# Lichtso/contrast_renderer

Measured on AMD Instinct MI355X. Metric: paths/sec, 10k mixed-Bezier paths @ 4096^2 (tessellate + tile raster), higher is better.
Workload: dtype f32

## Files before the change

contrast_renderer_amd/_ffi.py:

```python
import ctypes as C
import os

import numpy as np

HERE = os.path.dirname(os.path.abspath(__file__))
LIB_PATH = os.path.join(HERE, "libcontrast_hip.so")

OK = 0
ERR_NUMBER_OF_STENCIL_BITS_IS_UNSUPPORTED = 1
ERR_CLIP_STACK_OVERFLOW = 2
ERR_TOO_MANY_NESTED_OPACITY_GROUPS = 3
ERR_TOO_MANY_DASH_INTERVALS = 4
ERR_DYNAMIC_STROKE_OPTIONS_INDEX_OUT_OF_BOUNDS = 5
ERR_NON_FINITE = 6
ERR_DEGENERATE_CUBIC = 7
ERR_UNSUPPORTED = 8
ERR_HIP = 9
ERR_INVALID_ARGUMENT = 10

STATUS_NAMES = {
    0: "Ok",
    1: "NumberOfStencilBitsIsUnsupported",
    2: "ClipStackOverflow",
    3: "TooManyNestedOpacityGroups",
# ... 111 lines not shown
                 shape_dynamic_begin=None, dynamic_stroke_options=()):
        self.shape_path_begin = np.ascontiguousarray(shape_path_begin, dtype=np.uint32)
        self.path_segment_begin = np.ascontiguousarray(path_segment_begin, dtype=np.uint32)
        self.path_start = np.ascontiguousarray(path_start, dtype=np.float32).reshape(-1, 2)
        self.path_stroke_options = np.ascontiguousarray(path_stroke_options, dtype=np.int32)
        self.segment_types = np.ascontiguousarray(segment_types, dtype=np.uint8)
        self.control_data = np.ascontiguousarray(control_data, dtype=np.float32).reshape(-1)
        self.n_shapes = len(self.shape_path_begin) - 1
        self.n_paths = len(self.path_segment_begin) - 1
        self.n_segments = len(self.segment_types)
        assert self.path_start.shape[0] == self.n_paths and len(self.path_stroke_options) == self.n_paths
        assert int(self.shape_path_begin[-1]) == self.n_paths and int(self.path_segment_begin[-1]) == self.n_segments
        sizes = np.asarray(SEGMENT_FLOATS, dtype=np.int64)[self.segment_types]
        assert int(sizes.sum()) == self.control_data.size, "control_data does not match segment_types"
        self.stroke_options = (StrokeOptionsC * max(1, len(stroke_options)))(*stroke_options)
        self.n_stroke_options = len(stroke_options)
        if shape_dynamic_begin is None:
            shape_dynamic_begin = np.zeros(self.n_shapes + 1, dtype=np.uint32)
        self.shape_dynamic_begin = np.ascontiguousarray(shape_dynamic_begin, dtype=np.uint32)
        self.dynamic_stroke_options = (DynamicStrokeOptionsC * max(1, len(dynamic_stroke_options)))(*dynamic_stroke_options)
        self.n_dynamic_stroke_options = len(dynamic_stroke_options)
        c = PathBatchC()
        c.n_shapes = self.n_shapes
        c.shape_path_begin = _ptr(self.shape_path_begin, C.c_uint32)
        c.n_paths = self.n_paths
        c.path_segment_begin = _ptr(self.path_segment_begin, C.c_uint32)
        c.path_start = _ptr(self.path_start, C.c_float)
        c.path_stroke_options = _ptr(self.path_stroke_options, C.c_int32)
        c.n_segments = self.n_segments
        c.segment_types = _ptr(self.segment_types, C.c_uint8)
        c.control_data = _ptr(self.control_data, C.c_float)
        c.n_control_floats = self.control_data.size
        c.n_stroke_options = self.n_stroke_options
        c.stroke_options = C.cast(self.stroke_options, C.POINTER(StrokeOptionsC))
        c.shape_dynamic_begin = _ptr(self.shape_dynamic_begin, C.c_uint32)
        c.n_dynamic_stroke_options = self.n_dynamic_stroke_options
        c.dynamic_stroke_options = C.cast(self.dynamic_stroke_options, C.POINTER(DynamicStrokeOptionsC))
        self.c = c

    def input_bytes(self):
        stroked = int((self.path_stroke_options >= 0).sum())
        return self.control_data.nbytes + self.n_segments + 8 * self.n_paths + 32 * stroked

    def slice_shapes(self, begin, end):
        p0, p1 = int(self.shape_path_begin[begin]), int(self.shape_path_begin[end])
        s0, s1 = int(self.path_segment_begin[p0]), int(self.path_segment_begin[p1])
        sizes = np.asarray(SEGMENT_FLOATS, dtype=np.int64)[self.segment_types]
        offsets = np.concatenate([[0], np.cumsum(sizes)])
        d0, d1 = int(self.shape_dynamic_begin[begin]), int(self.shape_dynamic_begin[end])
        return PathBatch(
            self.shape_path_begin[begin:end + 1] - p0,
            self.path_segment_begin[p0:p1 + 1] - s0,
            self.path_start[p0:p1],
            self.path_stroke_options[p0:p1],
            self.segment_types[s0:s1],
            self.control_data[int(offsets[s0]):int(offsets[s1])],
            [self.stroke_options[i] for i in range(self.n_stroke_options)],
            self.shape_dynamic_begin[begin:end + 1] - d0,
            [self.dynamic_stroke_options[i] for i in range(d0, d1)],
        )


class DrawC(C.Structure):
    _fields_ = [("shape", C.c_uint32), ("instance", C.c_uint32), ("op", C.c_uint32), ("clip_depth", C.c_uint32), ("alpha_layer", C.c_uint32)]


MAX_GRADIENT_STOPS = 8


class GradientStopC(C.Structure):
    _fields_ = [("offset", C.c_float), ("color", C.c_float * 4)]


class PaintC(C.Structure):
    _fields_ = [("kind", C.c_uint32), ("spread", C.c_uint32), ("p0", C.c_float * 2), ("p1", C.c_float * 2), ("n_stops", C.c_uint32),
                ("stops", GradientStopC * MAX_GRADIENT_STOPS)]


class ImagePaintC(C.Structure):
    _fields_ = [("image", C.c_void_p), ("filter", C.c_uint32), ("spread_x", C.c_uint32), ("spread_y", C.c_uint32), ("m", C.c_float * 6)]


class CompositeC(C.Structure):
    _fields_ = [("op", C.c_uint32), ("mode", C.c_uint32), ("opacity", C.c_float), ("x", C.c_int32), ("y", C.c_int32)]


class ConvolveC(C.Structure):
    _fields_ = [("order_x", C.c_uint32), ("order_y", C.c_uint32), ("target_x", C.c_uint32), ("target_y", C.c_uint32), ("kernel", C.POINTER(C.c_float)),
                ("divisor", C.c_float), ("bias", C.c_float), ("edge", C.c_uint32), ("preserve_alpha", C.c_uint32)]


class LightingC(C.Structure):
    _fields_ = [("op", C.c_uint32), ("light", C.c_uint32), ("edge", C.c_uint32), ("surface_scale", C.c_float), ("constant", C.c_float), ("specular_exponent", C.c_float),
                ("color", C.c_float * 3), ("azimuth", C.c_float), ("elevation", C.c_float), ("position", C.c_float * 3), ("points_at", C.c_float * 3),
                ("spot_exponent", C.c_float), ("cone_angle", C.c_float)]


class TurbulenceC(C.Structure):
    _fields_ = [("kind", C.c_uint32), ("octaves", C.c_uint32), ("seed", C.c_int32), ("stitch", C.c_uint32), ("opaque", C.c_uint32), ("base_frequency", C.c_float * 2),
                ("offset", C.c_float * 2)]


class DisplaceC(C.Structure):
    _fields_ = [("scale", C.c_float * 2), ("x_channel", C.c_uint32), ("y_channel", C.c_uint32), ("filter", C.c_uint32), ("edge", C.c_uint32)]


class FontMetricsC(C.Structure):
    _fields_ = [("units_per_em", C.c_uint32), ("number_of_glyphs", C.c_uint32), ("ascender", C.c_int32), ("descender", C.c_int32),
                ("line_gap", C.c_int32), ("height", C.c_int32), ("has_x_height", C.c_int32), ("x_height", C.c_int32),
                ("has_vertical_metrics", C.c_int32), ("vertical_height", C.c_int32), ("vertical_line_gap", C.c_int32), ("has_kerning", C.c_int32)]


class TextLayoutC(C.Structure):
    _fields_ = [("size", C.c_float), ("orientation", C.c_uint32), ("major_alignment", C.c_uint32), ("minor_alignment", C.c_uint32)]


_lib = None


def _share_hip_runtime_with_torch():
    import importlib.util
    import sys
    if "torch" not in sys.modules and importlib.util.find_spec("torch") is not None:
        import torch


def load_library():
    global _lib
    if _lib is not None:
        return _lib
    if not os.path.exists(LIB_PATH):
        raise RuntimeError(f"{LIB_PATH} is missing: build it with `python -c 'import __graft_entry__ as g; g.build()'` "
                           "(hipcc --offload-arch=gfx950). contrast_renderer_amd has no CPU fallback.")
    _share_hip_runtime_with_torch()
    lib = C.CDLL(LIB_PATH)
    V = C.c_void_p
    sig = {
        "crh_renderer_create": (C.c_int, [C.POINTER(ConfigC), C.c_int, C.POINTER(V)]),
        "crh_renderer_destroy": (None, [V]),
        "crh_renderer_get_config": (C.c_int, [V, C.POINTER(ConfigC)]),
        "crh_renderer_create_blended": (C.c_int, [C.POINTER(ConfigC), C.POINTER(ColorTargetStateC), C.c_int, C.POINTER(V)]),
        "crh_renderer_get_blending": (C.c_int, [V, C.POINTER(ColorTargetStateC)]),
        "crh_convert_dynamic_stroke_options": (C.c_int, [C.POINTER(DynamicStrokeOptionsC), C.POINTER(DynamicStrokeDescriptorC)]),
        "crh_scene_upload": (C.c_int, [V, C.POINTER(PathBatchC), V, C.POINTER(V)]),
        "crh_scene_tessellate": (C.c_int, [V]),
        "crh_scene_status": (C.c_int, [V]),
        "crh_scene_destroy": (None, [V]),
        "crh_shape_from_paths": (C.c_int, [V, C.POINTER(PathBatchC), V, C.POINTER(V)]),
        "crh_scene_shape_layout": (C.c_int, [V, C.c_uint32, C.POINTER(C.c_uint64), C.POINTER(C.c_uint64)]),
        "crh_scene_shape_download": (C.c_int, [V, C.c_uint32, V, V]),
        "crh_scene_layout_all": (C.c_int, [V, C.POINTER(C.c_uint64), C.POINTER(C.c_uint64), C.POINTER(C.c_uint64)]),
        "crh_scene_download_all": (C.c_int, [V, V, V]),
        "crh_scene_traffic": (C.c_int, [V, C.POINTER(C.c_uint64), C.POINTER(C.c_uint64)]),
        "crh_scene_set_dynamic_stroke_options": (C.c_int, [V, C.c_uint32, C.c_uint32, C.POINTER(DynamicStrokeOptionsC)]),
        "crh_frame_create": (C.c_int, [V, C.c_uint32, C.c_uint32, C.POINTER(V)]),
        "crh_frame_create_format": (C.c_int, [V, C.c_uint32, C.c_uint32, C.c_uint32, C.POINTER(V)]),
        "crh_frame_format": (C.c_int, [V, C.POINTER(C.c_uint32)]),
        "crh_frame_destroy": (None, [V]),
        "crh_frame_clear": (C.c_int, [V]),
        "crh_frame_keep_pass_state": (C.c_int, [V]),
        "crh_frame_synchronize": (C.c_int, [V]),
        "crh_frame_set_tile_rows": (C.c_int, [V, C.c_uint32, C.c_uint32]),
        "crh_frame_clear_depth": (C.c_int, [V, C.c_float]),
        "crh_frame_upload_depth": (C.c_int, [V, C.POINTER(C.c_float)]),
        "crh_frame_download_depth": (C.c_int, [V, C.POINTER(C.c_float)]),
        "crh_scene_render": (C.c_int, [V, V, C.POINTER(C.c_float), C.POINTER(C.c_float)]),
        "crh_scene_set_instances": (C.c_int, [V, C.POINTER(C.c_float), C.POINTER(C.c_float)]),
        "crh_scene_render_resident": (C.c_int, [V, V]),
        "crh_scene_render_draws": (C.c_int, [V, V, C.POINTER(C.c_float), C.POINTER(C.c_float), C.c_uint32, C.POINTER(DrawC), C.c_uint32]),
        "crh_paint_validate": (C.c_int, [C.POINTER(PaintC)]),
        "crh_scene_set_paints": (C.c_int, [V, C.POINTER(PaintC), C.c_uint32, C.POINTER(C.c_int32), C.c_uint32]),
        "crh_image_create": (C.c_int, [V, C.c_uint32, C.c_uint32, V, C.POINTER(V)]),
        "crh_image_create_from_frame": (C.c_int, [V, C.POINTER(V)]),
        "crh_image_size": (C.c_int, [V, C.POINTER(C.c_uint32), C.POINTER(C.c_uint32)]),
        "crh_image_destroy": (None, [V]),
        "crh_image_generate_mipmaps": (C.c_int, [V]),
        "crh_image_level_count": (C.c_int, [V, C.POINTER(C.c_uint32)]),
        "crh_image_download_level": (C.c_int, [V, C.c_uint32, V, C.POINTER(C.c_uint32), C.POINTER(C.c_uint32)]),
        "crh_blur_taps": (C.c_int, [C.c_float, C.POINTER(C.c_uint32), C.c_uint32, C.POINTER(C.c_uint32)]),
        "crh_image_blur": (C.c_int, [V, C.c_float, C.c_float, C.c_uint32, C.POINTER(V)]),
        "crh_composite_validate": (C.c_int, [C.POINTER(CompositeC)]),
        "crh_composite_texels": (C.c_int, [C.POINTER(CompositeC), V, V, C.c_uint64, V]),
        "crh_image_composite": (C.c_int, [V, V, C.POINTER(CompositeC), C.POINTER(V)]),
        "crh_color_filter_validate": (C.c_int, [C.POINTER(C.c_float), C.POINTER(C.c_uint8)]),
        "crh_color_filter_texels": (C.c_int, [C.POINTER(C.c_float), C.POINTER(C.c_uint8), V, C.c_uint64, V]),
        "crh_image_color_filter": (C.c_int, [V, C.POINTER(C.c_float), C.POINTER(C.c_uint8), C.POINTER(V)]),
        "crh_morphology_size": (C.c_int, [C.c_uint32, C.c_uint32, C.c_uint32, C.c_uint32, C.c_uint32, C.c_uint32, C.POINTER(C.c_uint32), C.POINTER(C.c_uint32)]),
        "crh_morphology_texels": (C.c_int, [C.c_uint32, C.c_uint32, V, C.c_uint32, C.c_uint32, C.c_uint32, C.c_uint32, V]),
        "crh_image_morphology": (C.c_int, [V, C.c_uint32, C.c_uint32, C.c_uint32, C.c_uint32, C.POINTER(V)]),
        "crh_convolve_validate": (C.c_int, [C.POINTER(ConvolveC)]),
        "crh_convolve_coefficients": (C.c_int, [C.POINTER(ConvolveC), C.POINTER(C.c_int32), C.c_uint32, C.POINTER(C.c_int32)]),
        "crh_convolve_texels": (C.c_int, [C.c_uint32, C.c_uint32, V, C.POINTER(ConvolveC), V]),
        "crh_image_convolve": (C.c_int, [V, C.POINTER(ConvolveC), C.POINTER(V)]),
        "crh_lighting_validate": (C.c_int, [C.POINTER(LightingC)]),
        "crh_lighting_texels": (C.c_int, [C.c_uint32, C.c_uint32, V, C.POINTER(LightingC), V]),
        "crh_image_lighting": (C.c_int, [V, C.POINTER(LightingC), C.POINTER(V)]),
        "crh_turbulence_validate": (C.c_int, [C.POINTER(TurbulenceC)]),
        "crh_turbulence_tables": (C.c_int, [C.c_int32, C.POINTER(C.c_uint8), C.POINTER(C.c_double)]),
        "crh_turbulence_texels": (C.c_int, [C.c_uint32, C.c_uint32, C.POINTER(TurbulenceC), V]),
        "crh_image_turbulence": (C.c_int, [V, C.c_uint32, C.c_uint32, C.POINTER(TurbulenceC), C.POINTER(V)]),
        "crh_displace_validate": (C.c_int, [C.POINTER(DisplaceC)]),
        "crh_displace_offset": (C.c_int, [C.POINTER(DisplaceC), C.c_uint32, C.c_uint32, C.POINTER(C.c_int32)]),
        "crh_displace_texels": (C.c_int, [C.c_uint32, C.c_uint32, V, V, C.POINTER(DisplaceC), V]),
        "crh_image_displace": (C.c_int, [V, V, C.POINTER(DisplaceC), C.POINTER(V)]),
        "crh_image_paint_validate": (C.c_int, [C.POINTER(ImagePaintC)]),
        "crh_scene_set_paints_with_images": (C.c_int, [V, C.POINTER(PaintC), C.c_uint32, C.POINTER(ImagePaintC), C.c_uint32, C.POINTER(C.c_int32), C.c_uint32]),
        "crh_frame_upload": (C.c_int, [V, V]),
        "crh_frame_load_image": (C.c_int, [V, V]),
        "crh_frame_download": (C.c_int, [V, V]),
        "crh_frame_download_f16": (C.c_int, [V, V]),
        "crh_frame_device_pointer": (C.c_int, [V, C.POINTER(V)]),
        "crh_composite_over": (C.c_int, [V, C.POINTER(V), C.c_uint32, C.c_uint64, V]),
        "crh_comm_shard": (C.c_int, [C.c_uint32, C.c_uint32, C.c_uint32, C.POINTER(C.c_uint32), C.POINTER(C.c_uint32)]),
        "crh_comm_slab_rows": (C.c_int, [C.c_uint32, C.c_uint32, C.c_uint32, C.POINTER(C.c_uint32), C.POINTER(C.c_uint32)]),
        "crh_comm_unique_id": (C.c_int, [V]),
        "crh_comm_create": (C.c_int, [V, C.c_uint32, C.c_uint32, V, C.POINTER(V)]),
        "crh_comm_create_local": (C.c_int, [V, C.c_uint32, C.c_uint32, V, C.POINTER(V)]),
        "crh_comm_destroy": (None, [V]),
        "crh_frame_exchange": (C.c_int, [V, V, V]),
        "crh_frame_gather_slabs": (C.c_int, [V, V, V]),
        "crh_comm_local_exchange": (C.c_int, [V, C.POINTER(V), V]),
        "crh_comm_local_gather_slabs": (C.c_int, [V, C.POINTER(V), V]),
        "crh_comm_last_traffic": (C.c_int, [V, C.POINTER(C.c_uint64), C.POINTER(C.c_uint64)]),
        "crh_comm_last_timing": (C.c_int, [V, C.POINTER(C.c_float)]),
        "crh_comm_last_peer_bytes": (C.c_int, [V, C.POINTER(C.c_uint64)]),
        "crh_comm_info": (C.c_int, [V, C.POINTER(C.c_uint32), C.POINTER(C.c_int32)]),
        "crh_renderer_synchronize": (C.c_int, [V]),
        "crh_renderer_stream": (V, [V]),
        "crh_renderer_enable_timing": (C.c_int, [V, C.c_int]),
        "crh_renderer_kernel_times": (C.c_int, [V, C.POINTER(KernelTimeC), C.c_uint32, C.POINTER(C.c_uint32)]),
        "crh_selftest_fmath": (C.c_int, [V, C.c_int, C.POINTER(C.c_float), C.POINTER(C.c_float), C.POINTER(C.c_float), C.c_uint64]),
        "crh_selftest_srgb": (C.c_int, [V, C.POINTER(C.c_float), C.POINTER(C.c_uint8), C.c_uint64, C.POINTER(C.c_float)]),
        "crh_font_create": (C.c_int, [V, C.c_size_t, C.POINTER(V)]),
        "crh_font_destroy": (None, [V]),
        "crh_font_get_metrics": (C.c_int, [V, C.POINTER(FontMetricsC)]),
        "crh_font_glyph_index": (C.c_int, [V, C.c_uint32, C.POINTER(C.c_uint16), C.POINTER(C.c_uint32)]),
        "crh_font_glyph_advance": (C.c_int, [V, C.c_uint16, C.c_uint32, C.POINTER(C.c_uint16), C.POINTER(C.c_uint32)]),
        "crh_font_glyph_bounding_box": (C.c_int, [V, C.c_uint16, C.POINTER(C.c_int16), C.POINTER(C.c_uint32)]),
        "crh_font_glyphs_kerning": (C.c_int, [V, C.c_uint16, C.c_uint16, C.POINTER(C.c_int16), C.POINTER(C.c_uint32)]),
        "crh_paths_of_glyph": (C.c_int, [V, C.c_uint16, C.POINTER(V)]),
        "crh_paths_of_text": (C.c_int, [V, C.POINTER(TextLayoutC), C.POINTER(C.c_uint32), C.c_size_t, C.POINTER(C.c_float), C.c_size_t, C.POINTER(V)]),
        "crh_text_aligned_positions": (C.c_int, [V, C.POINTER(TextLayoutC), C.POINTER(C.c_uint32), C.c_size_t, C.POINTER(C.c_int64), C.POINTER(C.c_int64),
                                                 C.POINTER(C.c_int64), C.POINTER(C.c_uint64), C.POINTER(C.c_uint64), C.POINTER(C.c_uint64)]),
        "crh_path_elliptical_arc": (C.c_int, [C.POINTER(C.c_float), C.POINTER(C.c_float), C.c_float, C.c_uint32, C.c_uint32, C.POINTER(C.c_float),
                                              C.POINTER(C.c_float), C.c_uint32, C.POINTER(C.c_uint32), C.POINTER(C.c_uint32)]),
        "crh_path_list_transform": (C.c_int, [V, C.c_float, C.POINTER(C.c_float)]),
        "crh_path_list_view": (C.c_int, [V, C.POINTER(PathBatchC)]),
        "crh_path_list_destroy": (None, [V]),
        "crh_last_error": (C.c_char_p, []),
        "crh_version": (C.c_char_p, []),
    }
    for name, (res, args) in sig.items():
        fn = getattr(lib, name)
        fn.restype = res
        fn.argtypes = args
    lib._crh_signatures = sig
    _lib = lib
    return lib


class ContrastError(RuntimeError):

    def __init__(self, status, detail=""):
        self.status = status
        super().__init__(f"{STATUS_NAMES.get(status, status)}{(': ' + detail) if detail else ''}")


def check(status):
    if status != OK:
        detail = ""
        if status == ERR_HIP and _lib is not None:
            detail = (_lib.crh_last_error() or b"").decode()
        raise ContrastError(status, detail)
```

contrast_renderer_amd/csrc/api.hip:

```cpp
#include <hip/hip_runtime.h>

#include <algorithm>
#include <atomic>
#include <chrono>
#include <cmath>
#include <cstdio>
#include <cstdlib>
#include <cstring>
#include <memory>
#include <string>
#include <vector>

#include "api_internal.hpp"
#include "launch.hpp"
#include "raster_params.hpp"
#include "scene.hpp"

using namespace crh;

namespace {
thread_local std::string g_error;

struct DevBuf {
    void* p = nullptr;
// ... 466 lines not shown

crh_status decode_status(crh_scene* scene, uint32_t word) {
    (void)scene;
    if (word == 0xFFFFFFFFu) return CRH_OK;
    const uint32_t code = word & 0xFFu;
    if (code >= 0x80u) return CRH_ERR_UNSUPPORTED;
    return static_cast<crh_status>(code);
}

void bind_tess_pointers(crh_scene* sc) {
    SceneDev& d = sc->d;
    d.elem_scan = sc->elem_scan.as<ElemScan>();
    d.wg_total = sc->wg_total.as<uint32_t>();
    d.wg_base = sc->wg_base.as<uint32_t>();
    d.group_base = sc->group_base.as<uint32_t>();
    d.totals = sc->totals.as<uint32_t>();
    d.shape_base = sc->shape_base.as<uint32_t>();
    d.path_scan = sc->path_scan.as<uint32_t>();
    d.hull_count = sc->hull_count.as<uint32_t>();
    d.hull_large_count = sc->hull_large.as<uint32_t>();
    d.hull_large_list = sc->hull_large.as<uint32_t>() + 4;
    d.status = sc->status.as<uint32_t>();
    d.line_v = sc->line_v.as<Vertex2f1i>();
    d.joint_v = sc->joint_v.as<Vertex3f1i>();
    d.solid_v = sc->solid_v.as<Vertex0>();
    d.iq_v = sc->iq_v.as<Vertex2f>();
    d.ic_v = sc->ic_v.as<Vertex3f>();
    d.rq_v = sc->rq_v.as<Vertex3f>();
    d.rc_v = sc->rc_v.as<Vertex4f>();
    d.hull_cand = sc->hull_cand.as<Vertex0>();
    d.hull_v = sc->hull_v.as<Vertex0>();
    d.hull_sort = sc->hull_sort.as<float2>();
    d.hull_chain = sc->hull_chain.as<float2>();
    d.line_i = sc->line_i.as<uint16_t>();
    d.joint_i = sc->joint_i.as<uint16_t>();
    d.solid_i = sc->solid_i.as<uint16_t>();
    d.solid_flag = sc->solid_flag.as<uint8_t>();
    d.line_pair_cut = sc->line_pair_cut.as<uint8_t>();
    d.line_pair_mode = sc->line_pair_mode.as<uint8_t>();
    d.line_inc = sc->line_inc.as<float>();
}

crh_status flip_tess_set(crh_scene* sc) {
    crh_scene::TessShadow& o = sc->shadow;
    DevBuf* cur[kTessBufs];
    sc->tess_bufs(cur);
    if (!o.allocated) {
        for (int i = 0; i < kTessBufs; ++i)
            if (cur[i]->cap) HIP_TRY(o.buf[i].ensure(cur[i]->cap));
        for (hipEvent_t* e : {&o.tess_done, &o.vertices_free, &o.ranges_free})
            if (!*e) HIP_TRY(hipEventCreateWithFlags(e, hipEventDisableTiming));
        o.capacity_known = sc->capacity_known;
        std::memcpy(o.totals_host, sc->totals_host, sizeof(o.totals_host));
        std::memcpy(o.cap_host, sc->cap_host, sizeof(o.cap_host));
        if (o.buf[5].p) HIP_TRY(hipMemsetAsync(o.buf[5].p, 0, o.buf[5].cap, sc->renderer->tessellation_stream()));
        if (o.buf[6].p) HIP_TRY(hipMemsetAsync(o.buf[6].p, 0, o.buf[6].cap, sc->renderer->tessellation_stream()));
        o.emitted_bytes = sc->emitted_bytes;
        o.rendered_once = false;
        o.allocated = true;
    }
    for (int i = 0; i < kTessBufs; ++i) std::swap(*cur[i], o.buf[i]);
    std::swap(sc->tess_done, o.tess_done);
    std::swap(sc->vertices_free, o.vertices_free);
    std::swap(sc->ranges_free, o.ranges_free);
    std::swap(sc->capacity_known, o.capacity_known);
    std::swap(sc->rendered_once, o.rendered_once);
    std::swap(sc->last_render_one_event, o.last_render_one_event);
    std::swap(sc->emitted_bytes, o.emitted_bytes);
    for (int c = 0; c < NCH; ++c) std::swap(sc->totals_host[c], o.totals_host[c]), std::swap(sc->cap_host[c], o.cap_host[c]);
    for (int c = 0; c < NCH; ++c) sc->d.capacity[c] = sc->capacity_known ? sc->cap_host[c] : 0u;
    bind_tess_pointers(sc);
    return CRH_OK;
}

crh_status ensure_outputs(crh_scene* sc) {
    uint32_t want[NCH];
    for (int c = 0; c < NCH; ++c) want[c] = (uint32_t)std::min<uint64_t>(0xFFFFFFF0ull, (uint64_t)sc->totals_host[c] + sc->totals_host[c] / 16u + 64u);
    want[CH_LINE_V] &= ~1u;
    const uint32_t* t = want;
    SceneDev& d = sc->d;
    const size_t pairs = t[CH_LINE_V] / 2 + 1;
    HIP_TRY(sc->line_v.ensure((size_t)t[CH_LINE_V] * 20));
    HIP_TRY(sc->line_i.ensure(((size_t)t[CH_LINE_V] + t[CH_LINE_CUT]) * 2));
    HIP_TRY(sc->line_inc.ensure(pairs * 4));
    HIP_TRY(sc->line_pair_cut.ensure(pairs));
    HIP_TRY(sc->line_pair_mode.ensure(pairs));
    HIP_TRY(sc->joint_v.ensure((size_t)t[CH_JOINT] * 5 * 24));
    HIP_TRY(sc->joint_i.ensure((size_t)t[CH_JOINT] * 6 * 2));
    HIP_TRY(sc->solid_v.ensure((size_t)t[CH_SOLID_V] * 8));
    HIP_TRY(sc->solid_i.ensure(((size_t)t[CH_SOLID_V] + t[CH_SOLID_END]) * 2));
    HIP_TRY(sc->solid_flag.ensure((size_t)t[CH_SOLID_V] + 2));
    HIP_TRY(sc->iq_v.ensure((size_t)t[CH_IQ] * 3 * 16));
    HIP_TRY(sc->ic_v.ensure((size_t)t[CH_IC_V] * 20));
    HIP_TRY(sc->rq_v.ensure((size_t)t[CH_RQ] * 3 * 20));
    HIP_TRY(sc->rc_v.ensure((size_t)t[CH_RC_V] * 24));
    HIP_TRY(sc->hull_cand.ensure((size_t)t[CH_HULL] * 8));
    HIP_TRY(sc->hull_v.ensure((size_t)t[CH_HULL] * 8));
    if (sc->big_shapes || sc->has_stroke) {
        HIP_TRY(sc->hull_sort.ensure((size_t)t[CH_HULL] * 16 + 16));
        HIP_TRY(sc->hull_chain.ensure((size_t)t[CH_HULL] * 16 + 16));
    }
    for (int c = 0; c < NCH; ++c) d.capacity[c] = sc->cap_host[c] = t[c];
    bind_tess_pointers(sc);
    t = sc->totals_host;
    sc->emitted_bytes = (uint64_t)t[CH_LINE_V] * 20 + ((uint64_t)t[CH_LINE_V] + t[CH_LINE_CUT]) * 2 + (uint64_t)t[CH_JOINT] * (5 * 24 + 6 * 2) +
                        (uint64_t)t[CH_SOLID_V] * 8 + ((uint64_t)t[CH_SOLID_V] + t[CH_SOLID_END]) * 2 + (uint64_t)t[CH_IQ] * 48 + (uint64_t)t[CH_IC_V] * 20 +
                        (uint64_t)t[CH_RQ] * 60 + (uint64_t)t[CH_RC_V] * 24;
    return CRH_OK;
}

crh_status run_tessellation(crh_scene* sc, bool again) {
    crh_renderer* r = sc->renderer;
    HIP_TRY(hipSetDevice(r->device));
    if (sc->tessellated_once && !again) {
        const crh_status st = flip_tess_set(sc);
        if (st != CRH_OK) return st;
    }
    sc->tessellated_once = true;
    sc->tess_runs += 1u;
    if (again) sc->bounds_generation = 0;
    if (again) sc->hull_queued_state = 0;
    SceneDev& d = sc->d;
    const hipStream_t ts = r->tessellation_stream();
    if (sc->rendered_once) HIP_TRY(hipStreamWaitEvent(ts, sc->vertices_free, 0));
    if (sc->geometry_pending) {
        HIP_TRY(hipStreamWaitEvent(ts, sc->geometry_ready, 0));
        launch_build_elements(sc->pending_build, ts);
        sc->geometry_pending = false;
    }
    if (r->raster_exclusive && r->raster_events[1]) HIP_TRY(hipStreamWaitEvent(ts, r->raster_events[1], 0));
    r->begin_marks(1);
    HIP_TRY(hipMemsetAsync(d.status, 0xFF, 4, ts));
    if (d.n_elems == 0) {
        HIP_TRY(hipMemsetAsync(d.totals, 0, NCH * 4, ts));
        if (d.n_shapes) HIP_TRY(hipMemsetAsync(d.shape_base, 0, (size_t)d.n_shapes * kShapeRow * 4, ts));
        if (d.n_shapes) HIP_TRY(hipMemsetAsync(d.hull_count, 0, (size_t)d.n_shapes * 4, ts));
    }
    const uint64_t bytes[4] = {sc->input_bytes, 0, sc->input_bytes + sc->emitted_bytes, 0};
    if (!sc->capacity_known)
        for (int c = 0; c < NCH; ++c) d.capacity[c] = 0u;
    launch_tessellate(d, ts, r->mark_fn_tess(), r, bytes, sc->has_stroke, !sc->capacity_known || !sc->counts_valid || getenv("CRH_TESS_COUNT_EVERY_RUN") != nullptr);
    sc->counts_valid = true;
    if (!sc->capacity_known) {
        HIP_TRY(hipMemcpyAsync(sc->totals_host, d.totals, sizeof(uint32_t) * NCH, hipMemcpyDeviceToHost, ts));
        HIP_TRY(hipStreamSynchronize(ts));
        crh_status st = ensure_outputs(sc);
        if (st != CRH_OK) return st;
        sc->capacity_known = true;
        sc->optimistic = false;
    }
    if (sc->has_stroke) HIP_TRY(hipMemsetAsync(d.line_pair_cut, 0, sc->line_pair_cut.cap, ts));
    const uint64_t bytes2[4] = {sc->input_bytes, 0, sc->input_bytes + sc->emitted_bytes, (uint64_t)sc->totals_host[CH_HULL] * 8};
    if (sc->hull_queued_state == 1 && hipEventQuery(sc->hull_queued_ready) == hipSuccess) sc->hull_queued_state = 2;
    launch_emit(d, ts, r->mark_fn_tess(), r, bytes2, sc->has_stroke, sc->big_shapes, sc->hull_queued_state == 2 ? sc->hull_queued_host : nullptr);
    if (sc->hull_queued_state == 0 && (sc->has_stroke || sc->big_shapes)) {
        if (!sc->hull_queued_host) HIP_TRY(hipHostMalloc(reinterpret_cast<void**>(&sc->hull_queued_host), 16, hipHostMallocDefault));
        if (!sc->hull_queued_ready) HIP_TRY(hipEventCreateWithFlags(&sc->hull_queued_ready, hipEventDisableTiming));
        HIP_TRY(hipMemcpyAsync(sc->hull_queued_host, d.hull_large_count, 16, hipMemcpyDeviceToHost, ts));
        HIP_TRY(hipEventRecord(sc->hull_queued_ready, ts));
        sc->hull_queued_state = 1;
    }
    if (sc->rendered_once && !sc->last_render_one_event) HIP_TRY(hipStreamWaitEvent(ts, sc->ranges_free, 0));
    launch_plain_ranges(d, sc->shape_ncand.as<uint32_t>(), sc->shape_prim_begin.as<uint32_t>(), sc->shape_nslots.as<uint32_t>(), sc->shape_slot_begin.as<uint32_t>(),
                        sc->prim_scan_scratch.as<uint32_t>(), sc->prim_scan_scratch.as<uint32_t>() + ((size_t)(d.n_shapes + 511) / 512 + 2), ts);
    if (r->timing & 2u) crh_renderer::mark_cb_tess(r, "tess_prim_ranges", 0);
    HIP_TRY(hipEventRecord(sc->tess_done, ts));
    HIP_TRY(hipGetLastError());
    sc->layout_valid = false;
    return CRH_OK;
}

crh_status settle_tessellation(crh_scene* sc, uint32_t* status_word) {
    crh_renderer* r = sc->renderer;
    for (int attempt = 0; attempt < 2; ++attempt) {
        uint32_t word = 0;
        HIP_TRY(hipMemcpyAsync(&word, sc->d.status, 4, hipMemcpyDeviceToHost, r->tessellation_stream()));
        HIP_TRY(r->sync());
        if (word != 0xFFFFFFFFu && (word & 0xFFu) >= 0x80u && attempt == 0) {
            sc->capacity_known = false, sc->optimistic = false;
            crh_status st = run_tessellation(sc, true);
            if (st != CRH_OK) return st;
            continue;
        }
        if (sc->optimistic && sc->capacity_known) {
            HIP_TRY(hipMemcpy(sc->totals_host, sc->d.totals, sizeof(uint32_t) * NCH, hipMemcpyDeviceToHost));
            sc->optimistic = false;
        }
        *status_word = word;
        return CRH_OK;
    }
    return CRH_ERR_UNSUPPORTED;
}

crh_status fetch_layout(crh_scene* sc) {
    if (sc->layout_valid) return CRH_OK;
    crh_renderer* r = sc->renderer;
    uint32_t word;
    crh_status st = settle_tessellation(sc, &word);
    if (st != CRH_OK) return st;
    sc->shape_base_host.resize((size_t)sc->d.n_shapes * kShapeRow);
    sc->hull_count_host.resize(sc->d.n_shapes);
    if (sc->d.n_shapes) HIP_TRY(hipMemcpyAsync(sc->shape_base_host.data(), sc->d.shape_base, sc->shape_base_host.size() * 4, hipMemcpyDeviceToHost, r->stream));
    if (sc->d.n_shapes == 0) sc->shape_base_host.clear();
    if (sc->d.n_shapes) HIP_TRY(hipMemcpyAsync(sc->hull_count_host.data(), sc->d.hull_count, sc->hull_count_host.size() * 4, hipMemcpyDeviceToHost, r->stream));
    HIP_TRY(hipMemcpyAsync(sc->totals_host, sc->d.totals, sizeof(uint32_t) * NCH, hipMemcpyDeviceToHost, r->stream));
    HIP_TRY(r->sync());
    sc->layout_valid = true;
    return CRH_OK;
}

void shape_layout(const crh_scene* sc, uint32_t s, uint64_t vo[8], uint64_t io[3]) {
    const uint32_t* a = &sc->shape_base_host[(size_t)s * kShapeRow];
    const uint32_t* b = a + NCH;
    auto n = [&](int c) { return (uint64_t)(b[c] - a[c]); };
    uint64_t v = 0;
    v += n(CH_LINE_V) * 20;
    vo[0] = v;
    v += n(CH_JOINT) * 5 * 24;
    vo[1] = v;
    v += n(CH_SOLID_V) * 8;
    vo[2] = v;
    v += n(CH_IQ) * 3 * 16;
    vo[3] = v;
    v += n(CH_IC_V) * 20;
    vo[4] = v;
    v += n(CH_RQ) * 3 * 20;
    vo[5] = v;
    v += n(CH_RC_V) * 24;
    vo[6] = v;
    v += (uint64_t)sc->hull_count_host[s] * 8;
    vo[7] = v;
    uint64_t i = 0;
    i += (n(CH_LINE_V) + n(CH_LINE_CUT)) * 2;
    io[0] = i;
    i += n(CH_JOINT) * 6 * 2;
    io[1] = i;
    i += (n(CH_SOLID_V) + n(CH_SOLID_END)) * 2;
    io[2] = i;
}

struct HostCopy {
    std::vector<uint8_t> line_v, joint_v, solid_v, iq_v, ic_v, rq_v, rc_v, hull_v, line_i, joint_i, solid_i;
};
crh_status fetch_outputs(crh_scene* sc, HostCopy& h) {
    const uint32_t* t = sc->totals_host;
    hipStream_t st = sc->renderer->stream;
    auto get = [&](std::vector<uint8_t>& dst, const void* src, size_t bytes) -> crh_status {
        dst.resize(bytes);
        if (bytes) HIP_TRY(hipMemcpyAsync(dst.data(), src, bytes, hipMemcpyDeviceToHost, st));
        return CRH_OK;
    };
    crh_status rc;
    if ((rc = get(h.line_v, sc->d.line_v, (size_t)t[CH_LINE_V] * 20)) != CRH_OK) return rc;
    if ((rc = get(h.joint_v, sc->d.joint_v, (size_t)t[CH_JOINT] * 120)) != CRH_OK) return rc;
    if ((rc = get(h.solid_v, sc->d.solid_v, (size_t)t[CH_SOLID_V] * 8)) != CRH_OK) return rc;
    if ((rc = get(h.iq_v, sc->d.iq_v, (size_t)t[CH_IQ] * 48)) != CRH_OK) return rc;
    if ((rc = get(h.ic_v, sc->d.ic_v, (size_t)t[CH_IC_V] * 20)) != CRH_OK) return rc;
    if ((rc = get(h.rq_v, sc->d.rq_v, (size_t)t[CH_RQ] * 60)) != CRH_OK) return rc;
    if ((rc = get(h.rc_v, sc->d.rc_v, (size_t)t[CH_RC_V] * 24)) != CRH_OK) return rc;
    if ((rc = get(h.hull_v, sc->d.hull_v, (size_t)t[CH_HULL] * 8)) != CRH_OK) return rc;
    if ((rc = get(h.line_i, sc->d.line_i, ((size_t)t[CH_LINE_V] + t[CH_LINE_CUT]) * 2)) != CRH_OK) return rc;
    if ((rc = get(h.joint_i, sc->d.joint_i, (size_t)t[CH_JOINT] * 12)) != CRH_OK) return rc;
    if ((rc = get(h.solid_i, sc->d.solid_i, ((size_t)t[CH_SOLID_V] + t[CH_SOLID_END]) * 2)) != CRH_OK) return rc;
    HIP_TRY(hipStreamSynchronize(st));
    return CRH_OK;
}

void assemble_shape(const crh_scene* sc, const HostCopy& h, uint32_t s, uint8_t* vb, uint8_t* ib) {
    const uint32_t* a = &sc->shape_base_host[(size_t)s * kShapeRow];
    const uint32_t* b = a + NCH;
    auto put = [](uint8_t*& dst, const std::vector<uint8_t>& src, size_t begin, size_t bytes) {
        if (dst && bytes) {
            std::memcpy(dst, src.data() + begin, bytes);
            dst += bytes;
        }
    };
    put(vb, h.line_v, (size_t)a[CH_LINE_V] * 20, (size_t)(b[CH_LINE_V] - a[CH_LINE_V]) * 20);
    put(vb, h.joint_v, (size_t)a[CH_JOINT] * 120, (size_t)(b[CH_JOINT] - a[CH_JOINT]) * 120);
    put(vb, h.solid_v, (size_t)a[CH_SOLID_V] * 8, (size_t)(b[CH_SOLID_V] - a[CH_SOLID_V]) * 8);
    put(vb, h.iq_v, (size_t)a[CH_IQ] * 48, (size_t)(b[CH_IQ] - a[CH_IQ]) * 48);
    put(vb, h.ic_v, (size_t)a[CH_IC_V] * 20, (size_t)(b[CH_IC_V] - a[CH_IC_V]) * 20);
    put(vb, h.rq_v, (size_t)a[CH_RQ] * 60, (size_t)(b[CH_RQ] - a[CH_RQ]) * 60);
    put(vb, h.rc_v, (size_t)a[CH_RC_V] * 24, (size_t)(b[CH_RC_V] - a[CH_RC_V]) * 24);
    put(vb, h.hull_v, (size_t)a[CH_HULL] * 8, (size_t)sc->hull_count_host[s] * 8);
    put(ib, h.line_i, ((size_t)a[CH_LINE_V] + a[CH_LINE_CUT]) * 2, ((size_t)(b[CH_LINE_V] - a[CH_LINE_V]) + (b[CH_LINE_CUT] - a[CH_LINE_CUT])) * 2);
    put(ib, h.joint_i, (size_t)a[CH_JOINT] * 12, (size_t)(b[CH_JOINT] - a[CH_JOINT]) * 12);
    put(ib, h.solid_i, ((size_t)a[CH_SOLID_V] + a[CH_SOLID_END]) * 2, ((size_t)(b[CH_SOLID_V] - a[CH_SOLID_V]) + (b[CH_SOLID_END] - a[CH_SOLID_END])) * 2);
}

size_t grown_pair_bytes(const crh_frame* f, const uint32_t ov[8]) {
    size_t pairs = (size_t)ov[1] + (ov[1] >> 1) + 65536;
    if (ov[5] != 0) pairs = std::max(pairs, f->pair_capacity_bytes / 4 + f->pair_capacity_bytes / 8);
    return pairs * 4;
}
constexpr uint32_t kMovingListRadius = 3u;
int choose_pass(crh_scene* sc, const crh_frame* f, int* timed, bool* measured) {
    *timed = -1, *measured = false;
    if (!edge_pass_samples(sc->renderer->config.msaa_sample_count)) return 2;
    const bool rows_eligible = sc->renderer->config.msaa_sample_count == 1 && !sc->has_stroke && getenv("CRH_NO_ROWS") == nullptr;
    if (f->triangle_pass_for == sc && f->triangle_pass_generation == sc->generation) return 2;
    if (getenv("CRH_TRIANGLE_PASS")) return 2;
    if (getenv("CRH_ROWS")) return rows_eligible ? 3 : 1;
    if (getenv("CRH_EDGE_PASS")) return 1;
    if (sc->d.n_shapes < 256u) return 1;
    uint32_t cls = 0;
    for (uint64_t area = (uint64_t)f->width * f->height; area > 3u && cls < 15u; area >>= 2) ++cls;
    if (cls != sc->pass_class) {
        sc->pass_class = cls;
        sc->pass_choice = sc->pass_known[cls], sc->pass_frames = 0;
        for (crh_scene::PassTrial& t : sc->pass_trial) t.started = t.recorded = false;
    }
    if (sc->pass_choice == 3 && !rows_eligible) return 1;
    *measured = sc->pass_choice != 0;
    if (sc->pass_choice) return sc->pass_choice;
    const uint32_t candidates = rows_eligible ? 3u : 2u;
    static const int code_of[3] = {1, 2, 3};
    const uint32_t n = sc->pass_frames++;
// ... 957 lines not shown
            for (size_t i = 0; i < n; ++i) {
                uint32_t u;
                std::memcpy(&u, &src[i], 4);
                bad |= (uint32_t)((u & 0x7F800000u) == 0x7F800000u);
                dst[i] = src[i] + 0.0f;
            }
            return bad;
        };
        uint32_t bad = canonical(reinterpret_cast<float*>(arena + part[R_CONTROL].at), b->control_data, b->n_control_floats);
        bad |= canonical(reinterpret_cast<float*>(arena + part[R_START].at), b->path_start, 2u * (size_t)b->n_paths);
        if (bad != 0u) {
            if (!existing) {
                sc->geometry_stage.release();
                delete sc;
            }
            return CRH_ERR_NON_FINITE;
        }
        if (b->n_segments) std::memcpy(arena + part[R_TYPES].at, b->segment_types, b->n_segments);
        std::memcpy(arena + part[R_PATH_SEG].at, b->path_segment_begin, ((size_t)b->n_paths + 1) * 4);
        std::memcpy(arena + part[R_SHAPE_PATH].at, b->shape_path_begin, ((size_t)b->n_shapes + 1) * 4);
        std::memcpy(arena + part[R_SEG_PREFIX].at, seg_prefix.data(), ((size_t)b->n_segments + 1) * 4);
        if (b->n_segments) std::memcpy(arena + part[R_SEG_PATH].at, seg_path.data(), (size_t)b->n_segments * 4);
        if (b->n_paths) std::memcpy(arena + part[P_PATH_STROKE].at, b->path_stroke_options, (size_t)b->n_paths * 4);
        uint32_t* const dyn_begin = reinterpret_cast<uint32_t*>(arena + part[P_DYN_BEGIN].at);
        if (b->shape_dynamic_begin) std::memcpy(dyn_begin, b->shape_dynamic_begin, ((size_t)b->n_shapes + 1) * 4);
        else std::memset(dyn_begin, 0, ((size_t)b->n_shapes + 1) * 4);
        sc->shape_dyn_begin_host.assign(dyn_begin, dyn_begin + b->n_shapes + 1);
        if (b->n_stroke_options) std::memcpy(arena + part[P_OPTIONS].at, b->stroke_options, part[P_OPTIONS].bytes);
        if (!descriptors.empty()) std::memcpy(arena + part[P_DESCRIPTORS].at, descriptors.data(), part[P_DESCRIPTORS].bytes);
        if (!runs.empty()) std::memcpy(arena + part[P_RUNS].at, runs.data(), part[P_RUNS].bytes);
    }
    phase("element stream built");
    sc->renderer = r;
    sc->device = r->device;
    static std::atomic<uint64_t> next_generation{1};
    sc->generation = next_generation.fetch_add(1);
    if (!sc->tess_done) {
        if (!hip_ok(hipEventCreateWithFlags(&sc->tess_done, hipEventDisableTiming), "hipEventCreate") ||
            !hip_ok(hipEventCreateWithFlags(&sc->vertices_free, hipEventDisableTiming), "hipEventCreate") ||
            !hip_ok(hipEventCreateWithFlags(&sc->ranges_free, hipEventDisableTiming), "hipEventCreate")) {
            if (!existing) delete sc;
            return CRH_ERR_HIP;
        }
        for (hipEvent_t& e : sc->rec_raster_done)
            if (!hip_ok(hipEventCreateWithFlags(&e, hipEventDisableTiming), "hipEventCreate")) {
                if (!existing) delete sc;
                return CRH_ERR_HIP;
            }
    }
    const uint32_t new_runs = (runs.empty() || n_elems == 0u) ? 0u : (uint32_t)runs.size() - 1u;
    const bool same_structure = existing && sc->capacity_known && sc->d.n_elems == n_elems && sc->d.n_paths == b->n_paths && sc->d.n_shapes == b->n_shapes && sc->has_stroke == has_stroke &&
                                sc->d.n_runs == new_runs && sc->d.run_block == run_block && n_elems != 0u && sc->structure_hash == structure_hash && std::getenv("CRH_NO_OPTIMISTIC_UPLOAD") == nullptr;
    sc->structure_hash = structure_hash;
    sc->rendered_once = false;
    sc->last_render_one_event = false;
    if (sc->shadow.allocated && !same_structure) {
        if (!hip_ok(r->sync(), "sync")) return CRH_ERR_HIP;
        for (DevBuf& buf : sc->shadow.buf) buf.release();
        sc->shadow.allocated = false;
    }
    sc->tessellated_once_before_upload = sc->tessellated_once;
    sc->tessellated_once = false;
    {
        auto log2_of = [](uint32_t v) { uint32_t n = 0; while (v > 1u) v >>= 1, ++n; return n; };
        const uint32_t geometry = (log2_of(b->n_shapes) << 8) | log2_of(b->n_segments);
        if (geometry != sc->pass_geometry || !existing) {
            sc->pass_choice = 0, sc->pass_frames = 0, sc->pass_class = 0;
            std::memset(sc->pass_known, 0, sizeof(sc->pass_known));
            for (crh_scene::PassTrial& t : sc->pass_trial) t.started = t.recorded = false;
        } else if (sc->pass_choice == 0) {
            sc->pass_frames = 0;
            for (crh_scene::PassTrial& t : sc->pass_trial) t.started = t.recorded = false;
        }
        sc->pass_geometry = geometry;
    }
    for (bool& used : sc->rec_used) used = false;
    sc->n_segments = b->n_segments;
    sc->has_stroke = has_stroke;
    sc->capacity_known = same_structure, sc->optimistic = same_structure, sc->counts_valid = false;
    if (same_structure) {
        std::memcpy(sc->totals_host, sc->cap_host, sizeof(sc->totals_host));
        if (sc->shadow.allocated) std::memcpy(sc->shadow.totals_host, sc->shadow.cap_host, sizeof(sc->shadow.totals_host));
    } else {
        sc->lineage = sc->generation;
    }
    if (std::getenv("CRH_NO_LINEAGE")) sc->lineage = sc->generation;
    if (sc->hull_queued_state == 1) (void)hipEventSynchronize(sc->hull_queued_ready);
    sc->hull_queued_state = 0;
    sc->instances_set = false;
    sc->layout_valid = false;
    uint64_t stroked = 0;
    for (uint32_t p = 0; p < b->n_paths; ++p) stroked += b->path_stroke_options[p] >= 0;
    sc->input_bytes = (uint64_t)b->n_control_floats * 4 + b->n_segments + 8ull * b->n_paths + 32ull * stroked;
    sc->big_shapes = false;
    for (uint32_t s = 0; s < b->n_shapes; ++s) {
        const uint32_t p0 = b->shape_path_begin[s], p1 = b->shape_path_begin[s + 1];
        const uint64_t segs = b->path_segment_begin[p1] - b->path_segment_begin[p0];
        if (3 * segs + (p1 - p0) > 64) sc->big_shapes = true;
    }
    SceneDev& d = sc->d;
    std::memset(&d, 0, sizeof(d));
    d.n_elems = n_elems;
    d.n_paths = b->n_paths;
    d.n_shapes = b->n_shapes;
    d.n_wg = (n_elems + kTessBlock - 1) / kTessBlock;
    d.n_runs = new_runs;
    d.run_block = run_block;
    for (int c = 0; c < NCH; ++c) d.capacity[c] = same_structure ? sc->cap_host[c] : 0u;
    const hipStream_t st = r->upload_stream;
    crh_status rc;
    {
        if (!sc->geometry_ready && !hip_ok(hipEventCreateWithFlags(&sc->geometry_ready, hipEventDisableTiming), "hipEventCreate")) {
            rc = CRH_ERR_HIP;
            goto fail;
        }
        bool ok = true;
        if (existing && sc->tess_done && sc->tessellated_once_before_upload) ok = hip_ok(hipStreamWaitEvent(st, sc->tess_done, 0), "hipStreamWaitEvent");
        if (existing && sc->shadow.tess_done && sc->tessellated_once_before_upload) ok = ok && hip_ok(hipStreamWaitEvent(st, sc->shadow.tess_done, 0), "hipStreamWaitEvent");
        for (int k = 0; k < kPipelineDepth && ok; ++k)
            if (existing && sc->rec_used_ever[k]) ok = hip_ok(hipStreamWaitEvent(st, sc->rec_raster_done[k], 0), "hipStreamWaitEvent");
        const size_t second_off = has_stroke ? ((part[P_OFF].bytes + 255u) & ~(size_t)255u) : 0u;
        ok = ok && hip_ok(sc->geometry.ensure(arena_bytes + second_off + 256u), "hipMalloc");
        if (ok && staged_bytes) ok = hip_ok(hipMemcpyAsync(static_cast<uint8_t*>(sc->geometry.p) + staged_begin, staged, staged_bytes, hipMemcpyHostToDevice, st), "hipMemcpyAsync");
        if (ok) {
            uint8_t* const g = static_cast<uint8_t*>(sc->geometry.p);
            UploadBuild u = {};
            u.control = reinterpret_cast<const float*>(g + part[R_CONTROL].at), u.start = reinterpret_cast<const float*>(g + part[R_START].at), u.types = g + part[R_TYPES].at;
            u.path_seg = reinterpret_cast<const uint32_t*>(g + part[R_PATH_SEG].at), u.shape_path = reinterpret_cast<const uint32_t*>(g + part[R_SHAPE_PATH].at);
            u.n_segments = b->n_segments, u.n_paths = b->n_paths, u.n_shapes = b->n_shapes, u.n_elems = n_elems;
            u.seg_prefix = reinterpret_cast<const uint32_t*>(g + part[R_SEG_PREFIX].at), u.seg_path = reinterpret_cast<const uint32_t*>(g + part[R_SEG_PATH].at);
            u.elem_type = g + part[P_TYPE].at, u.elem_off = reinterpret_cast<uint32_t*>(g + part[P_OFF].at), u.elem_off_again = second_off ? reinterpret_cast<uint32_t*>(g + arena_bytes) : nullptr;
            u.elem_prev_off = reinterpret_cast<uint32_t*>(g + part[P_PREV].at), u.elem_path = reinterpret_cast<uint32_t*>(g + part[P_PATH].at), u.pool = reinterpret_cast<float*>(g + part[P_POOL].at);
            u.path_elem_begin = reinterpret_cast<uint32_t*>(g + part[P_PATH_BEGIN].at), u.path_shape = reinterpret_cast<uint32_t*>(g + part[P_PATH_SHAPE].at);
            u.shape_elem_begin = reinterpret_cast<uint32_t*>(g + part[P_SHAPE_BEGIN].at);
            sc->pending_build = u;
        }
        if (ok) ok = hip_ok(sc->status.ensure(4), "hipMalloc") && hip_ok(hipMemsetAsync(sc->status.p, 0xFF, 4, st), "hipMemset");
        if (ok) ok = hip_ok(sc->geometry_stage.done(st), "hipEventRecord") && hip_ok(hipEventRecord(sc->geometry_ready, st), "hipEventRecord");
        if (!ok) {
            rc = CRH_ERR_HIP;
            goto fail;
        }
        sc->geometry_pending = true;
    }
    if ((d.n_runs == 0u && (!hip_ok(sc->elem_scan.ensure((size_t)n_elems * sizeof(ElemScan)), "hipMalloc elem_scan") ||
        !hip_ok(sc->wg_total.ensure((size_t)d.n_wg * NCH * 4), "hipMalloc") || !hip_ok(sc->wg_base.ensure((size_t)d.n_wg * NCH * 4), "hipMalloc") || !hip_ok(sc->group_base.ensure(((size_t)d.n_wg / 64 + 2) * NCH * 4), "hipMalloc"))) ||
        (d.n_runs != 0u && (!hip_ok(sc->elem_cnt.ensure((size_t)n_elems * 4), "hipMalloc") || !hip_ok(sc->run_base.ensure(((size_t)d.n_runs + 1) * NCH * 4), "hipMalloc"))) ||
        (d.n_runs != 0u && has_stroke && !hip_ok(sc->path_scan.ensure((size_t)b->n_paths * 12), "hipMalloc")) ||
        !hip_ok(sc->totals.ensure(NCH * 4), "hipMalloc") || !hip_ok(sc->shape_base.ensure((size_t)b->n_shapes * kShapeRow * 4), "hipMalloc") ||
        !hip_ok(sc->hull_count.ensure((size_t)b->n_shapes * 4), "hipMalloc") || !hip_ok(sc->hull_large.ensure((3 * (size_t)b->n_shapes + 4) * 4), "hipMalloc") || !hip_ok(sc->status.ensure(4), "hipMalloc") ||
        !hip_ok(sc->transforms.ensure((size_t)b->n_shapes * 64), "hipMalloc") || !hip_ok(sc->colors.ensure((size_t)b->n_shapes * 16), "hipMalloc") ||
        !hip_ok(sc->shape_ncand.ensure((size_t)b->n_shapes * 4 + 4), "hipMalloc") || !hip_ok(sc->shape_prim_begin.ensure(((size_t)b->n_shapes + 1) * 4), "hipMalloc") ||
        !hip_ok(sc->shape_nslots.ensure((size_t)b->n_shapes * 4 + 4), "hipMalloc") || !hip_ok(sc->shape_slot_begin.ensure(((size_t)b->n_shapes + 1) * 4), "hipMalloc") ||
        !hip_ok(sc->prim_scan_scratch.ensure(((size_t)(b->n_shapes + 511) / 512 + 2) * 8), "hipMalloc")) {
        rc = CRH_ERR_HIP;
        goto fail;
    }
    {
        uint8_t* const g = static_cast<uint8_t*>(sc->geometry.p);
        auto at = [&](int k) { return g + part[k].at; };
        d.elem_type = at(P_TYPE);
        d.elem_off0 = reinterpret_cast<const uint32_t*>(at(P_OFF));
        d.elem_off = has_stroke ? reinterpret_cast<uint32_t*>(g + arena_bytes) : reinterpret_cast<uint32_t*>(at(P_OFF));
        d.elem_prev_off = reinterpret_cast<uint32_t*>(at(P_PREV));
        d.elem_path = reinterpret_cast<const uint32_t*>(at(P_PATH));
        d.pool = reinterpret_cast<const float*>(at(P_POOL));
        d.path_elem_begin = reinterpret_cast<const uint32_t*>(at(P_PATH_BEGIN));
        d.path_shape = reinterpret_cast<const uint32_t*>(at(P_PATH_SHAPE));
        d.path_stroke = reinterpret_cast<const int32_t*>(at(P_PATH_STROKE));
        d.shape_elem_begin = reinterpret_cast<const uint32_t*>(at(P_SHAPE_BEGIN));
        d.shape_dyn_begin = reinterpret_cast<const uint32_t*>(at(P_DYN_BEGIN));
        d.stroke_options = reinterpret_cast<const crh_stroke_options*>(at(P_OPTIONS));
        d.descriptors = reinterpret_cast<crh_dynamic_stroke_descriptor*>(at(P_DESCRIPTORS));
        d.tess_run = reinterpret_cast<const uint32_t*>(at(P_RUNS));
    }
    d.elem_cnt = sc->elem_cnt.as<uint32_t>(), d.run_base = sc->run_base.as<uint32_t>();
    bind_tess_pointers(sc);
    if (!existing) r->scenes.push_back(sc);
    phase("enqueued");
    *out = sc;
    return CRH_OK;
fail:
    if (!existing) {
        sc->release_all();
        delete sc;
    }
    return rc;
}

crh_status crh_scene_tessellate(crh_scene* sc) {
    if (!sc) return CRH_ERR_INVALID_ARGUMENT;
    return run_tessellation(sc, false);
}
crh_status crh_scene_status(crh_scene* sc) {
    if (!sc) return CRH_ERR_INVALID_ARGUMENT;
    HIP_TRY(hipSetDevice(sc->renderer->device));
    uint32_t word = 0xFFFFFFFFu;
    crh_status st = settle_tessellation(sc, &word);
    if (st != CRH_OK) return st;
    return decode_status(sc, word);
}
void crh_scene_destroy(crh_scene* sc) {
    if (!sc) return;
    (void)hipSetDevice(sc->device);
    if (sc->renderer) {
        (void)settle_frames_of(sc, true);
        (void)sc->renderer->sync();
        if (sc->renderer->last_pass_scene == sc) sc->renderer->last_pass_scene = nullptr, sc->renderer->last_pass_steady = false;
        for (hipEvent_t& seen : sc->renderer->raster_events)
            for (hipEvent_t mine : sc->rec_raster_done)
                if (seen == mine) seen = nullptr;
        std::vector<crh_scene*>& live = sc->renderer->scenes;
        for (size_t i = 0; i < live.size(); ++i)
            if (live[i] == sc) {
                live.erase(live.begin() + (long)i);
                break;
            }
    }
    sc->release_all();
    if (sc->geometry_ready) (void)hipEventSynchronize(sc->geometry_ready);
    for (hipEvent_t e : {sc->tess_done, sc->vertices_free, sc->ranges_free, sc->shadow.tess_done, sc->shadow.vertices_free, sc->shadow.ranges_free, sc->geometry_ready})
        if (e) (void)hipEventDestroy(e);
    for (hipEvent_t e : sc->rec_raster_done)
        if (e) (void)hipEventDestroy(e);
    for (crh_scene::PassTrial& t : sc->pass_trial)
        for (hipEvent_t e : t.e)
            if (e) (void)hipEventDestroy(e);
    delete sc;
}
crh_status crh_shape_from_paths(crh_renderer* r, const crh_path_batch* one_shape, crh_scene* existing, crh_scene** out) {
    if (!one_shape || one_shape->n_shapes != 1) return CRH_ERR_INVALID_ARGUMENT;
    crh_status st = crh_scene_upload(r, one_shape, existing, out);
    if (st != CRH_OK) return st;
    st = crh_scene_tessellate(*out);
    if (st != CRH_OK) return st;
    return crh_scene_status(*out);
}

crh_status crh_scene_shape_layout(crh_scene* sc, uint32_t shape, uint64_t vo[8], uint64_t io[3]) {
    if (!sc || shape >= sc->d.n_shapes) return CRH_ERR_INVALID_ARGUMENT;
    HIP_TRY(hipSetDevice(sc->renderer->device));
    crh_status st = fetch_layout(sc);
    if (st != CRH_OK) return st;
    shape_layout(sc, shape, vo, io);
    return CRH_OK;
}
crh_status crh_scene_shape_download(crh_scene* sc, uint32_t shape, void* vb, void* ib) {
    if (!sc || shape >= sc->d.n_shapes) return CRH_ERR_INVALID_ARGUMENT;
    HIP_TRY(hipSetDevice(sc->renderer->device));
    crh_status st = fetch_layout(sc);
    if (st != CRH_OK) return st;
    HostCopy h;
    if ((st = fetch_outputs(sc, h)) != CRH_OK) return st;
    assemble_shape(sc, h, shape, static_cast<uint8_t*>(vb), static_cast<uint8_t*>(ib));
    return CRH_OK;
}
crh_status crh_scene_layout_all(crh_scene* sc, uint64_t* layout, uint64_t* total_v, uint64_t* total_i) {
    if (!sc) return CRH_ERR_INVALID_ARGUMENT;
    HIP_TRY(hipSetDevice(sc->renderer->device));
    crh_status st = fetch_layout(sc);
    if (st != CRH_OK) return st;
    uint64_t tv = 0, ti = 0;
    for (uint32_t s = 0; s < sc->d.n_shapes; ++s) {
        uint64_t vo[8], io[3];
        shape_layout(sc, s, vo, io);
        if (layout) {
            for (int k = 0; k < 8; ++k) layout[(size_t)s * 11 + k] = vo[k];
            for (int k = 0; k < 3; ++k) layout[(size_t)s * 11 + 8 + k] = io[k];
        }
        tv += vo[7];
        ti += io[2];
    }
    if (total_v) *total_v = tv;
    if (total_i) *total_i = ti;
    return CRH_OK;
}
crh_status crh_scene_download_all(crh_scene* sc, void* vb, void* ib) {
    if (!sc) return CRH_ERR_INVALID_ARGUMENT;
    HIP_TRY(hipSetDevice(sc->renderer->device));
    crh_status st = fetch_layout(sc);
    if (st != CRH_OK) return st;
    HostCopy h;
    if ((st = fetch_outputs(sc, h)) != CRH_OK) return st;
    uint8_t* v = static_cast<uint8_t*>(vb);
    uint8_t* i = static_cast<uint8_t*>(ib);
    for (uint32_t s = 0; s < sc->d.n_shapes; ++s) {
        uint64_t vo[8], io[3];
        shape_layout(sc, s, vo, io);
        assemble_shape(sc, h, s, v, i);
        if (v) v += vo[7];
        if (i) i += io[2];
    }
    return CRH_OK;
}
crh_status crh_scene_traffic(crh_scene* sc, uint64_t* bytes_read, uint64_t* bytes_written) {
    if (!sc) return CRH_ERR_INVALID_ARGUMENT;
    if (bytes_read) *bytes_read = sc->input_bytes;
    if (bytes_written) *bytes_written = sc->emitted_bytes;
    return CRH_OK;
}
crh_status crh_scene_set_dynamic_stroke_options(crh_scene* sc, uint32_t shape, uint32_t group, const crh_dynamic_stroke_options* o) {
    if (!sc || !o || shape >= sc->d.n_shapes) return CRH_ERR_INVALID_ARGUMENT;
    const uint32_t begin = sc->shape_dyn_begin_host[shape], end = sc->shape_dyn_begin_host[shape + 1];
    if (group >= end - begin) return CRH_ERR_DYNAMIC_STROKE_OPTIONS_INDEX_OUT_OF_BOUNDS;
    crh_dynamic_stroke_descriptor d;
    const crh_status st = convert_options(*o, d);
    if (st != CRH_OK) return st;
    HIP_TRY(hipSetDevice(sc->renderer->device));
    {
        const crh_status pending = settle_frames_of(sc, false);
        if (pending != CRH_OK) return pending;
    }
    if (sc->geometry_ready) HIP_TRY(hipEventSynchronize(sc->geometry_ready));
    HIP_TRY(hipMemcpyAsync(sc->d.descriptors + begin + group, &d, sizeof(d), hipMemcpyHostToDevice, sc->renderer->stream));
    HIP_TRY(sc->renderer->sync());
    return CRH_OK;
}

crh_status crh_frame_create(crh_renderer* r, uint32_t width, uint32_t height, crh_frame** out) { return crh_frame_create_format(r, width, height, CRH_FORMAT_RGBA8, out); }
crh_status crh_frame_format(const crh_frame* f, uint32_t* format) {
    if (!f || !format) return CRH_ERR_INVALID_ARGUMENT;
    *format = f->format;
    return CRH_OK;
}
crh_status crh_frame_create_format(crh_renderer* r, uint32_t width, uint32_t height, uint32_t format, crh_frame** out) {
    if (!r || !out || width == 0 || height == 0 || width > 65535u || height > 65535u || format > CRH_FORMAT_BGRA8_SRGB_ATTACHMENT) return CRH_ERR_INVALID_ARGUMENT;
    HIP_TRY(hipSetDevice(r->device));
    crh_frame* f = new crh_frame;
    f->renderer = r;
    f->format = format;
    f->device = r->device;
    f->width = width;
    f->height = height;
    f->tiles_x = (width + 15) / 16;
    f->tiles_y = (height + 15) / 16;
    f->n_tiles = f->tiles_x * f->tiles_y;
    bool ok = hip_ok(f->rgba8.ensure(f->image_bytes()), "hipMalloc frame") && hip_ok(hipEventCreateWithFlags(&f->ext_read, hipEventDisableTiming), "hipEventCreate") &&
              hip_ok(hipEventCreateWithFlags(&f->ext_write, hipEventDisableTiming), "hipEventCreate");
    for (crh_frame::BinSet& set : f->sets)
        ok = ok && hip_ok(set.tile_count_cursor.ensure((size_t)f->n_tiles * 8 + 512), "hipMalloc") && hip_ok(set.tile_offset.ensure((size_t)(f->n_tiles + 1) * 4), "hipMalloc") &&
             hip_ok(set.tile_list.ensure(f->pair_capacity_bytes), "hipMalloc") &&
             hip_ok(hipEventCreateWithFlags(&set.bin_done, hipEventDisableTiming), "hipEventCreate") &&
             hip_ok(hipEventCreateWithFlags(&set.raster_done, hipEventDisableTiming), "hipEventCreate") &&
             hip_ok(hipEventCreateWithFlags(&set.flags_ready, hipEventDisableTiming), "hipEventCreate") &&
             hip_ok(hipHostMalloc(reinterpret_cast<void**>(&set.flags_host), sizeof(uint32_t) * 128, hipHostMallocDefault), "hipHostMalloc");
    if (!ok) {
        crh_frame_destroy(f);
        return CRH_ERR_HIP;
    }
    HIP_TRY(hipMemsetAsync(f->rgba8.p, 0, f->image_bytes(), r->stream));
    if (r->config.depth_compare != CRH_COMPARE_ALWAYS || r->config.depth_write_enabled) {
        const size_t n = (size_t)width * height * r->config.msaa_sample_count;
        HIP_TRY(f->depth.ensure(n * 4));
        HIP_TRY(hipMemsetD32Async(reinterpret_cast<hipDeviceptr_t>(f->depth.p), 0x3f800000, n, r->stream));
    }
    for (crh_frame::BinSet& set : f->sets) {
        set.overflow_p = static_cast<uint8_t*>(set.tile_count_cursor.p) + (size_t)f->n_tiles * 8;
        HIP_TRY(hipMemsetAsync(set.overflow_p, 0, 512, r->stream));
    }
    HIP_TRY(r->sync());
    r->frames.push_back(f);
    *out = f;
    return CRH_OK;
}
void crh_frame_destroy(crh_frame* f) {
    if (!f) return;
    (void)hipSetDevice(f->device);
    if (f->ext_read_set) (void)hipEventSynchronize(f->ext_read);
    if (f->ext_write_set) (void)hipEventSynchronize(f->ext_write);
    if (f->renderer) {
        (void)f->renderer->sync();
        for (size_t i = 0; i < f->renderer->frames.size(); ++i)
            if (f->renderer->frames[i] == f) {
                f->renderer->frames.erase(f->renderer->frames.begin() + (long)i);
                break;
            }
    }
    DevBuf* all[] = {&f->tile_order, &f->item_cost, &f->bin_batches, &f->tile_base, &f->tile_base_b, &f->tile_caps, &f->rgba8, &f->depth, &f->items, &f->item_transforms, &f->item_colors, &f->item_transforms_b, &f->item_colors_b, &f->item_ncand, &f->item_prim_begin, &f->item_scan_scratch,
                     &f->item_nslots, &f->item_slot_begin, &f->state_stencil, &f->state_alpha, &f->state_color};
    for (DevBuf* b : all) b->release();
    f->item_upload_t.release();
    f->item_upload_c.release();
    for (InstanceSlot& k : f->item_slot) k.release();
    for (crh_frame::BinSet& set : f->sets) {
        DevBuf* bins[] = {&set.tile_count_cursor, &set.tile_offset, &set.tile_list, &set.scan_scratch, &set.pair_tile, &set.pair_pos, &set.pair_key, &set.bin_queue, &set.item_elsewhere};
        for (DevBuf* b : bins) b->release();
        if (set.bin_done) (void)hipEventDestroy(set.bin_done);
        if (set.raster_done) (void)hipEventDestroy(set.raster_done);
        if (set.flags_ready) (void)hipEventDestroy(set.flags_ready);
        if (set.flags_host) (void)hipHostFree(set.flags_host), set.flags_host = nullptr;
    }
    if (f->ext_read) {
        if (f->ext_read_set) (void)hipEventSynchronize(f->ext_read);
        (void)hipEventDestroy(f->ext_read);
    }
    if (f->ext_write) {
        if (f->ext_write_set) (void)hipEventSynchronize(f->ext_write);
        (void)hipEventDestroy(f->ext_write);
    }
    delete f;
}
crh_status crh_frame_clear(crh_frame* f) {
    if (!f) return CRH_ERR_INVALID_ARGUMENT;
    f->cleared = true;
    f->carry = f->carry_valid = f->carry_recolor = false;
    return f->depth.p ? crh_frame_clear_depth(f, 1.0f) : CRH_OK;
}
crh_status crh_frame_keep_pass_state(crh_frame* f) {
    if (!f) return CRH_ERR_INVALID_ARGUMENT;
    f->carry = true;
    return CRH_OK;
}
namespace {
crh_status load_pixels(crh_frame* f, const void* rgba8, hipMemcpyKind kind) {
    crh_renderer* r = f->renderer;
    HIP_TRY(hipSetDevice(r->device));
    const crh_status st = settle_frame(f);
    if (st != CRH_OK) return st;
    HIP_TRY(order_after_external(f, r->stream));
    HIP_TRY(hipMemcpyAsync(f->rgba8.p, rgba8, f->image_bytes(), kind, r->stream));
    HIP_TRY(hipStreamSynchronize(r->stream));
    f->cleared = false;
    f->carry = f->carry_valid = f->carry_recolor = false;
    f->counts_describe_pixels = false, f->check_pending = false, f->last_scene = nullptr;
    return CRH_OK;
}
bool loadable(const crh_frame* f) { return f && f->renderer && f->format != CRH_FORMAT_RGBA16F && f->slab_ty0 == 0u && f->slab_ty1 == 0xFFFFFFFFu; }
}
crh_status crh_frame_upload(crh_frame* f, const void* rgba8) {
    if (!loadable(f) || !rgba8) return CRH_ERR_INVALID_ARGUMENT;
    return load_pixels(f, rgba8, hipMemcpyHostToDevice);
}
crh_status crh_frame_load_image(crh_frame* f, const crh_image* image) {
    if (!loadable(f) || !image) return CRH_ERR_INVALID_ARGUMENT;
    if (image->renderer != f->renderer) {
        g_error = "crh_frame_load_image: the image belongs to another renderer";
        return CRH_ERR_INVALID_ARGUMENT;
    }
    if (image->width != f->width || image->height != f->height) {
        g_error = "crh_frame_load_image: the image's size is not the frame's";
        return CRH_ERR_INVALID_ARGUMENT;
    }
    return load_pixels(f, image->pixels->p, hipMemcpyDeviceToDevice);
}
crh_status crh_frame_clear_depth(crh_frame* f, float value) {
    if (!f || !f->depth.p || !std::isfinite(value)) return CRH_ERR_INVALID_ARGUMENT;
    crh_renderer* r = f->renderer;
    HIP_TRY(hipSetDevice(r->device));
    uint32_t bits;
    memcpy(&bits, &value, 4);
    HIP_TRY(hipMemsetD32Async(reinterpret_cast<hipDeviceptr_t>(f->depth.p), (int)bits, (size_t)f->width * f->height * r->config.msaa_sample_count, r->stream));
// ... 659 lines not shown
```

contrast_renderer_amd/csrc/bin_edges.hip:

```cpp
#include <algorithm>
#include <type_traits>
#include <vector>

#include "edge_slots.hpp"
#include "launch.hpp"

namespace crh {

struct ItemCtx {
    uint32_t shape, instance, dyn0;
    uint32_t lv0, jn0, iq0, ic0, rq0, rc0, hull0, sv0;
    uint32_t cb[8];
    float m0, m4, m12, m1, m5, m13;
    float col[4];
};
CRH_D ItemCtx item_ctx(const SceneDev& s, const RasterParams& r, const DrawItem& it, const uint32_t cb[8]) {
    ItemCtx c;
    const uint32_t* b0 = s.shape_base + it.shape * kShapeRow;
    c.shape = it.shape, c.instance = it.instance, c.dyn0 = s.shape_dyn_begin[it.shape];
    c.lv0 = b0[CH_LINE_V], c.jn0 = b0[CH_JOINT], c.iq0 = b0[CH_IQ], c.ic0 = b0[CH_IC_V], c.rq0 = b0[CH_RQ], c.rc0 = b0[CH_RC_V], c.hull0 = b0[CH_HULL], c.sv0 = b0[CH_SOLID_V];
#pragma unroll
    for (int i = 0; i < 8; ++i) c.cb[i] = cb[i];
    const float* m = r.transforms + 16u * it.instance;
    c.m0 = m[0], c.m4 = m[4], c.m12 = m[12], c.m1 = m[1], c.m5 = m[5], c.m13 = m[13];
// ... 1716 lines not shown
                else
                    begin = sub * region + got;
            }
            for (uint32_t w = 0; w < kFlatWaveCount; ++w) {
                const uint32_t mine = wave_entries[kFlatWaveCount + w] + wave_entries[w];
                wave_entries[w] = begin;
                if (begin != 0xFFFFFFFFu) begin += mine;
            }
        }
        lds_barrier();
        st.at = wave_entries[wave];
#pragma unroll 1
        for (uint32_t ch = 0; !direct_cells && ch * kFlatThreads < n_pool; ++ch) {
            const uint32_t p = ch * kFlatThreads + tid;
            const bool active = p < n_pool;
            const uint32_t j = active ? find_item(pool_begin, p) : 0u;
            const FlatItem& fi = items[j];
            const uint32_t q = active ? p - pool_begin[j] : 0u, row_len = max(fi.nx, 1u), qy = q / row_len, qx = q - qy * row_len;
            const uint32_t tile = (fi.ty_a + qy) * r.tiles_x + fi.tx_a + qx;
            const uint32_t verdict = active ? (uint32_t)pool_back[p] : 0u;
            const SynthKeys keys = synth_keys(fi, verdict);
            const uint32_t cover_key = keys.cover, bd_key = keys.bd, hbd_key = keys.hbd;
            uint32_t left = verdict & 4095u, n_bd = (verdict >> 12) & 4095u, pos = active ? pool_cursor[p] - left : 0u;
            bool cover = (verdict >> 24) & 1u;
            if (replay && active) pool_back[p] = (int)tile;
            for (;;) {
                const unsigned long long ballot = __ballot(left != 0u);
                if (!ballot) break;
                uint32_t key = 0;
                if (left) {
                    if (cover)
                        cover = false, key = cover_key;
                    else if (n_bd)
                        --n_bd, key = bd_key;
                    else
                        key = hbd_key;
                }
                stage_append<true>(st, r, lane, ballot, tile, pos, key);
                if (left) ++pos, --left;
            }
        }
        lds_barrier();
        CRH_FLAT_PHASE(6)
        if (replay) {
            stage_flush_reserved(st, r, lane);
            for (uint32_t i = lane; i < n_hits; i += 64u) {
                const uint32_t rec = *hit_slot(i), cell = (rec >> kHitIndexBits) & ((1u << kHitCellBits) - 1u);
                const uint32_t tile = (uint32_t)pool_back[cell], pos = pool_cursor[cell] + (rec & ((1u << kHitIndexBits) - 1u)), key = key0 + (rec >> (kHitIndexBits + kHitCellBits));
#ifdef CRH_ABLATE
                if (r.debug & 512u) continue;
#endif
                if (direct_cells) {
                    if (pos < tile) r.tile_list[pos] = key;
                    else r.overflow[0] = 1u;
                } else if (r.direct) {
                    const uint32_t place = r.tile_base[tile];
                    if (pos < r.tile_base[tile + 1u] - place && place + pos < r.pair_capacity) r.tile_list[place + pos] = key;
                    else r.overflow[0] = 1u;
                } else if (st.at != 0xFFFFFFFFu) {
                    r.pair_tile[st.at + i] = tile, r.pair_pos[st.at + i] = pos, r.pair_key[st.at + i] = key;
                }
            }
            if (st.at != 0xFFFFFFFFu) st.at += n_hits;
        } else {
        for_edge_rows([&](bool active, const BinEdge& e, uint32_t j, const FlatItem& fi, int ty, int x0, int x1, uint32_t key) {
            const uint32_t base = pool_begin[j] + ((uint32_t)ty - fi.ty_a) * fi.nx, tx_a = fi.tx_a;
            const uint32_t cols = wave_max_u32(active && x0 <= x1 ? (uint32_t)(x1 - x0 + 1) : 0u);
            for (uint32_t c = 0; c < cols; ++c) {
                const int tx = x0 + (int)c;
                const bool hit = active && tx <= x1 && matters(e, tx, ty);
                const unsigned long long ballot = __ballot(hit);
                if (ballot) {
                    uint32_t pos = 0;
                    if (hit) pos = atomicAdd(&pool_cursor[base + ((uint32_t)tx - tx_a)], 1u);
                    stage_append<true>(st, r, lane, ballot, (uint32_t)ty * r.tiles_x + (uint32_t)tx, pos, key);
                }
            }
        });
        if (n_tris) {
            const FlatItem& fi = items[tri.item];
            const bool live = tri.nt != 0u && fi.n_rect != 0u;
            const uint32_t base = pool_begin[tri.item], nx = fi.nx, tx_a = fi.tx_a, ty_a = fi.ty_a;
            walk_tri(tri, live, [&](bool hit, uint32_t tx, uint32_t ty) {
                const unsigned long long ballot = __ballot(hit);
                if (ballot) {
                    uint32_t pos = 0;
                    if (hit) pos = atomicAdd(&pool_cursor[base + (ty - ty_a) * nx + (tx - tx_a)], 1u);
                    stage_append<true>(st, r, lane, ballot, ty * r.tiles_x + tx, pos, tri.key);
                }
            });
        }
        stage_flush_reserved(st, r, lane);
        }
        CRH_FLAT_PHASE(7)
        bool any_folded = false;
        for (uint32_t j = 0; j < n_turn; ++j) any_folded = any_folded || (items[j].flags & (kFiHullTris | kFiSkip)) == kFiHullTris;
        if (any_folded) {
            st.sub = ((kFlatWaveCount * blockIdx.x + wave + 977u * turn) * 2654435761u) >> 26;
            for (uint32_t j = 0; j < n_turn; ++j) {
                const FlatItem& fi = items[j];
                if ((fi.flags & (kFiHullTris | kFiSkip)) != kFiHullTris) continue;
                const ItemCtx& ctx = fi.ctx;
                for (uint32_t t0 = 64u * wave; t0 + 2u < fi.n_hull; t0 += kFlatThreads) {
                    const uint32_t t = t0 + lane;
                    PrimRec rec = {};
                    bool drawn = false;
                    if (t + 2u < fi.n_hull) {
                        drawn = setup_plain_triangle(s, r, ctx, ctx.cb[6] + t, rec);
                        if (drawn) *reinterpret_cast<PrimRec*>(r.slots + (size_t)(fi.hull_slot0 + 4u * t) * 32u) = rec;
                    }
                    bin_triangles(st, r, lane, drawn, rec.cov, fi.hull_slot0 + 4u * t, ry_first, r_last);
                }
            }
            stage_flush(st, r, lane);
        }
#ifdef CRH_ABLATE
        dump_items += n_turn, dump_tris += n_tris, dump_edges += n_edges, dump_pool += n_pool, dump_work += n_work, dump_walk += wave_max_u32(tri.nt);
#endif
        next += n_turn;
        ++turn;
        CRH_FLAT_PHASE(8)
    }
    if (r.bin_batches && turn > 1u && tid0 == 0u) atomicAdd(&r.overflow[kExtraTurnsWord], turn - 1u);
#ifdef CRH_ABLATE
    if ((r.debug & 65536u) && tid0 == 0u) {
        const unsigned long long life = __builtin_amdgcn_s_memtime() - born_t;
        atomicMax(reinterpret_cast<unsigned long long*>(r.overflow + 120), life);
        atomicAdd(reinterpret_cast<unsigned long long*>(r.overflow + 122), life);
        atomicAdd(r.overflow + 124, 1u);
    }
    if ((r.debug & 65536u) && r.item_cost && tid0 == 0u) {
        uint32_t* rec = r.item_cost + 2u * (size_t)(r.n_items + 1u) + 8u * (size_t)blockIdx.x;
        rec[0] = (uint32_t)(__builtin_amdgcn_s_memtime() - born_t), rec[1] = min(turn, 255u) | (min(dump_wave_hits, 4095u) << 8) | (min(dump_batch_hits, 4095u) << 20), rec[2] = dump_items, rec[3] = dump_tris, rec[4] = dump_edges, rec[5] = dump_pool, rec[6] = dump_work, rec[7] = dump_walk;
    }
#endif
}

__global__ __launch_bounds__(256) void k_scatter(RasterParams r) {
    if (r.overflow[0] | r.overflow[5]) return;
    const uint32_t i = blockIdx.x * 256u + threadIdx.x, region = r.pair_capacity / kSubStreams;
    const uint32_t sub = i / region, at = i - sub * region;
    if (sub >= kSubStreams || at >= r.pair_cursor[sub]) return;
    r.tile_list[r.tile_offset[r.pair_tile[i]] + r.pair_pos[i]] = r.pair_key[i];
}

void launch_slot_ranges(const SceneDev& s, const RasterParams& r, uint32_t n_items, uint32_t* item_nslots, uint32_t* slot_begin, uint32_t* scratch, hipStream_t stream) {
    if (n_items == 0) {
        (void)hipMemsetAsync(slot_begin, 0, 4, stream);
        return;
    }
    hipLaunchKernelGGL(k_item_nslots, dim3((n_items + 255u) / 256u), dim3(256), 0, stream, s, r, n_items, item_nslots);
    launch_scan_u32(item_nslots, slot_begin, scratch, n_items, stream);
}
__global__ __launch_bounds__(64) void k_shape_counts(SceneDev s, uint32_t* shape_ncand, uint32_t* shape_nslots) {
    const uint32_t shape = blockIdx.x * 64u + threadIdx.x;
    if (shape >= s.n_shapes) return;
    uint32_t c[8];
    shape_ncand[shape] = shape_candidates(s, shape, c);
    RasterParams plain = {};
    shape_nslots[shape] = item_slots(s, item_of(plain, shape)).total;
}
struct WaveScan {
    const uint32_t* in;
    uint32_t* out;
    uint32_t* block_sum;
};
constexpr uint32_t kWaveScanItems = 8, kWaveScanBlock = 64 * kWaveScanItems;
__global__ __launch_bounds__(64) void k_wave_scan_local2(WaveScan a, WaveScan b, uint32_t n) {
    const WaveScan j = blockIdx.y ? b : a;
    const uint32_t lane = threadIdx.x, i0 = blockIdx.x * kWaveScanBlock + lane * kWaveScanItems;
    uint32_t v[kWaveScanItems], mine = 0;
#pragma unroll
    for (uint32_t k = 0; k < kWaveScanItems; ++k) v[k] = i0 + k < n ? j.in[i0 + k] : 0u, mine += v[k];
    uint32_t incl = mine;
#pragma unroll
    for (int d = 1; d < 64; d <<= 1) {
        const uint32_t up = __shfl_up(incl, d, 64);
        if (lane >= (uint32_t)d) incl += up;
    }
    uint32_t run = incl - mine;
#pragma unroll
    for (uint32_t k = 0; k < kWaveScanItems; ++k) {
        if (i0 + k < n) j.out[i0 + k] = run;
        run += v[k];
    }
    if (lane == 63u) j.block_sum[blockIdx.x] = incl;
}
__global__ __launch_bounds__(64) void k_wave_scan_add2(WaveScan a, WaveScan b, uint32_t n, uint32_t blocks) {
    const WaveScan j = blockIdx.y ? b : a;
    const uint32_t lane = threadIdx.x;
    uint32_t sum = 0;
    for (uint32_t k = lane; k < blockIdx.x; k += 64u) sum += j.block_sum[k];
#pragma unroll
    for (int d = 32; d > 0; d >>= 1) sum += (uint32_t)__shfl_xor((int)sum, d, 64);
    const uint32_t i0 = blockIdx.x * kWaveScanBlock + lane * kWaveScanItems;
#pragma unroll
    for (uint32_t k = 0; k < kWaveScanItems; ++k)
        if (i0 + k < n) j.out[i0 + k] += sum;
    if (blockIdx.x + 1u == blocks && lane == 0u) j.out[n] = sum + j.block_sum[blockIdx.x];
}
void launch_plain_ranges(const SceneDev& s, uint32_t* shape_ncand, uint32_t* shape_prim_begin, uint32_t* shape_nslots, uint32_t* shape_slot_begin, uint32_t* scratch0, uint32_t* scratch1, hipStream_t stream) {
    if (s.n_shapes == 0) {
        (void)hipMemsetAsync(shape_prim_begin, 0, 4, stream);
        (void)hipMemsetAsync(shape_slot_begin, 0, 4, stream);
        return;
    }
    hipLaunchKernelGGL(k_shape_counts, dim3((s.n_shapes + 63u) / 64u), dim3(64), 0, stream, s, shape_ncand, shape_nslots);
    const uint32_t blocks = (s.n_shapes + kWaveScanBlock - 1u) / kWaveScanBlock;
    const WaveScan a = {shape_ncand, shape_prim_begin, scratch0}, b = {shape_nslots, shape_slot_begin, scratch1};
    hipLaunchKernelGGL(k_wave_scan_local2, dim3(blocks, 2), dim3(64), 0, stream, a, b, s.n_shapes);
    hipLaunchKernelGGL(k_wave_scan_add2, dim3(blocks, 2), dim3(64), 0, stream, a, b, s.n_shapes, blocks);
}
uint32_t flat_threads_for(uint32_t n_items) {
    if (const char* e = getenv("CRH_BIN_FLAT_THREADS")) return atoi(e) == 64 ? 64u : kFlatThreads;
    return (n_items >= 65536u && kFlatThreads != 64u) ? 64u : kFlatThreads;
}
bool bin_itemwise(const RasterParams& r) {
    const FlatShape shape = flat_shape(flat_threads_for(r.n_items));
    return getenv("CRH_BIN_ITEMWISE") != nullptr ||
           (getenv("CRH_BIN_FLAT") == nullptr && r.n_items != 0u && (r.hint_tris / r.n_items > shape.tris / 2u || r.hint_edges / r.n_items > shape.edges / 2u));
}
void flat_batches(const uint32_t* cost, uint32_t n_items, std::vector<uint32_t>& runs) {
    const FlatShape shape = flat_shape(flat_threads_for(n_items));
    const uint32_t kFlatBatch = shape.batch, kFlatTris = shape.tris, kFlatEdges = shape.edges, kFlatPool = shape.pool;
    struct Run {
        uint32_t first, last;
        float ticks;
    };
    std::vector<Run> all;
    const float cap = getenv("CRH_BIN_BATCH_TICKS") ? (float)atof(getenv("CRH_BIN_BATCH_TICKS")) : 0.0f;
    const uint32_t most = getenv("CRH_BIN_BATCH_ITEMS") ? (uint32_t)std::max(1, atoi(getenv("CRH_BIN_BATCH_ITEMS"))) : kFlatBatch;
    uint32_t n = 0, tris = 0, edges = 0, cells = 0, widest = 0, folded = 0, first = 0;
    bool closed = false;
    auto ticks = [&]() { return 76000.0f + 2000.0f * (float)n + 40.0f * (float)tris + 250.0f * (float)edges + 60.0f * (float)cells + 45.0f * (float)widest + 8000.0f * (float)folded; };
    for (uint32_t i = 0; i < n_items; ++i) {
        const uint32_t c = cost[2u * i], w = cost[2u * i + 1u];
        const bool alone = c == 0xFFFFFFFFu;
        const uint32_t t = (w >> 31) ? 0u : (w & 0x1FFu), e = (w >> 31) ? 0u : ((w >> 9) & 0x3FFu);
        if (n != 0u && (alone || closed || n >= std::min(most, kFlatBatch) || tris + t > kFlatTris || edges + e > kFlatEdges || cells + c > kFlatPool || (cap > 0.0f && ticks() > cap))) {
            all.push_back(Run{first, i, ticks()});
            n = tris = edges = cells = widest = folded = 0u, first = i, closed = false;
        }
        n += 1u, tris += t, edges += e, cells += alone ? 0u : c, widest = std::max(widest, alone ? 0u : c), folded += (w >> 29) & 1u;
        if (alone) closed = true;
    }
    if (n_items) all.push_back(Run{first, n_items, ticks()});
    const bool in_order = getenv("CRH_BIN_BATCH_ORDER") != nullptr;
    if (!in_order) std::stable_sort(all.begin(), all.end(), [](const Run& a, const Run& b) { return a.ticks > b.ticks; });
    runs.clear();
    for (const Run& run : all) runs.push_back(run.first), runs.push_back(run.last);
}
void flat_batch_limits(uint32_t n_items, uint32_t limits[4]) {
    const FlatShape shape = flat_shape(flat_threads_for(n_items));
    limits[0] = shape.batch, limits[1] = shape.tris, limits[2] = shape.edges, limits[3] = shape.pool;
}
constexpr uint32_t kClearWordsPerLane = 8u;
__global__ __launch_bounds__(64) void k_clear_words(uint32_t* words, uint32_t n) {
    const uint32_t first = blockIdx.x * (64u * kClearWordsPerLane) + threadIdx.x;
#pragma unroll
    for (uint32_t k = 0; k < kClearWordsPerLane; ++k) {
        const uint32_t i = first + k * 64u;
        if (i < n) words[i] = 0u;
    }
}
void launch_clear_words(uint32_t* words, size_t n_words, hipStream_t stream) {
    if (n_words == 0) return;
    if (getenv("CRH_NO_CLEAR_KERNEL") != nullptr || n_words > 0x7FFFFFFFu) {
        (void)hipMemsetAsync(words, 0, n_words * sizeof(uint32_t), stream);
        return;
    }
    const uint32_t per_group = 64u * kClearWordsPerLane;
    hipLaunchKernelGGL(k_clear_words, dim3((uint32_t)((n_words + per_group - 1u) / per_group)), dim3(64), 0, stream, words, (uint32_t)n_words);
}
uint32_t launch_bin_edges(const SceneDev& s, const RasterParams& r, uint32_t samples, hipStream_t stream, MarkFn mark, void* ctx, hipEvent_t after_bin) {
    if (!edge_pass_samples(samples)) return 0u;
    launch_clear_words(r.tile_count, (size_t)r.n_tiles + 8u + kSubStreams + 8u, stream);
    const uint32_t pinned = getenv("CRH_BIN_ITEMS") ? max(1, atoi(getenv("CRH_BIN_ITEMS"))) : 0u;
    const bool itemwise = bin_itemwise(r);
    auto by_samples = [&](auto launch) { samples == 4 ? launch(std::integral_constant<int, 4>{}) : launch(std::integral_constant<int, 1>{}); };
    uint32_t route = r.n_items == 0u ? 0u : (itemwise ? kBinItemwise : (r.bin_batches ? kBinFlatBatches : kBinFlatItems));
    if (r.n_items && itemwise) {
        const uint32_t items_per_group = pinned ? pinned : min(8u, max(1u, (r.n_items + 12287u) / 12288u));
        route |= min(items_per_group, 255u) << 16;
        const uint32_t bin_grid = (r.n_items + items_per_group - 1u) / items_per_group;
        by_samples([&](auto S) { hipLaunchKernelGGL((k_bin_edges<S(), false>), dim3(bin_grid), dim3(128), 0, stream, s, r); });
    } else if (r.n_items) {
        const FlatShape shape = flat_shape(flat_threads_for(r.n_items));
        const uint32_t resident = (getenv("CRH_BIN_CUS") ? (uint32_t)max(1, atoi(getenv("CRH_BIN_CUS"))) : 256u) * (4u * CRH_FLAT_WAVES) / (shape.threads / 64u);
        const uint32_t by_tris = r.hint_tris ? (uint32_t)((uint64_t)shape.tris * 9u / 10u * r.n_items / r.hint_tris) : shape.batch;
        const uint32_t by_edges = r.hint_edges ? (uint32_t)((uint64_t)shape.edges * 9u / 10u * r.n_items / r.hint_edges) : shape.batch;
        const uint32_t fitting = max(1u, min(shape.batch, min(by_tris, by_edges)));
        const uint32_t items_per_group = pinned ? min(pinned, shape.batch) : min(fitting, max(1u, (r.n_items + resident - 1u) / resident));
        const uint32_t flat_grid = r.bin_batches ? r.n_bin_batches : (r.n_items + items_per_group - 1u) / items_per_group, queue_grid = min(r.n_items, 4096u);
        if (!r.bin_batches) route |= min(items_per_group, 255u) << 16;
        const char* const replay_env = getenv("CRH_BIN_REPLAY");
        const bool replay = flat_replays(shape.threads) && !(replay_env && atoi(replay_env) == 0);
        const uint32_t replay_cap = getenv("CRH_BIN_REPLAY_CAP") ? (uint32_t)max(0, atoi(getenv("CRH_BIN_REPLAY_CAP"))) : 0xFFFFFFFFu;
        if (replay) route |= kBinReplayed;
        by_samples([&](auto S) {
            if (shape.threads == 64u) hipLaunchKernelGGL((k_bin_flat<S(), 64u, false>), dim3(flat_grid), dim3(64), 0, stream, s, r, items_per_group, replay_cap);
            else if (replay) hipLaunchKernelGGL((k_bin_flat<S(), kFlatThreads, kFlatThreads == 128u>), dim3(flat_grid), dim3(kFlatThreads), 0, stream, s, r, items_per_group, replay_cap);
            else hipLaunchKernelGGL((k_bin_flat<S(), kFlatThreads, false>), dim3(flat_grid), dim3(kFlatThreads), 0, stream, s, r, items_per_group, replay_cap);
            if (!r.skip_queue) hipLaunchKernelGGL((k_bin_edges<S(), true>), dim3(queue_grid), dim3(128), 0, stream, s, r);
        });
    }
    if (after_bin) (void)hipEventRecord(after_bin, stream);
    if (mark) mark(ctx, "raster_bin", 0);
    if (!r.direct) launch_scan_tiles(r, stream);
    if (mark) mark(ctx, "raster_tile_scan", 0);
    return route;
}
void launch_scatter(const RasterParams& r, hipStream_t stream, MarkFn mark, void* ctx) {
    if (r.pair_capacity && !r.direct) hipLaunchKernelGGL(k_scatter, dim3((r.pair_capacity + 255u) / 256u), dim3(256), 0, stream, r);
    if (mark) mark(ctx, "raster_scatter", 0);
}
constexpr uint32_t kListSlack = 64u;
__global__ __launch_bounds__(64) void k_tile_caps(const uint32_t* count, uint32_t* caps, uint32_t n, uint32_t tiles_x, uint32_t radius) {
    const uint32_t t = blockIdx.x * 64u + threadIdx.x;
    if (t >= n) return;
    uint32_t longest = count[t];
    if (radius) {
        const uint32_t tiles_y = n / tiles_x, ty = t / tiles_x, tx = t - ty * tiles_x;
        const uint32_t x0 = tx > radius ? tx - radius : 0u, x1 = min(tiles_x - 1u, tx + radius), y0 = ty > radius ? ty - radius : 0u, y1 = min(tiles_y - 1u, ty + radius);
        for (uint32_t y = y0; y <= y1; ++y)
            for (uint32_t x = x0; x <= x1; ++x) longest = max(longest, count[y * tiles_x + x]);
    }
    caps[t] = longest + (longest >> 1) + kListSlack;
}
void launch_tile_bases(const uint32_t* tile_count, uint32_t* caps, uint32_t* tile_base, uint32_t* scratch, uint32_t n_tiles, uint32_t tiles_x, uint32_t radius, hipStream_t stream) {
    const uint32_t blocks = (n_tiles + kWaveScanBlock - 1u) / kWaveScanBlock;
    const WaveScan job = {caps, tile_base, scratch};
    hipLaunchKernelGGL(k_tile_caps, dim3((n_tiles + 63u) / 64u), dim3(64), 0, stream, tile_count, caps, n_tiles, tiles_x, radius);
    hipLaunchKernelGGL(k_wave_scan_local2, dim3(blocks, 1), dim3(64), 0, stream, job, job, n_tiles);
    hipLaunchKernelGGL(k_wave_scan_add2, dim3(blocks, 1), dim3(64), 0, stream, job, job, n_tiles, blocks);
}

}
```

contrast_renderer_amd/csrc/edge_slots.hpp:

```cpp
#pragma once
#include "raster_common.hpp"

namespace crh {

constexpr uint32_t EK_EDGE = 0, EK_SYNTH = 7, EK_COVER_TRI = 8;
constexpr uint32_t kCoverHull = 9u, kCoverOpaque = 18u;
constexpr uint32_t kEdgeTl = 1u, kEdgeSigmaPos = 2u, kEdgeHull = 4u;
struct EdgeRec {
    uint32_t flags, pad0;
    float lo_x, lo_y, hi_x, hi_y, bx, nay;
};
struct SynthRec {
    uint32_t flags, first_slot;
    float r, g, b, a;
    uint32_t synth_a, pad;
};
static_assert(sizeof(EdgeRec) == 32 && sizeof(SynthRec) == 32, "slots");

struct ItemSlots {
    uint32_t n_tri, n_fe, n_hull;
    uint32_t fe0, synth_a, hull0, synth_b, total;
    uint32_t cb[8];
};
CRH_D ItemSlots item_slots(const SceneDev& s, const DrawItem& it) {
    ItemSlots k;
    shape_candidates(s, it.shape, k.cb);
    const uint32_t* b0 = s.shape_base + it.shape * kShapeRow;
    const bool stencil = (it.ops & 1u) != 0u, cover = (it.ops >> 4) != 0u;
    const uint32_t hn = s.hull_count[it.shape];
    k.n_tri = stencil ? k.cb[1] + (k.cb[6] - k.cb[2]) : 0u;
    k.n_fe = stencil ? b0[NCH + CH_SOLID_V] - b0[CH_SOLID_V] : 0u;
    k.n_hull = (cover && hn >= 3u) ? hn : 0u;
    k.fe0 = 4u * k.n_tri;
    k.synth_a = k.fe0 + ((k.n_fe + 3u) & ~3u);
    k.hull0 = k.synth_a + 4u;
    k.synth_b = k.hull0 + (k.n_hull ? 4u * (k.n_hull - 2u) : 0u);
    k.total = k.synth_b + 28u;
    return k;
}

}
```

contrast_renderer_amd/csrc/launch.hpp:

```cpp
#pragma once
#include <hip/hip_runtime.h>

#include <vector>

#include "raster_params.hpp"
#include "scene.hpp"

namespace crh {

typedef void (*MarkFn)(void*, const char*, uint64_t);

void launch_tessellate(const SceneDev& s, hipStream_t stream, MarkFn mark, void* ctx, const uint64_t bytes[4], bool has_stroke, bool need_totals);
void launch_emit(const SceneDev& s, hipStream_t stream, MarkFn mark, void* ctx, const uint64_t bytes[4], bool has_stroke, bool big_shapes, const uint32_t* hull_queued);
void launch_build_elements(const UploadBuild& u, hipStream_t stream);
void launch_fmath(int fn, const float* a, const float* b, float* out, uint64_t n, hipStream_t stream);

void launch_prim_ranges(const SceneDev& s, uint32_t* shape_ncand, uint32_t* shape_prim_begin, uint32_t* scratch, hipStream_t stream);
void launch_item_ranges(const SceneDev& s, const RasterParams& r, uint32_t* item_ncand, uint32_t* item_prim_begin, uint32_t* scratch, hipStream_t stream);
void launch_bin(const SceneDev& s, const RasterParams& r, uint32_t samples, hipStream_t stream, MarkFn mark, void* ctx, hipEvent_t after_setup);
void launch_fill(const SceneDev& s, const RasterParams& r, uint32_t samples, hipStream_t stream, MarkFn mark, void* ctx, hipEvent_t after_fill);
uint32_t launch_raster(const SceneDev& s, const RasterParams& r, uint32_t samples, hipStream_t stream, MarkFn mark, void* ctx, uint64_t raster_bytes, bool has_stroke,
                       const BlendForm* blend, const PaintArgs* paint = nullptr, const ImageArgs* images = nullptr, bool mips = false);
void launch_paint_items(const RasterParams& r, const PaintTable& t, hipStream_t stream);
void launch_paint_items_images(const RasterParams& r, const PaintTable& t, uint32_t n_gradients, hipStream_t stream);
void launch_image_downsample(const uint32_t* src, uint32_t src_w, uint32_t src_h, uint32_t* dst, uint32_t dst_w, uint32_t dst_h, hipStream_t stream);
void launch_scan_u32(const uint32_t* in, uint32_t* out, uint32_t* block_sum, uint32_t n, hipStream_t stream);
void launch_scan_u32_pair(const uint32_t* in0, uint32_t* out0, uint32_t* block_sum0, const uint32_t* in1, uint32_t* out1, uint32_t* block_sum1, uint32_t n, hipStream_t stream);
void launch_scan_tiles(const RasterParams& r, hipStream_t stream);
void launch_state_colors_from_image(const RasterParams& r, uint32_t samples, hipStream_t stream);
void launch_selftest_srgb(const float* x, uint8_t* codes, uint64_t n, float* decoded, hipStream_t stream);
void launch_composite(const uint8_t* const* layers_dev, uint32_t n_layers, uint64_t n_pixels, uint8_t* dst, hipStream_t stream);

constexpr uint32_t kBlurMaxRadius = 192;
constexpr uint32_t kBlurTapPad = 8;
void launch_image_blur_h(const uint32_t* src, uint32_t src_w, uint32_t src_h, void* tmp, uint32_t out_w, const uint32_t* taps, uint32_t radius, uint32_t origin, uint32_t edge, hipStream_t stream);
void launch_image_blur_v(const void* tmp, uint32_t tmp_h, uint32_t* out, uint32_t out_w, uint32_t out_h, const uint32_t* pairs, uint32_t radius, uint32_t origin, uint32_t edge, hipStream_t stream);
void launch_image_composite(const uint32_t* backdrop, uint32_t w, uint32_t h, const uint32_t* source, uint32_t source_w, uint32_t source_h, int32_t x, int32_t y, uint32_t o, uint32_t mode,
                            uint32_t op, uint32_t* out, hipStream_t stream);
struct ColorFilterCoefficients;
void launch_image_color_filter(const uint32_t* src, uint32_t w, uint32_t h, const ColorFilterCoefficients& f, const uint32_t* tables, uint32_t* out, hipStream_t stream);
void launch_image_morph_h(const uint32_t* src, uint32_t src_w, uint32_t src_h, uint32_t* out, uint32_t out_w, uint32_t op, uint32_t radius, uint32_t origin, uint32_t edge, hipStream_t stream);
void launch_image_morph_v(const uint32_t* in, uint32_t in_h, uint32_t* out, uint32_t out_w, uint32_t out_h, uint32_t op, uint32_t radius, uint32_t origin, uint32_t edge, hipStream_t stream);
struct ConvolveCoefficients;
void launch_image_convolve(const uint32_t* src, uint32_t w, uint32_t h, const ConvolveCoefficients& f, uint32_t order_x, uint32_t order_y, uint32_t target_x, uint32_t target_y, uint32_t edge,
                           bool preserve_alpha, uint32_t* out, hipStream_t stream);
struct LightingConstants;
void launch_image_lighting(const uint32_t* src, uint32_t w, uint32_t h, const LightingConstants& f, uint32_t op, uint32_t light, uint32_t edge, uint32_t* out, hipStream_t stream);
struct TurbulenceTables;
struct TurbulenceConstants;
void launch_image_turbulence(const TurbulenceTables* tables, uint32_t w, uint32_t h, const TurbulenceConstants& f, uint32_t kind, bool opaque, uint32_t* out, hipStream_t stream);
struct DisplaceConstants;
void launch_image_displace(const uint32_t* src, const uint32_t* map, uint32_t w, uint32_t h, const DisplaceConstants& f, uint32_t* out, hipStream_t stream);

void launch_clear_words(uint32_t* words, size_t n_words, hipStream_t stream);
void launch_slot_ranges(const SceneDev& s, const RasterParams& r, uint32_t n_items, uint32_t* item_nslots, uint32_t* slot_begin, uint32_t* scratch, hipStream_t stream);
uint32_t launch_bin_edges(const SceneDev& s, const RasterParams& r, uint32_t samples, hipStream_t stream, MarkFn mark, void* ctx, hipEvent_t after_bin);
void launch_scatter(const RasterParams& r, hipStream_t stream, MarkFn mark, void* ctx);
void launch_shape_bounds(const SceneDev& s, float* bounds, hipStream_t stream);
void launch_slab_items(const RasterParams& r, uint8_t* elsewhere, hipStream_t stream);
void launch_plain_ranges(const SceneDev& s, uint32_t* shape_ncand, uint32_t* shape_prim_begin, uint32_t* shape_nslots, uint32_t* shape_slot_begin, uint32_t* scratch0, uint32_t* scratch1, hipStream_t stream);
bool bin_itemwise(const RasterParams& r);
void flat_batches(const uint32_t* cost, uint32_t n_items, std::vector<uint32_t>& runs);
void flat_batch_limits(uint32_t n_items, uint32_t limits[4]);
void launch_tile_bases(const uint32_t* tile_count, uint32_t* caps, uint32_t* tile_base, uint32_t* scratch, uint32_t n_tiles, uint32_t tiles_x, uint32_t radius, hipStream_t stream);

uint32_t launch_raster_edges(const SceneDev& s, const RasterParams& r, uint32_t samples, hipStream_t stream, MarkFn mark, void* ctx, uint64_t raster_bytes, bool has_stroke);

}
```

contrast_renderer_amd/csrc/raster_common.hpp:

```cpp
#pragma once
#include "ga.hpp"
#include "raster_params.hpp"
#include "scene.hpp"
#include "srgb_tables.h"

#ifndef CRH_TILE_WAVES
#define CRH_TILE_WAVES 6
#endif
#ifndef CRH_WALK_WAVES
#define CRH_WALK_WAVES 2
#endif


namespace crh {

constexpr int kTile = 16;
constexpr uint32_t kSortBytesMax = 32u * 1024u;

CRH_D constexpr uint32_t sample_pattern_x(int samples) { return samples == 2 ? 0x4Cu : (samples == 4 ? 0xA2E6u : (samples == 8 ? 0xFB135D79u : 0x8u)); }
CRH_D constexpr uint32_t sample_pattern_y(int samples) { return samples == 2 ? 0x4Cu : (samples == 4 ? 0xEA62u : (samples == 8 ? 0x1F7D39B5u : 0x8u)); }
CRH_D constexpr float sample_dx(int samples, int k) { return (float)((sample_pattern_x(samples) >> (4 * k)) & 15u) * 0.0625f; }
CRH_D constexpr float sample_dy(int samples, int k) { return (float)((sample_pattern_y(samples) >> (4 * k)) & 15u) * 0.0625f; }
CRH_D constexpr float sample_lo(int samples) { return samples == 2 ? 0.25f : (samples == 4 ? 0.125f : (samples == 8 ? 0.0625f : 0.5f)); }
CRH_D constexpr float sample_hi(int samples) { return samples == 2 ? 0.75f : (samples == 4 ? 0.875f : (samples == 8 ? 0.9375f : 0.5f)); }
// ... 8 lines not shown
    const float v[4] = {c0, c1, c2, c3};
    uint32_t out = 0;
#pragma unroll
    for (int ch = 0; ch < 4; ++ch) {
#if defined(__HIP_DEVICE_COMPILE__)
        const float x = __builtin_amdgcn_fmed3f(v[ch], 0.0f, 1.0f);
#else
        const float x = v[ch];
#endif
        out |= (uint32_t)(int)(x * 255.0f + 0.5f) << (8 * ch);
    }
    return out;
}
CRH_D float attachment_unorm8(float v) {
#if defined(__HIP_DEVICE_COMPILE__)
    const float x = __builtin_amdgcn_fmed3f(v, 0.0f, 1.0f);
#else
    const float x = v;
#endif
    return (float)(uint32_t)(int)(x * 255.0f + 0.5f) * (1.0f / 255.0f);
}
CRH_D float clamp_unit(float v) {
    const float x = v > 0.0f ? v : 0.0f;
    return x < 1.0f ? x : 1.0f;
}
CRH_D void store_pixel(const RasterParams& r, uint32_t gx, uint32_t gy, float c0, float c1, float c2, float c3) {
    const size_t at = (size_t)gy * r.width + gx;
    if (r.format == CRH_FORMAT_RGBA16F) {
        float v[4] = {c0, c1, c2, c3};
#pragma unroll
        for (int ch = 0; ch < 4; ++ch) {
            float x = v[ch];
            x = x < 0.0f ? 0.0f : (x > 1.0f ? 1.0f : x);
            if (!(x == x)) x = 0.0f;
            v[ch] = x;
        }
        typedef _Float16 h4 __attribute__((ext_vector_type(4)));
        reinterpret_cast<h4*>(r.rgba8)[at] = h4{(_Float16)v[0], (_Float16)v[1], (_Float16)v[2], (_Float16)v[3]};
    } else {
        reinterpret_cast<uint32_t*>(r.rgba8)[at] = pack_unorm8(c0, c1, c2, c3);
    }
}
CRH_D float4 load_pixel(const RasterParams& r, uint32_t gx, uint32_t gy) {
    const size_t at = (size_t)gy * r.width + gx;
    if (r.format == CRH_FORMAT_RGBA16F) {
        typedef _Float16 h4 __attribute__((ext_vector_type(4)));
        const h4 d = reinterpret_cast<const h4*>(r.rgba8)[at];
        return make_float4((float)d[0], (float)d[1], (float)d[2], (float)d[3]);
    }
    const uchar4 d = reinterpret_cast<const uchar4*>(r.rgba8)[at];
    return make_float4((float)d.x * (1.0f / 255.0f), (float)d.y * (1.0f / 255.0f), (float)d.z * (1.0f / 255.0f), (float)d.w * (1.0f / 255.0f));
}

static __constant__ float kSrgbDecode[256] = CRH_SRGB_DECODE_INIT;
static __constant__ float kSrgbThreshold[257] = CRH_SRGB_THRESHOLD_INIT;
__device__ __forceinline__ bool format_srgb(uint32_t format) { return format - 5u <= 3u; }
__device__ __forceinline__ bool format_bgra(uint32_t format) { return format - 5u > 1u; }
__device__ __forceinline__ bool format_rounds(uint32_t format) { return ((format - 3u) & 1u) != 0u; }
__device__ __forceinline__ float srgb_decode(uint32_t code) { return kSrgbDecode[code]; }
__device__ __forceinline__ uint32_t srgb_encode(float v) {
    const float x = __builtin_amdgcn_fmed3f(v, 0.0f, 1.0f);
    const float s = x <= 0.0031308f ? x * 12.92f : 1.055f * __builtin_amdgcn_exp2f(__builtin_amdgcn_logf(x) * (1.0f / 2.4f)) - 0.055f;
    const int c = (int)__builtin_amdgcn_fmed3f(s * 255.0f + 0.5f, 0.0f, 255.0f);
    return (uint32_t)(c + (int)(x >= kSrgbThreshold[c + 1]) - (int)(x < kSrgbThreshold[c]));
}
__device__ __forceinline__ uint32_t unorm8(float v) { return (uint32_t)(int)(__builtin_amdgcn_fmed3f(v, 0.0f, 1.0f) * 255.0f + 0.5f); }
__device__ __forceinline__ uint32_t pack_pixel_x(uint32_t format, float c0, float c1, float c2, float c3) {
    const bool srgb = format_srgb(format);
    const uint32_t r = srgb ? srgb_encode(c0) : unorm8(c0), g = srgb ? srgb_encode(c1) : unorm8(c1), b = srgb ? srgb_encode(c2) : unorm8(c2);
    const uint32_t a = unorm8(c3) << 24;
    return format_bgra(format) ? (b | g << 8 | r << 16 | a) : (r | g << 8 | b << 16 | a);
}
__device__ __forceinline__ float4 unpack_pixel_x(uint32_t format, uint32_t bits) {
    const uint32_t lo = bits & 255u, mid = (bits >> 8) & 255u, hi = (bits >> 16) & 255u;
    const uint32_t r = format_bgra(format) ? hi : lo, g = mid, b = format_bgra(format) ? lo : hi;
    const float a = (float)(bits >> 24) * (1.0f / 255.0f);
    if (format_srgb(format)) return make_float4(srgb_decode(r), srgb_decode(g), srgb_decode(b), a);
    return make_float4((float)r * (1.0f / 255.0f), (float)g * (1.0f / 255.0f), (float)b * (1.0f / 255.0f), a);
}
__device__ __forceinline__ float attachment_x(uint32_t format, int ch, float v) {
    return (ch < 3 && format_srgb(format)) ? srgb_decode(srgb_encode(v)) : attachment_unorm8(v);
}
template <bool XFMT>
__device__ __forceinline__ void store_px(const RasterParams& r, uint32_t gx, uint32_t gy, float c0, float c1, float c2, float c3) {
    if constexpr (XFMT) reinterpret_cast<uint32_t*>(r.rgba8)[(size_t)gy * r.width + gx] = pack_pixel_x(r.format, c0, c1, c2, c3);
    else store_pixel(r, gx, gy, c0, c1, c2, c3);
}
template <bool XFMT>
__device__ __forceinline__ float4 load_px(const RasterParams& r, uint32_t gx, uint32_t gy) {
    if constexpr (XFMT) return unpack_pixel_x(r.format, reinterpret_cast<const uint32_t*>(r.rgba8)[(size_t)gy * r.width + gx]);
    else return load_pixel(r, gx, gy);
}
template <bool XFMT>
__device__ __forceinline__ uint32_t pack_px(const RasterParams& r, float c0, float c1, float c2, float c3) {
    if constexpr (XFMT) return pack_pixel_x(r.format, c0, c1, c2, c3);
    else return pack_unorm8(c0, c1, c2, c3);
}
template <bool XFMT>
__device__ __forceinline__ bool rounds_writes(const RasterParams& r) {
    if constexpr (XFMT) return format_rounds(r.format);
    else return r.format == CRH_FORMAT_RGBA8_ATTACHMENT;
}
template <bool XFMT>
__device__ __forceinline__ float attachment(const RasterParams& r, int ch, float v) {
    if constexpr (XFMT) return attachment_x(r.format, ch, v);
    else return attachment_unorm8(v);
}

enum : uint32_t { KIND_SOLID = 0, KIND_IQ = 1, KIND_IC = 2, KIND_RQ = 3, KIND_RC = 4, KIND_LINE = 5, KIND_JOINT = 6, KIND_COVER = 7 };

struct PrimCoverage {
    uint32_t flags;
    uint32_t desc;
    ushort4 box;
    float lo_x[3], lo_y[3], bx[3], nay[3];
};
struct PrimFragment {
    float a0[4], gx[4], gy[4];
    float v0x, v0y;
    uint32_t flat_u;
    float end_y;
};
struct PrimRec {
    PrimCoverage cov;
    PrimFragment frag;
};
static_assert(sizeof(PrimCoverage) == 64 && sizeof(PrimFragment) == 64 && sizeof(PrimRec) == 128, "PrimRec");
struct PrimProj {
    float q0, qgx, qgy, z0, zgx, zgy, ax, ay;
};
static_assert(sizeof(PrimProj) == 32, "PrimProj");
constexpr uint32_t kFlagProjective = 1u << 28;

#if defined(__HIP_DEVICE_COMPILE__)
#define CRH_CONST __attribute__((address_space(4)))
#else
#define CRH_CONST
#endif
typedef uint32_t u32x4 __attribute__((ext_vector_type(4)));
typedef float f32x2 __attribute__((ext_vector_type(2)));
CRH_D f32x2 fma2(f32x2 a, f32x2 b, f32x2 c) { return __builtin_elementwise_fma(a, b, c); }
CRH_D f32x2 splat2(float v) { return f32x2{v, v}; }
template <class T>
CRH_D T load_uniform(const T* p) {
    static_assert(sizeof(T) % 16 == 0, "16-byte multiples");
    T out;
    const u32x4 CRH_CONST* src = (const u32x4 CRH_CONST*)p;
    u32x4* dst = reinterpret_cast<u32x4*>(&out);
#pragma unroll
    for (unsigned i = 0; i < sizeof(T) / 16; ++i) dst[i] = src[i];
    return out;
}

CRH_D uint32_t shape_candidates(const SceneDev& s, uint32_t shape, uint32_t c[8]) {
    const uint32_t* b0 = s.shape_base + shape * kShapeRow;
    const uint32_t* b1 = b0 + NCH;
    const uint32_t lvn = b1[CH_LINE_V] - b0[CH_LINE_V], svn = b1[CH_SOLID_V] - b0[CH_SOLID_V], hn = s.hull_count[shape];
    c[0] = lvn >= 3u ? lvn - 2u : 0u;
    c[1] = c[0] + 3u * (b1[CH_JOINT] - b0[CH_JOINT]);
    c[2] = c[1] + (svn >= 3u ? svn - 2u : 0u);
    c[3] = c[2] + (b1[CH_IQ] - b0[CH_IQ]);
    c[4] = c[3] + (b1[CH_IC_V] - b0[CH_IC_V]) / 3u;
    c[5] = c[4] + (b1[CH_RQ] - b0[CH_RQ]);
    c[6] = c[5] + (b1[CH_RC_V] - b0[CH_RC_V]) / 3u;
    c[7] = c[6] + (hn >= 3u ? hn - 2u : 0u);
    return c[7];
}

CRH_D DrawItem item_of(const RasterParams& r, uint32_t i) {
    if (r.items) return r.items[i];
    return DrawItem{i, i, 1u | ((uint32_t)(CRH_OP_COLOR + 1) << 4), 0u};
}
CRH_D void item_candidates(const SceneDev& s, const DrawItem& it, uint32_t cb[8], uint32_t& first, uint32_t& last) {
    shape_candidates(s, it.shape, cb);
    first = (it.ops & 1u) ? 0u : cb[6];
    last = (it.ops >> 4) ? cb[7] : cb[6];
}

CRH_D bool cap_test(float x, float y, uint32_t cap_type) {
    switch (cap_type & 15u) {
        case 0: return y > 0.5f;
        case 1: return x * x + y * y < 0.25f;
        case 2: return 0.5f - y > fabsf(x);
        case 3: return y < fabsf(x);
        case 4: return 0.5f - y > x;
        case 5: return y - 0.5f < x;
        default: return y < 0.0f;
    }
}
CRH_D float wave_uniform(float v) {
#if defined(__HIP_DEVICE_COMPILE__)
    return __uint_as_float(__builtin_amdgcn_readfirstlane(__float_as_uint(v)));
#else
    return v;
#endif
}
CRH_D bool stroke_dashed(const crh_dynamic_stroke_descriptor& d, float tx, float ty) {
    const float ge0 = wave_uniform(d.gap_end[0]), ge1 = wave_uniform(d.gap_end[1]), ge2 = wave_uniform(d.gap_end[2]), ge3 = wave_uniform(d.gap_end[3]);
    const float gs0 = wave_uniform(d.gap_start[0]), gs1 = wave_uniform(d.gap_start[1]), gs2 = wave_uniform(d.gap_start[2]), gs3 = wave_uniform(d.gap_start[3]);
    const uint32_t last = d.count_dashed_join >> 3;
    const float ge_last = last == 0u ? ge0 : (last == 1u ? ge1 : (last == 2u ? ge2 : ge3));
    const float pattern_length = ge_last;
    float position = crh_wgsl_mod(ty - d.phase, pattern_length);
    if (position < 0.0f) position = position + pattern_length;
    const bool a0 = !(ge0 - position >= 0.0f) && 0u < last;
    const bool a1 = a0 && !(ge1 - position >= 0.0f) && 1u < last;
    const bool a2 = a1 && !(ge2 - position >= 0.0f) && 2u < last;
    const uint32_t interval = (uint32_t)a0 + (uint32_t)a1 + (uint32_t)a2;
    const float ge = a2 ? ge3 : (a1 ? ge2 : (a0 ? ge1 : ge0));
    const float gs = a2 ? gs3 : (a1 ? gs2 : (a0 ? gs1 : gs0));
    const float gap_end = ge - position;
    const float gap_start = position - gs;
    if (gap_start > 0.0f) {
        const uint32_t caps = d.caps >> (interval * 8u);
        const bool start_cap = cap_test(tx, gap_start, caps >> 4);
        const bool end_cap = cap_test(tx, gap_end, caps);
        return start_cap || end_cap;
    }
    return true;
}
CRH_D bool stroke_dashed_joint(const crh_dynamic_stroke_descriptor& d, float radius, float a0, float a1, float a2) {
    const float tau = crh_acosf(-1.0f) * 2.0f;
    return stroke_dashed(d, radius, a2 + crh_atan2f(a1, a0) / tau);
}

}
```

contrast_renderer_amd/csrc/tessellate.hip:

```cpp
#include "fill.hpp"
#include "launch.hpp"
#include "paint_angle.hpp"
#include "scene.hpp"
#include "stroke.hpp"

namespace crh {

struct CountSink {
    uint32_t curve_n = 0, solid_n = 0, hull_n = 0;
    CRH_D void curve(float2, const float*) { curve_n += 1; }
    CRH_D void solid(float2) { solid_n += 1; }
    CRH_D void hull(float2) { hull_n += 1; }
};

struct SolidCursor {
    const SceneDev* s;
    uint32_t vertex_base;
    uint32_t index_base;
    uint32_t first_value;
    uint32_t n;
    uint32_t j;
    CRH_D void push(float2 v) {
        const uint32_t pos = (j < ((n + 1) >> 1)) ? 2u * j : 2u * (n - 1u - j) + 1u;
        s->solid_v[vertex_base + pos] = {v.x, v.y};
        s->solid_i[index_base + pos] = (uint16_t)(first_value + pos);
        s->solid_flag[vertex_base + pos] = (uint8_t)((pos & 1u) | (pos + 1u == n ? 2u : 0u));
        j += 1;
    }
};

struct HullCursor {
    const SceneDev* s;
    uint32_t at;
    uint32_t path;
    CRH_D void push(float2 v) {
        if (!is_finite(v.x) || !is_finite(v.y)) raise_error(*s, path, CRH_ERR_NON_FINITE);
        s->hull_cand[at] = {v.x == 0.0f ? 0.0f : v.x, v.y == 0.0f ? 0.0f : v.y};
        at += 1;
    }
};

template <bool RATIONAL>
struct CubicEmitSink {
    SolidCursor solid_cursor;
    HullCursor hull_cursor;
    uint32_t curve_at;
    CRH_D void curve(float2 v, const float* w) {
        if constexpr (RATIONAL)
            solid_cursor.s->rc_v[curve_at] = {v.x, v.y, w[0], w[1], w[2], w[3]};
        else
            solid_cursor.s->ic_v[curve_at] = {v.x, v.y, w[0], w[1], w[2]};
        curve_at += 1;
    }
    CRH_D void solid(float2 v) { solid_cursor.push(v); }
    CRH_D void hull(float2 v) { hull_cursor.push(v); }
};

CRH_D float2 fill_start_point(const SceneDev& s, uint32_t e) {
    const float* q = s.pool + s.elem_off[e - 1u];
    if (s.elem_type[e - 1u] == ELEM_RC) {
        const float w = q[3];
        return make_float2((q[8] * w) / w, (q[9] * w) / w);
    }
    const float* p = s.pool + s.elem_off[e];
    return make_float2(p[-2], p[-1]);
}

CRH_D void load_cubic(const SceneDev& s, uint32_t e, bool rational, Pt cp[4]) {
    const float* p = s.pool + s.elem_off[e];
    const float2 start = fill_start_point(s, e);
    if (rational) {
        cp[0] = weighted_vec_to_point(p[0], start.x, start.y);
        cp[1] = weighted_vec_to_point(p[1], p[4], p[5]);
        cp[2] = weighted_vec_to_point(p[2], p[6], p[7]);
        cp[3] = weighted_vec_to_point(p[3], p[8], p[9]);
    } else {
        cp[0] = vec_to_point(start.x, start.y);
        cp[1] = vec_to_point(p[0], p[1]);
        cp[2] = vec_to_point(p[2], p[3]);
        cp[3] = vec_to_point(p[4], p[5]);
    }
}

CRH_D void count_fill_element(const SceneDev& s, uint32_t e, uint32_t type, uint32_t path, uint32_t cnt[NCH]) {
    switch (type) {
        case ELEM_MOVE:
        case ELEM_LINE:
            cnt[CH_SOLID_V] = 1;
            cnt[CH_HULL] = 1;
            break;
        case ELEM_IQ:
            cnt[CH_SOLID_V] = 1;
            cnt[CH_HULL] = 2;
            cnt[CH_IQ] = 1;
            break;
        case ELEM_RQ:
            cnt[CH_SOLID_V] = 1;
            cnt[CH_HULL] = 2;
            cnt[CH_RQ] = 1;
            break;
        case ELEM_IC:
        case ELEM_RC: {
            Pt cp[4];
            load_cubic(s, e, type == ELEM_RC, cp);
            CountSink sink;
            uint32_t err = 0;
            cubic_fill(cp, type == ELEM_IC, sink, err);
            if (err) raise_error(s, path, err);
            cnt[CH_SOLID_V] = sink.solid_n;
            cnt[CH_HULL] = sink.hull_n;
            cnt[type == ELEM_IC ? CH_IC_V : CH_RC_V] = sink.curve_n;
            break;
        }
        default:
            cnt[CH_SOLID_END] = 1;
            break;
    }
}

template <bool STROKES = true>
CRH_D void count_element(const SceneDev& s, uint32_t e, uint32_t cnt[NCH]) {
    const uint32_t type = s.elem_type[e];
    const uint32_t path = s.elem_path[e];
    const int32_t stroke = STROKES ? s.path_stroke[path] : -1;
    if (!STROKES || stroke < 0)
        count_fill_element(s, e, type, path, cnt);
    else
        count_stroke_element(s, e, type, path, s.stroke_options[stroke], cnt);
}

#ifdef CRH_TESS_WAVES
#define CRH_TESS_OCCUPANCY __attribute__((amdgpu_waves_per_eu(CRH_TESS_WAVES)))
#else
#define CRH_TESS_OCCUPANCY
#endif
__global__ __launch_bounds__(kTessBlock) CRH_TESS_OCCUPANCY void k_count(SceneDev s) {
    __shared__ uint32_t wave_total[kTessBlock / 64][NCH];
    const uint32_t e = blockIdx.x * kTessBlock + threadIdx.x;
    const uint32_t lane = threadIdx.x & 63u, wave = threadIdx.x >> 6;
    uint32_t cnt[NCH];
#pragma unroll
    for (int c = 0; c < NCH; ++c) cnt[c] = 0;
    if (e < s.n_elems) count_element(s, e, cnt);
    uint32_t excl[NCH];
#pragma unroll
    for (int c = 0; c < NCH; ++c) {
        uint32_t v = cnt[c];
#pragma unroll
        for (int d = 1; d < 64; d <<= 1) {
            const uint32_t up = __shfl_up(v, d, 64);
            if (lane >= (uint32_t)d) v += up;
        }
// ... 214 lines not shown
template <bool STROKES, int BLOCK>
__global__ __launch_bounds__(BLOCK) CRH_TESS_OCCUPANCY void k_tess_count_runs(SceneDev s) {
    __shared__ uint32_t wave_total[BLOCK / 64][NCH];
    const uint32_t tid = threadIdx.x, lane = tid & 63u, wave = tid >> 6;
    const uint32_t shape0 = s.tess_run[blockIdx.x], shape1 = s.tess_run[blockIdx.x + 1u];
    const uint32_t first = s.shape_elem_begin[shape0], n = s.shape_elem_begin[shape1] - first;
    const uint32_t e = first + tid;
    uint32_t cnt[NCH];
#pragma unroll
    for (int c = 0; c < NCH; ++c) cnt[c] = 0;
    if (tid < n) {
        count_element<STROKES>(s, e, cnt);
        const uint32_t path = s.elem_path[e];
        bool fits_word;
        s.elem_cnt[e] = pack_counts(cnt, STROKES && s.path_stroke[path] >= 0, fits_word);
        if (!fits_word) raise_error(s, path, CRH_ERR_UNSUPPORTED);
    }
#pragma unroll
    for (int c = 0; c < NCH; ++c) {
        uint32_t v = cnt[c];
#pragma unroll
        for (int d = 32; d > 0; d >>= 1) v += (uint32_t)__shfl_xor((int)v, d, 64);
        if (lane == 0u) wave_total[wave][c] = v;
    }
    __syncthreads();
    if (tid < NCH) {
        uint32_t total = 0;
        for (uint32_t w = 0; w < (uint32_t)BLOCK / 64u; ++w) total += wave_total[w][tid];
        s.run_base[blockIdx.x * NCH + tid] = total;
    }
}

constexpr uint32_t kScanRunsThreads = 64;
__global__ __launch_bounds__(kScanRunsThreads) void k_scan_runs(SceneDev s) {
    const uint32_t lane = threadIdx.x;
    const uint32_t per = (s.n_runs + kScanRunsThreads - 1u) / kScanRunsThreads, first = min(s.n_runs, lane * per), last = min(s.n_runs, first + per);
    uint32_t sum[NCH];
#pragma unroll
    for (int c = 0; c < NCH; ++c) sum[c] = 0u;
    for (uint32_t run = first; run < last; ++run)
#pragma unroll
        for (int c = 0; c < NCH; ++c) sum[c] += s.run_base[run * NCH + c];
    uint32_t begin[NCH], total[NCH];
#pragma unroll
    for (int c = 0; c < NCH; ++c) {
        uint32_t v = sum[c];
#pragma unroll
        for (int d = 1; d < 64; d <<= 1) {
            const uint32_t up = __shfl_up(v, d, 64);
            if (lane >= (uint32_t)d) v += up;
        }
        begin[c] = v - sum[c];
        total[c] = (uint32_t)__shfl((int)v, 63, 64);
    }
    for (uint32_t run = first; run < last; ++run)
#pragma unroll
        for (int c = 0; c < NCH; ++c) {
            const uint32_t mine = s.run_base[run * NCH + c];
            s.run_base[run * NCH + c] = begin[c];
            begin[c] += mine;
        }
    if (lane == 0u) {
#pragma unroll
        for (int c = 0; c < NCH; ++c) s.run_base[s.n_runs * NCH + c] = total[c], s.totals[c] = total[c];
    }
}

template <bool STROKES, int BLOCK>
__global__ __launch_bounds__(BLOCK) CRH_TESS_OCCUPANCY void k_tess_runs(SceneDev s) {
    __shared__ uint32_t rows[(BLOCK + 1) * kScanPitch];
    __shared__ uint32_t wave_total[BLOCK / 64][NCH];
    const uint32_t tid = threadIdx.x, lane = tid & 63u, wave = tid >> 6;
    const uint32_t shape0 = s.tess_run[blockIdx.x], shape1 = s.tess_run[blockIdx.x + 1u];
    const uint32_t first = s.shape_elem_begin[shape0], n = s.shape_elem_begin[shape1] - first;
    const uint32_t e = first + tid;
    const uint32_t* const scene_totals = s.run_base + s.n_runs * NCH;
    if (blockIdx.x == 0u && tid < NCH) s.totals[tid] = scene_totals[tid];
    bool ok = true;
#pragma unroll
    for (int c = 0; c < NCH; ++c) ok = ok && scene_totals[c] <= s.capacity[c];
    if (!ok) {
        if (blockIdx.x == 0u && tid == 0u) raise_error(s, 0, CRH_ERR_UNSUPPORTED + 0x80u);
        return;
    }
    uint32_t type = ELEM_MOVE, path = 0;
    int32_t stroke = -1;
    uint32_t cnt[NCH];
#pragma unroll
    for (int c = 0; c < NCH; ++c) cnt[c] = 0;
    if (tid < n) {
        type = s.elem_type[e], path = s.elem_path[e];
        if (STROKES) stroke = s.path_stroke[path];
        unpack_counts(s.elem_cnt[e], stroke >= 0, cnt);
    }
    uint32_t g[NCH];
#pragma unroll
    for (int c = 0; c < NCH; ++c) {
        uint32_t v = cnt[c];
#pragma unroll
        for (int d = 1; d < 64; d <<= 1) {
            const uint32_t up = __shfl_up(v, d, 64);
            if (lane >= (uint32_t)d) v += up;
        }
        g[c] = v - cnt[c];
        if (lane == 63) wave_total[wave][c] = v;
    }
    __syncthreads();
#pragma unroll
    for (int c = 0; c < NCH; ++c) {
        uint32_t base = s.run_base[blockIdx.x * NCH + c];
#pragma unroll
        for (uint32_t w = 0; w + 1u < (uint32_t)BLOCK / 64u; ++w) base += w < wave ? wave_total[w][c] : 0u;
        g[c] += base;
        if (tid < n) rows[tid * kScanPitch + c] = g[c];
        if (tid == 0u) rows[n * kScanPitch + c] = s.run_base[(blockIdx.x + 1u) * NCH + c];
    }
    __syncthreads();
    for (uint32_t shape = shape0 + tid; shape < shape1; shape += BLOCK) {
        const uint32_t* b0 = rows + (s.shape_elem_begin[shape] - first) * kScanPitch;
        const uint32_t* b1 = rows + (s.shape_elem_begin[shape + 1u] - first) * kScanPitch;
#pragma unroll
        for (int c = 0; c < NCH; ++c) s.shape_base[shape * kShapeRow + c] = b0[c], s.shape_base[shape * kShapeRow + NCH + c] = b1[c];
    }
    if (tid >= n) return;
    const LocalScan scan = {rows, first};
    if (!STROKES || stroke < 0) {
        emit_fill_element(s, e, type, path, g, scan);
    } else {
        if (type == ELEM_MOVE) {
            const uint32_t end = s.path_elem_begin[path + 1u] - 1u;
            s.path_scan[3u * path] = g[CH_LINE_V] >> 1, s.path_scan[3u * path + 1u] = scan(end + 1u, CH_LINE_V) >> 1, s.path_scan[3u * path + 2u] = g[CH_JOINT];
        }
        emit_stroke_element(s, e, type, path, s.stroke_options[stroke], g, scan);
    }
}

#ifndef CRH_ABLATE_HULL
#define CRH_ABLATE_HULL 0
#endif
constexpr uint32_t kHullSmall = 64;
constexpr uint32_t kHullMid = 256;
constexpr uint32_t kHullMax = 2048;
#ifndef CRH_HULL_PACK
#define CRH_HULL_PACK 2
#endif
constexpr uint32_t kHullPack = CRH_HULL_PACK;

CRH_D bool lex_less(float2 a, float2 b) { return a.x < b.x || (a.x == b.x && a.y < b.y); }
CRH_D float turn(float2 a, float2 b, float2 c) { return triple(vec_to_point(a.x, a.y), vec_to_point(b.x, b.y), vec_to_point(c.x, c.y)); }

CRH_D uint32_t fan_to_strip_source(uint32_t i, uint32_t h) { return (i & 1u) == 0 ? (i >> 1) : h - 1u - (i >> 1); }

constexpr uint32_t kHullWaves = 1;
#ifndef CRH_HULL_BATCH
#define CRH_HULL_BATCH 4
#endif
constexpr uint32_t kHullBatch = CRH_HULL_BATCH;
constexpr uint32_t kHullRow = kHullSmall + 1;

template <uint32_t J>
CRH_D float lane_xor(float v, uint32_t lane) {
#if defined(__HIP_DEVICE_COMPILE__)
    const int x = __float_as_int(v);
    if (J == 1) return __int_as_float(__builtin_amdgcn_update_dpp(x, x, 0xB1, 0xF, 0xF, false));
    if (J == 2) return __int_as_float(__builtin_amdgcn_update_dpp(x, x, 0x4E, 0xF, 0xF, false));
    if (J == 8) return __int_as_float(__builtin_amdgcn_update_dpp(x, x, 0x128, 0xF, 0xF, false));
    if (J == 4) {
        const int down = __builtin_amdgcn_update_dpp(x, x, 0x124, 0xF, 0xF, false), up = __builtin_amdgcn_update_dpp(x, x, 0x12C, 0xF, 0xF, false);
        return __int_as_float((lane & 4u) ? down : up);
    }
    return __shfl_xor(v, (int)J, 64);
#else
    (void)lane;
    return v;
#endif
}
template <uint32_t J>
CRH_D void bitonic_step(float2& p, uint32_t lane, uint32_t k) {
    const float2 q = make_float2(lane_xor<J>(p.x, lane), lane_xor<J>(p.y, lane));
    const bool keep_min = ((lane & J) == 0) == ((lane & k) == 0);
    const bool q_less = q.x < p.x || (q.x == p.x && q.y < p.y);
    p = (keep_min == q_less) ? q : p;
}
template <uint32_t K>
CRH_D void bitonic_stage(float2& p, uint32_t lane) {
    if (K >= 64) bitonic_step<32>(p, lane, K);
    if (K >= 32) bitonic_step<16>(p, lane, K);
    if (K >= 16) bitonic_step<8>(p, lane, K);
    if (K >= 8) bitonic_step<4>(p, lane, K);
    if (K >= 4) bitonic_step<2>(p, lane, K);
    bitonic_step<1>(p, lane, K);
}

__global__ __launch_bounds__(256) void k_hull_queues(SceneDev s) {
    __shared__ uint32_t wave_count[4][3], block_base[3];
    if (!fits(s)) return;
    const uint32_t shape = blockIdx.x * 256u + threadIdx.x, lane = threadIdx.x & 63u, wave = threadIdx.x >> 6;
    uint32_t n = 0;
    if (shape < s.n_shapes) n = s.shape_base[shape * kShapeRow + NCH + CH_HULL] - s.shape_base[shape * kShapeRow + CH_HULL];
    const uint32_t queue = n > kHullMax ? 2u : (n > kHullMid ? 1u : (n > kHullSmall ? 0u : 3u));
    unsigned long long members[3];
#pragma unroll
    for (uint32_t q = 0; q < 3u; ++q) {
        members[q] = __ballot(queue == q);
        if (lane == 0u) wave_count[wave][q] = (uint32_t)__popcll(members[q]);
    }
    __syncthreads();
    if (threadIdx.x < 3u) {
        const uint32_t q = threadIdx.x, total = wave_count[0][q] + wave_count[1][q] + wave_count[2][q] + wave_count[3][q];
        block_base[q] = total ? atomicAdd(s.hull_large_count + q, total) : 0u;
    }
    __syncthreads();
    if (queue < 3u) {
        uint32_t at = block_base[queue];
        for (uint32_t w = 0; w < wave; ++w) at += wave_count[w][queue];
        const unsigned long long mine = queue == 0u ? members[0] : (queue == 1u ? members[1] : members[2]);
        at += (uint32_t)__popcll(mine & ((1ull << lane) - 1ull));
        s.hull_large_list[queue * s.n_shapes + at] = shape;
    }
}

__global__ __launch_bounds__(64 * kHullWaves) void k_hull_small(SceneDev s) {
    __shared__ float2 sorted[kHullBatch][kHullRow];
    __shared__ uint8_t stack[kHullBatch][2 * kHullSmall];
    __shared__ uint32_t count[kHullBatch];
    const uint32_t lane = threadIdx.x & 63u, wave = threadIdx.x >> 6;
    if (!fits(s)) return;
    const uint32_t first_shape = blockIdx.x * kHullBatch;
    constexpr uint32_t kPerWave = kHullBatch / kHullWaves;
    uint32_t n_of[kPerWave], base_of[kPerWave];
#pragma unroll
    for (uint32_t u = 0; u < kPerWave; ++u) {
        const uint32_t shape = first_shape + wave + kHullWaves * u;
        n_of[u] = 0;
        base_of[u] = 0;
        if (shape < s.n_shapes) {
            base_of[u] = s.shape_base[shape * kShapeRow + CH_HULL];
            n_of[u] = s.shape_base[shape * kShapeRow + NCH + CH_HULL] - base_of[u];
        }
    }
    const float inf = __uint_as_float(0x7f800000u);
    float2 p_of[kPerWave];
#pragma unroll
    for (uint32_t u = 0; u < kPerWave; ++u) {
        p_of[u] = make_float2(inf, inf);
        if (n_of[u] <= kHullSmall && lane < n_of[u]) p_of[u] = make_float2(s.hull_cand[base_of[u] + lane].x, s.hull_cand[base_of[u] + lane].y);
    }
#pragma unroll
    for (uint32_t u = 0; u < kPerWave; ++u) {
        const uint32_t slot = wave + kHullWaves * u, shape = first_shape + slot;
        uint32_t n = n_of[u];
        if (shape < s.n_shapes) {
            if (n > kHullSmall) {
                n = 0;
            } else if (n == 0) {
                if (lane == 0) s.hull_count[shape] = 0;
            } else {
                float2 p = p_of[u];
                if (n >= 3) {
                    bitonic_stage<2>(p, lane);
                    bitonic_stage<4>(p, lane);
                    bitonic_stage<8>(p, lane);
                    bitonic_stage<16>(p, lane);
                    bitonic_stage<32>(p, lane);
                    bitonic_stage<64>(p, lane);
                }
                sorted[slot][lane] = p;
            }
        }
        if (lane == 0) count[slot] = n;
    }
    __syncthreads();
#if CRH_ABLATE_HULL == 1
    return;
#endif
    if (wave != 0 || lane >= 2u * kHullBatch) return;
    const uint32_t slot = lane >> 1, upper = lane & 1u;
    const uint32_t n = count[slot];
    const uint32_t shape = first_shape + slot;
    if (n == 0) return;
    const float2* pts = sorted[slot];
    uint8_t* chain = stack[slot] + upper * kHullSmall;
    uint32_t m = 0;
    if (n < 3) {
        if (!upper)
            for (uint32_t i = 0; i < n; ++i) chain[i] = (uint8_t)i;
        m = upper ? 1u : n + 1u;
    } else {
        float2 a = make_float2(0.0f, 0.0f), b = a;
        for (uint32_t k = 0; k < n; ++k) {
            const uint32_t i = upper ? n - 1u - k : k;
            const float2 c = pts[i];
            while (m > 1 && turn(a, b, c) <= kErrorMargin) {
                m -= 1;
                b = a;
                if (m >= 2) a = pts[chain[m - 2]];
            }
            chain[m++] = (uint8_t)i;
            a = b;
            b = c;
        }
    }
    const uint32_t ml = (uint32_t)__shfl((int)m, (int)(lane & ~1u), 64) - 1u, mu = (uint32_t)__shfl((int)m, (int)(lane | 1u), 64) - 1u;
    const uint32_t h = ml + mu;
    const uint8_t* lower_chain = stack[slot];
    const uint8_t* upper_chain = stack[slot] + kHullSmall;
    const uint32_t base = s.shape_base[shape * kShapeRow + CH_HULL];
    for (uint32_t i = upper; i < h; i += 2u) {
        const uint32_t c = fan_to_strip_source(i, h);
        const float2 q = pts[c < ml ? lower_chain[c] : upper_chain[c - ml]];
        s.hull_v[base + i] = {q.x, q.y};
    }
    if (!upper) s.hull_count[shape] = h;
}

template <uint32_t CAP, uint32_t QUEUE, uint32_t PACK>
__global__ __launch_bounds__(64) void k_hull_large(SceneDev s) {
    __shared__ float2 pts[PACK][CAP];
    __shared__ uint16_t chain[PACK][2][CAP];
    __shared__ uint32_t chain_m[PACK][2], count[PACK], first_v[PACK], shape_of[PACK];
    if (!fits(s)) return;
    const uint32_t lane = threadIdx.x;
    const uint32_t queued = s.hull_large_count[QUEUE];
    for (uint32_t q0 = blockIdx.x * PACK; q0 < queued; q0 += gridDim.x * PACK) {
        const float inf = __uint_as_float(0x7f800000u);
        for (uint32_t k = 0; k < PACK; ++k) {
            uint32_t n = 0, base = 0, shape = 0;
            if (q0 + k < queued) {
                shape = s.hull_large_list[QUEUE * s.n_shapes + q0 + k];
                base = s.shape_base[shape * kShapeRow + CH_HULL];
                n = s.shape_base[shape * kShapeRow + NCH + CH_HULL] - base;
            }
            if (lane == 0u) count[k] = n, first_v[k] = base, shape_of[k] = shape;
            if (n == 0u) continue;
            uint32_t padded = 1;
            while (padded < n) padded <<= 1;
            float2* const p = pts[k];
            for (uint32_t i = lane; i < padded; i += 64) p[i] = i < n ? make_float2(s.hull_cand[base + i].x, s.hull_cand[base + i].y) : make_float2(inf, inf);
            __syncthreads();
            for (uint32_t kk = 2; kk <= padded; kk <<= 1) {
                for (uint32_t j = kk >> 1; j > 0; j >>= 1) {
                    for (uint32_t i = lane; i < padded; i += 64) {
                        const uint32_t partner = i ^ j;
                        if (partner > i) {
                            const float2 a = p[i], b = p[partner];
                            const bool ascending = (i & kk) == 0;
                            if (ascending ? lex_less(b, a) : lex_less(a, b)) {
                                p[i] = b;
                                p[partner] = a;
                            }
                        }
                    }
                    __syncthreads();
                }
            }
        }
        __syncthreads();
        if (lane < 2u * PACK) {
            const uint32_t k = lane >> 1, upper = lane & 1u, n = count[k];
            const float2* const p = pts[k];
            uint16_t* const mine = chain[k][upper];
            uint32_t m = 0;
            float2 below = make_float2(0.0f, 0.0f), top = make_float2(0.0f, 0.0f);
            for (uint32_t i = 0; i < n; ++i) {
                const uint32_t at = upper ? n - 1u - i : i;
                const float2 c = p[at];
                while (m > 1 && turn(below, top, c) <= kErrorMargin) {
                    m -= 1;
                    top = below;
                    if (m > 1) below = p[mine[m - 2]];
                }
                mine[m++] = (uint16_t)at;
                below = top;
                top = c;
            }
            chain_m[k][upper] = n ? m - 1u : 0u;
        }
        __syncthreads();
        for (uint32_t k = 0; k < PACK; ++k) {
            if (count[k] == 0u) continue;
            const uint32_t ml = chain_m[k][0], h = ml + chain_m[k][1], base = first_v[k];
            for (uint32_t i = lane; i < h; i += 64) {
                const uint32_t c = fan_to_strip_source(i, h);
                const float2 v = pts[k][c < ml ? chain[k][0][c] : chain[k][1][c - ml]];
                s.hull_v[base + i] = {v.x, v.y};
            }
            if (lane == 0) s.hull_count[shape_of[k]] = h;
        }
        __syncthreads();
    }
}

__global__ __launch_bounds__(256) void k_hull_huge(SceneDev s) {
    __shared__ uint32_t chain_n;
    if (!fits(s)) return;
    const uint32_t tid = threadIdx.x;
    const uint32_t queued = s.hull_large_count[2];
    for (uint32_t q = blockIdx.x; q < queued; q += gridDim.x) {
        const uint32_t shape = s.hull_large_list[2u * s.n_shapes + q];
        const uint32_t base = s.shape_base[shape * kShapeRow + CH_HULL];
        const uint32_t n = s.shape_base[shape * kShapeRow + NCH + CH_HULL] - base;
        float2* pts = s.hull_sort + 2u * (size_t)base;
        float2* chain = s.hull_chain + 2u * (size_t)base;
        uint32_t padded = 1;
        while (padded < n) padded <<= 1;
        const float inf = __uint_as_float(0x7f800000u);
        for (uint32_t i = tid; i < padded; i += 256u) pts[i] = i < n ? make_float2(s.hull_cand[base + i].x, s.hull_cand[base + i].y) : make_float2(inf, inf);
        __threadfence_block();
        __syncthreads();
        for (uint32_t k = 2; k <= padded; k <<= 1) {
            for (uint32_t j = k >> 1; j > 0; j >>= 1) {
                for (uint32_t i = tid; i < padded; i += 256u) {
                    const uint32_t partner = i ^ j;
                    if (partner > i) {
                        const float2 a = pts[i], b = pts[partner];
                        const bool ascending = (i & k) == 0;
                        if (ascending ? lex_less(b, a) : lex_less(a, b)) {
                            pts[i] = b;
                            pts[partner] = a;
                        }
                    }
                }
                __threadfence_block();
                __syncthreads();
            }
        }
        if (tid == 0) {
            uint32_t m = 0;
            for (uint32_t i = 0; i < n; ++i) {
                const float2 p = pts[i];
                while (m > 1 && turn(chain[m - 2], chain[m - 1], p) <= kErrorMargin) m -= 1;
                chain[m++] = p;
            }
            m -= 1;
            const uint32_t t = m + 1;
            for (uint32_t i = n; i-- > 0;) {
                const float2 p = pts[i];
                while (m > t && turn(chain[m - 2], chain[m - 1], p) <= kErrorMargin) m -= 1;
                chain[m++] = p;
            }
            m -= 1;
            chain_n = m;
        }
        __threadfence_block();
        __syncthreads();
        const uint32_t h = chain_n;
        for (uint32_t i = tid; i < h; i += 256u) {
            const float2 p = chain[fan_to_strip_source(i, h)];
            s.hull_v[base + i] = {p.x, p.y};
        }
        if (tid == 0) s.hull_count[shape] = h;
        __syncthreads();
    }
}

__global__ void k_fmath(int fn, const float* a, const float* b, float* out, uint64_t n) {
    const uint64_t i = (uint64_t)blockIdx.x * blockDim.x + threadIdx.x;
    if (i >= n) return;
    float s, c;
    switch (fn) {
        case 0: out[i] = crh_atan2f(a[i], b[i]); break;
        case 1: out[i] = crh_acosf(a[i]); break;
        case 2: crh_sincosf(a[i], &s, &c); out[i] = s; break;
        case 3: crh_sincosf(a[i], &s, &c); out[i] = c; break;
        case 4: out[i] = crh_powf(a[i], b[i]); break;
        case 6: out[i] = sqrtf(a[i]); break;
        case 7: out[i] = a[i] / b[i]; break;
        case 8: out[i] = 1.0f / sqrtf(a[i] * a[i] + b[i] * b[i]); break;
        case 9: out[i] = a[i] * b[i] - 4.0f * a[i] * b[i] * b[i]; break;
        case 10: out[i] = paint_turns(a[i], b[i]); break;
        default: out[i] = crh_wgsl_mod(a[i], b[i]); break;
    }
}
void launch_fmath(int fn, const float* a, const float* b, float* out, uint64_t n, hipStream_t stream) {
    hipLaunchKernelGGL(k_fmath, dim3((uint32_t)((n + 255) / 256)), dim3(256), 0, stream, fn, a, b, out, n);
}

void launch_stroke_records(const SceneDev& s, hipStream_t stream, MarkFn mark, void* ctx) {
    if (s.n_elems == 0) return;
    hipLaunchKernelGGL(k_stroke_records, dim3((s.n_paths + 63) / 64), dim3(64), 0, stream, s);
    if (mark) mark(ctx, "stroke_records", 0);
}
CRH_D uint32_t last_not_above(const uint32_t* begin, uint32_t n, uint32_t x) {
    uint32_t lo = 0, hi = n;
    while (hi - lo > 1u) {
        const uint32_t mid = (lo + hi) >> 1;
        if (begin[mid] <= x) lo = mid;
        else hi = mid;
    }
    return lo;
}
__global__ __launch_bounds__(256) void k_upload_build(UploadBuild u) {
    const uint32_t i = blockIdx.x * 256u + threadIdx.x;
    if (i < u.n_segments) {
        const uint32_t g = i;
        const uint32_t p = u.seg_path[g];
        const uint32_t e = g + 2u * p + 1u, from = u.seg_prefix[g], n = u.seg_prefix[g + 1u] - from, off = from + 2u * (p + 1u);
        u.elem_type[e] = u.types[g], u.elem_off[e] = off, u.elem_prev_off[e] = off - 2u, u.elem_path[e] = p;
        if (u.elem_off_again) u.elem_off_again[e] = off;
        for (uint32_t k = 0; k < n; ++k) u.pool[off + k] = u.control[from + k];
    }
    if (i < u.n_paths) {
        const uint32_t p = i, g0 = u.path_seg[p], g1 = u.path_seg[p + 1u];
        const uint32_t e0 = g0 + 2u * p, at0 = u.seg_prefix[g0] + 2u * p, e1 = g1 + 2u * p + 1u, at1 = u.seg_prefix[g1] + 2u * (p + 1u);
        u.elem_type[e0] = ELEM_MOVE, u.elem_off[e0] = at0, u.elem_prev_off[e0] = at0 >= 2u ? at0 - 2u : 0u, u.elem_path[e0] = p;
        u.elem_type[e1] = ELEM_END, u.elem_off[e1] = at1, u.elem_prev_off[e1] = at1 - 2u, u.elem_path[e1] = p;
        if (u.elem_off_again) u.elem_off_again[e0] = at0, u.elem_off_again[e1] = at1;
        u.pool[at0] = u.start[2u * p], u.pool[at0 + 1u] = u.start[2u * p + 1u];
        u.path_elem_begin[p] = e0;
        if (p + 1u == u.n_paths) u.path_elem_begin[u.n_paths] = u.n_elems;
        u.path_shape[p] = last_not_above(u.shape_path, u.n_shapes, p);
    }
    if (i <= u.n_shapes) {
        const uint32_t p0 = i < u.n_shapes ? u.shape_path[i] : u.n_paths;
        u.shape_elem_begin[i] = p0 < u.n_paths ? u.path_seg[p0] + 2u * p0 : u.n_elems;
    }
    if (i == 0u && u.n_paths == 0u) u.path_elem_begin[0] = u.n_elems;
}
void launch_build_elements(const UploadBuild& u, hipStream_t stream) {
    const uint32_t lanes = max(max(u.n_segments, u.n_paths), u.n_shapes + 1u);
    hipLaunchKernelGGL(k_upload_build, dim3((lanes + 255u) / 256u), dim3(256), 0, stream, u);
}

void launch_tessellate(const SceneDev& s, hipStream_t stream, MarkFn mark, void* ctx, const uint64_t bytes[4], bool has_stroke, bool need_totals) {
    if (s.n_elems == 0) return;
    if (has_stroke) launch_stroke_records(s, stream, mark, ctx);
    if (s.n_runs) {
        if (!need_totals) return;
        if (s.run_block == 128u) {
            if (has_stroke) hipLaunchKernelGGL((k_tess_count_runs<true, 128>), dim3(s.n_runs), dim3(128), 0, stream, s);
            else hipLaunchKernelGGL((k_tess_count_runs<false, 128>), dim3(s.n_runs), dim3(128), 0, stream, s);
        } else {
            if (has_stroke) hipLaunchKernelGGL((k_tess_count_runs<true, kTessBlock>), dim3(s.n_runs), dim3(kTessBlock), 0, stream, s);
            else hipLaunchKernelGGL((k_tess_count_runs<false, kTessBlock>), dim3(s.n_runs), dim3(kTessBlock), 0, stream, s);
        }
        if (mark) mark(ctx, "tess_count", bytes[0]);
        hipLaunchKernelGGL(k_scan_runs, dim3(1), dim3(kScanRunsThreads), 0, stream, s);
        if (mark) mark(ctx, "tess_scan", bytes[1]);
        return;
    }
    hipLaunchKernelGGL(k_count, dim3(s.n_wg), dim3(kTessBlock), 0, stream, s);
    if (mark) mark(ctx, "tess_count", bytes[0]);
    hipLaunchKernelGGL(k_scan_rows, dim3((s.n_wg + 63u) / 64u), dim3(64), 0, stream, s);
    hipLaunchKernelGGL(k_scan_groups, dim3(1), dim3(64), 0, stream, s);
    hipLaunchKernelGGL(k_shape_rows, dim3((s.n_shapes + 255u) / 256u), dim3(256), 0, stream, s);
    if (mark) mark(ctx, "tess_scan", bytes[1]);
}
void launch_emit(const SceneDev& s, hipStream_t stream, MarkFn mark, void* ctx, const uint64_t bytes[4], bool has_stroke, bool big_shapes, const uint32_t* hull_queued) {
    if (s.n_elems == 0) return;
    if (s.n_runs) {
        if (s.run_block == 128u) {
            if (has_stroke) hipLaunchKernelGGL((k_tess_runs<true, 128>), dim3(s.n_runs), dim3(128), 0, stream, s);
            else hipLaunchKernelGGL((k_tess_runs<false, 128>), dim3(s.n_runs), dim3(128), 0, stream, s);
        } else {
            if (has_stroke) hipLaunchKernelGGL((k_tess_runs<true, kTessBlock>), dim3(s.n_runs), dim3(kTessBlock), 0, stream, s);
            else hipLaunchKernelGGL((k_tess_runs<false, kTessBlock>), dim3(s.n_runs), dim3(kTessBlock), 0, stream, s);
        }
        if (mark) mark(ctx, "tess_fused", bytes[2]);
    } else {
        hipLaunchKernelGGL(k_emit, dim3(s.n_wg), dim3(kTessBlock), 0, stream, s);
        if (mark) mark(ctx, "tess_emit", bytes[2]);
    }
    if (has_stroke) {
        hipLaunchKernelGGL(k_stroke_lengths, dim3((s.n_paths + 63) / 64), dim3(64), 0, stream, s);
        if (mark) mark(ctx, "stroke_lengths", 0);
    }
    if (has_stroke || big_shapes) {
        (void)hipMemsetAsync(s.hull_large_count, 0, 16, stream);
        hipLaunchKernelGGL(k_hull_queues, dim3((s.n_shapes + 255u) / 256u), dim3(256), 0, stream, s);
    }
    hipLaunchKernelGGL(k_hull_small, dim3((s.n_shapes + kHullBatch - 1u) / kHullBatch), dim3(64 * kHullWaves), 0, stream, s);
    if (mark) mark(ctx, "tess_hull", bytes[3]);
    if (has_stroke || big_shapes) {
        if (!hull_queued || hull_queued[0]) hipLaunchKernelGGL((k_hull_large<kHullMid, 0, kHullPack>), dim3(min(((hull_queued ? hull_queued[0] : s.n_shapes) + kHullPack - 1u) / kHullPack, 16384u)), dim3(64), 0, stream, s);
        if (!hull_queued || hull_queued[1]) hipLaunchKernelGGL((k_hull_large<kHullMax, 1, 1>), dim3(min(hull_queued ? hull_queued[1] : s.n_shapes, 1024u)), dim3(64), 0, stream, s);
        if (!hull_queued || hull_queued[2]) hipLaunchKernelGGL(k_hull_huge, dim3(min(hull_queued ? hull_queued[2] : s.n_shapes, 256u)), dim3(256), 0, stream, s);
        if (mark) mark(ctx, "tess_hull_large", 0);
    }
}

}
```

include/contrast_hip.h:

```cpp
#ifndef CONTRAST_HIP_H
#define CONTRAST_HIP_H

#include <stddef.h>
#include <stdint.h>

#ifdef __cplusplus
extern "C" {
#endif

typedef enum crh_status {
    CRH_OK = 0,
    CRH_ERR_NUMBER_OF_STENCIL_BITS_IS_UNSUPPORTED = 1,
    CRH_ERR_CLIP_STACK_OVERFLOW = 2,
    CRH_ERR_TOO_MANY_NESTED_OPACITY_GROUPS = 3,
    CRH_ERR_TOO_MANY_DASH_INTERVALS = 4,
    CRH_ERR_DYNAMIC_STROKE_OPTIONS_INDEX_OUT_OF_BOUNDS = 5,
    CRH_ERR_NON_FINITE = 6,
    CRH_ERR_DEGENERATE_CUBIC = 7,
    CRH_ERR_UNSUPPORTED = 8,
    CRH_ERR_HIP = 9,
    CRH_ERR_INVALID_ARGUMENT = 10
} crh_status;


// ... 11 lines not shown

typedef struct crh_stroke_options {
    float width;
    float offset;
    float miter_clip;
    uint32_t closed;
    uint32_t dynamic_stroke_options_group;
    uint32_t curve_approximation;
    uint32_t steps;
    float angle_step;
} crh_stroke_options;

typedef struct crh_dash_interval {
    float gap_start;
    float gap_end;
    uint32_t dash_start;
    uint32_t dash_end;
} crh_dash_interval;

typedef struct crh_dynamic_stroke_options {
    uint32_t dashed;
    uint32_t join;
    uint32_t pattern_len;
    crh_dash_interval pattern[CRH_MAX_DASH_INTERVALS];
    float phase;
    uint32_t start;
    uint32_t end;
} crh_dynamic_stroke_options;

typedef struct crh_dynamic_stroke_descriptor {
    float gap_start[CRH_MAX_DASH_INTERVALS];
    float gap_end[CRH_MAX_DASH_INTERVALS];
    uint32_t caps;
    uint32_t count_dashed_join;
    float phase;
    uint32_t _padding;
} crh_dynamic_stroke_descriptor;

typedef struct crh_path_batch {
    uint32_t n_shapes;
    const uint32_t* shape_path_begin;
    uint32_t n_paths;
    const uint32_t* path_segment_begin;
    const float* path_start;
    const int32_t* path_stroke_options;
    uint32_t n_segments;
    const uint8_t* segment_types;
    const float* control_data;
    uint32_t n_control_floats;
    uint32_t n_stroke_options;
    const crh_stroke_options* stroke_options;
    const uint32_t* shape_dynamic_begin;
    uint32_t n_dynamic_stroke_options;
    const crh_dynamic_stroke_options* dynamic_stroke_options;
} crh_path_batch;


typedef enum crh_cull { CRH_CULL_NONE = 0, CRH_CULL_FRONT = 1, CRH_CULL_BACK = 2 } crh_cull;
typedef enum crh_compare {
    CRH_COMPARE_ALWAYS = 0,
    CRH_COMPARE_NEVER = 1,
    CRH_COMPARE_LESS = 2,
    CRH_COMPARE_EQUAL = 3,
    CRH_COMPARE_LESS_EQUAL = 4,
    CRH_COMPARE_GREATER = 5,
    CRH_COMPARE_NOT_EQUAL = 6,
    CRH_COMPARE_GREATER_EQUAL = 7
} crh_compare;
typedef struct crh_config {
    uint32_t msaa_sample_count;
    uint32_t clip_nesting_counter_bits;
    uint32_t winding_counter_bits;
    uint32_t alpha_layer_count;
    uint32_t cull_mode;
    uint32_t depth_compare;
    uint32_t depth_write_enabled;
} crh_config;

typedef struct crh_renderer crh_renderer;
typedef struct crh_scene crh_scene;
typedef struct crh_frame crh_frame;

typedef enum crh_render_op {
    CRH_OP_STENCIL = 0,
    CRH_OP_CLIP = 1,
    CRH_OP_UNCLIP = 2,
    CRH_OP_COLOR = 3,
    CRH_OP_SAVE_ALPHA_CONTEXT = 4,
    CRH_OP_SCALE_ALPHA_CONTEXT = 5,
    CRH_OP_RESTORE_ALPHA_CONTEXT = 6
} crh_render_op;

crh_status crh_renderer_create(const crh_config* config, int device_ordinal, crh_renderer** out);
void crh_renderer_destroy(crh_renderer* renderer);
crh_status crh_renderer_get_config(const crh_renderer* renderer, crh_config* out);

typedef enum crh_blend_factor {
    CRH_BLEND_ZERO = 0,
    CRH_BLEND_ONE = 1,
    CRH_BLEND_SRC = 2,
    CRH_BLEND_ONE_MINUS_SRC = 3,
    CRH_BLEND_SRC_ALPHA = 4,
    CRH_BLEND_ONE_MINUS_SRC_ALPHA = 5,
    CRH_BLEND_DST = 6,
    CRH_BLEND_ONE_MINUS_DST = 7,
    CRH_BLEND_DST_ALPHA = 8,
    CRH_BLEND_ONE_MINUS_DST_ALPHA = 9,
    CRH_BLEND_SRC_ALPHA_SATURATED = 10,
    CRH_BLEND_CONSTANT = 11,
    CRH_BLEND_ONE_MINUS_CONSTANT = 12,
    CRH_BLEND_SRC1 = 13,
    CRH_BLEND_ONE_MINUS_SRC1 = 14,
    CRH_BLEND_SRC1_ALPHA = 15,
    CRH_BLEND_ONE_MINUS_SRC1_ALPHA = 16
} crh_blend_factor;
typedef enum crh_blend_operation {
    CRH_BLEND_OP_ADD = 0,
    CRH_BLEND_OP_SUBTRACT = 1,
    CRH_BLEND_OP_REVERSE_SUBTRACT = 2,
    CRH_BLEND_OP_MIN = 3,
    CRH_BLEND_OP_MAX = 4
} crh_blend_operation;
typedef struct crh_blend_component {
    uint32_t src_factor;
    uint32_t dst_factor;
    uint32_t operation;
} crh_blend_component;
enum { CRH_COLOR_WRITE_RED = 1, CRH_COLOR_WRITE_GREEN = 2, CRH_COLOR_WRITE_BLUE = 4, CRH_COLOR_WRITE_ALPHA = 8, CRH_COLOR_WRITE_ALL = 15 };
typedef struct crh_color_target_state {
    uint32_t blend_enabled;
    crh_blend_component color;
    crh_blend_component alpha;
    uint32_t write_mask;
    float constant[4];
} crh_color_target_state;
crh_status crh_renderer_create_blended(const crh_config* config, const crh_color_target_state* blending, int device_ordinal, crh_renderer** out);
crh_status crh_renderer_get_blending(const crh_renderer* renderer, crh_color_target_state* out);

crh_status crh_convert_dynamic_stroke_options(const crh_dynamic_stroke_options* options, crh_dynamic_stroke_descriptor* out);


crh_status crh_scene_upload(crh_renderer* renderer, const crh_path_batch* batch, crh_scene* existing, crh_scene** out);
crh_status crh_scene_tessellate(crh_scene* scene);
crh_status crh_scene_status(crh_scene* scene);
void crh_scene_destroy(crh_scene* scene);

crh_status crh_shape_from_paths(crh_renderer* renderer, const crh_path_batch* one_shape, crh_scene* existing, crh_scene** out);

crh_status crh_scene_shape_layout(crh_scene* scene, uint32_t shape_index, uint64_t vertex_offsets[8], uint64_t index_offsets[3]);
crh_status crh_scene_shape_download(crh_scene* scene, uint32_t shape_index, void* vertex_bytes, void* index_bytes);
crh_status crh_scene_layout_all(crh_scene* scene, uint64_t* layout , uint64_t* total_vertex_bytes, uint64_t* total_index_bytes);
crh_status crh_scene_download_all(crh_scene* scene, void* vertex_bytes, void* index_bytes);
crh_status crh_scene_traffic(crh_scene* scene, uint64_t* bytes_read, uint64_t* bytes_written);

crh_status crh_scene_set_dynamic_stroke_options(crh_scene* scene, uint32_t shape_index, uint32_t group_index, const crh_dynamic_stroke_options* options);


crh_status crh_frame_create(crh_renderer* renderer, uint32_t width, uint32_t height, crh_frame** out);
enum {
    CRH_FORMAT_RGBA8 = 0,
    CRH_FORMAT_RGBA16F = 1,
    CRH_FORMAT_RGBA8_ATTACHMENT = 2,
    CRH_FORMAT_BGRA8 = 3,
    CRH_FORMAT_BGRA8_ATTACHMENT = 4,
    CRH_FORMAT_RGBA8_SRGB = 5,
    CRH_FORMAT_RGBA8_SRGB_ATTACHMENT = 6,
    CRH_FORMAT_BGRA8_SRGB = 7,
    CRH_FORMAT_BGRA8_SRGB_ATTACHMENT = 8
};
crh_status crh_frame_create_format(crh_renderer* renderer, uint32_t width, uint32_t height, uint32_t format, crh_frame** out);
crh_status crh_frame_format(const crh_frame* frame, uint32_t* format);
void crh_frame_destroy(crh_frame* frame);
crh_status crh_frame_clear(crh_frame* frame);
crh_status crh_frame_keep_pass_state(crh_frame* frame);
crh_status crh_frame_clear_depth(crh_frame* frame, float value);
crh_status crh_frame_upload_depth(crh_frame* frame, const float* depth);
crh_status crh_frame_download_depth(crh_frame* frame, float* depth_samples);

crh_status crh_scene_render(crh_scene* scene, crh_frame* frame, const float* transforms, const float* colors);
crh_status crh_scene_set_instances(crh_scene* scene, const float* transforms, const float* colors);
crh_status crh_scene_render_resident(crh_scene* scene, crh_frame* frame);

typedef struct crh_draw {
    uint32_t shape;
    uint32_t instance;
    uint32_t op;
    uint32_t clip_depth;
    uint32_t alpha_layer;
} crh_draw;
crh_status crh_scene_render_draws(crh_scene* scene, crh_frame* frame, const float* transforms, const float* colors, uint32_t n_instances,
                                  const crh_draw* draws, uint32_t n_draws);

#define CRH_MAX_GRADIENT_STOPS 8
typedef enum crh_paint_kind { CRH_PAINT_LINEAR = 1, CRH_PAINT_RADIAL = 2, CRH_PAINT_CONIC = 4 } crh_paint_kind;
typedef enum crh_spread { CRH_SPREAD_PAD = 0, CRH_SPREAD_REPEAT = 1, CRH_SPREAD_REFLECT = 2 } crh_spread;
typedef struct crh_gradient_stop {
    float offset;
    float color[4];
} crh_gradient_stop;
typedef struct crh_paint {
    uint32_t kind, spread;
    float p0[2], p1[2];
    uint32_t n_stops;
    crh_gradient_stop stops[CRH_MAX_GRADIENT_STOPS];
} crh_paint;
crh_status crh_paint_validate(const crh_paint* paint);
crh_status crh_scene_set_paints(crh_scene* scene, const crh_paint* paints, uint32_t n_paints, const int32_t* instance_paint, uint32_t n_instances);

typedef struct crh_image crh_image;
enum { CRH_FILTER_NEAREST = 0, CRH_FILTER_LINEAR = 1, CRH_FILTER_MIPMAP = 0x100  };
crh_status crh_image_create(crh_renderer* renderer, uint32_t width, uint32_t height, const void* rgba8, crh_image** out);
crh_status crh_image_create_from_frame(crh_frame* frame, crh_image** out);
crh_status crh_image_size(const crh_image* image, uint32_t* width, uint32_t* height);
void crh_image_destroy(crh_image* image);
crh_status crh_image_generate_mipmaps(crh_image* image);
crh_status crh_image_level_count(const crh_image* image, uint32_t* count);
crh_status crh_image_download_level(const crh_image* image, uint32_t level, void* rgba8, uint32_t* width, uint32_t* height);
#define CRH_MAX_BLUR_SIGMA 64.0f
#define CRH_MAX_BLUR_RADIUS 192u
typedef enum crh_blur_edge {
    CRH_BLUR_EDGE_TRANSPARENT = 0,
    CRH_BLUR_EDGE_PAD = 1,
    CRH_BLUR_EDGE_REPEAT = 2,
    CRH_BLUR_EDGE_REFLECT = 3
} crh_blur_edge;
crh_status crh_blur_taps(float sigma, uint32_t* taps, uint32_t capacity, uint32_t* radius);
crh_status crh_image_blur(const crh_image* src, float sigma_x, float sigma_y, uint32_t edge, crh_image** out);
typedef enum crh_composite_op {
    CRH_COMPOSITE_CLEAR = 0,
    CRH_COMPOSITE_COPY = 1,
    CRH_COMPOSITE_DST = 2,
    CRH_COMPOSITE_SRC_OVER = 3,
    CRH_COMPOSITE_DST_OVER = 4,
    CRH_COMPOSITE_SRC_IN = 5,
    CRH_COMPOSITE_DST_IN = 6,
    CRH_COMPOSITE_SRC_OUT = 7,
    CRH_COMPOSITE_DST_OUT = 8,
    CRH_COMPOSITE_SRC_ATOP = 9,
    CRH_COMPOSITE_DST_ATOP = 10,
    CRH_COMPOSITE_XOR = 11,
    CRH_COMPOSITE_PLUS = 12
} crh_composite_op;
typedef enum crh_blend_mode {
    CRH_BLEND_NORMAL = 0,
    CRH_BLEND_MULTIPLY = 1,
    CRH_BLEND_SCREEN = 2,
    CRH_BLEND_OVERLAY = 3,
    CRH_BLEND_DARKEN = 4,
    CRH_BLEND_LIGHTEN = 5,
    CRH_BLEND_HARD_LIGHT = 6,
    CRH_BLEND_DIFFERENCE = 7,
    CRH_BLEND_EXCLUSION = 8
} crh_blend_mode;
typedef struct crh_composite {
    uint32_t op, mode;
    float opacity;
    int32_t x, y;
} crh_composite;
crh_status crh_composite_validate(const crh_composite* how);
crh_status crh_composite_texels(const crh_composite* how, const void* source_rgba8, const void* backdrop_rgba8, uint64_t n, void* out_rgba8);
crh_status crh_image_composite(const crh_image* backdrop, const crh_image* source, const crh_composite* how, crh_image** out);
#define CRH_COLOR_MATRIX_MAX 16.0f
crh_status crh_color_filter_validate(const float* matrix, const uint8_t* tables);
crh_status crh_color_filter_texels(const float* matrix, const uint8_t* tables, const void* rgba8, uint64_t n, void* out);
crh_status crh_image_color_filter(const crh_image* src, const float* matrix, const uint8_t* tables, crh_image** out);
#define CRH_MAX_MORPHOLOGY_RADIUS 192u
typedef enum crh_morphology_op {
    CRH_MORPHOLOGY_ERODE = 0,
    CRH_MORPHOLOGY_DILATE = 1
} crh_morphology_op;
crh_status crh_morphology_size(uint32_t width, uint32_t height, uint32_t op, uint32_t radius_x, uint32_t radius_y, uint32_t edge, uint32_t* out_width,
                               uint32_t* out_height);
crh_status crh_morphology_texels(uint32_t width, uint32_t height, const void* rgba8, uint32_t op, uint32_t radius_x, uint32_t radius_y, uint32_t edge,
                                 void* out_rgba8);
crh_status crh_image_morphology(const crh_image* src, uint32_t op, uint32_t radius_x, uint32_t radius_y, uint32_t edge, crh_image** out);
#define CRH_MAX_CONVOLVE_ORDER 15u
#define CRH_CONVOLVE_MAX_GAIN 64.0f
typedef struct crh_convolve {
    uint32_t order_x, order_y;
    uint32_t target_x, target_y;
    const float* kernel;
    float divisor;
    float bias;
    uint32_t edge;
    uint32_t preserve_alpha;
} crh_convolve;
crh_status crh_convolve_validate(const crh_convolve* how);
crh_status crh_convolve_coefficients(const crh_convolve* how, int32_t* k, uint32_t capacity, int32_t* bias_k);
crh_status crh_convolve_texels(uint32_t width, uint32_t height, const void* rgba8, const crh_convolve* how, void* out_rgba8);
crh_status crh_image_convolve(const crh_image* src, const crh_convolve* how, crh_image** out);
typedef enum crh_lighting_op { CRH_LIGHTING_DIFFUSE = 0, CRH_LIGHTING_SPECULAR = 1 } crh_lighting_op;
typedef enum crh_light_kind { CRH_LIGHT_DISTANT = 0, CRH_LIGHT_POINT = 1, CRH_LIGHT_SPOT = 2 } crh_light_kind;
typedef struct crh_lighting {
    uint32_t op, light, edge;
    float surface_scale;
    float constant;
    float specular_exponent;
    float color[3];
    float azimuth, elevation;
    float position[3];
    float points_at[3];
    float spot_exponent;
    float cone_angle;
} crh_lighting;
crh_status crh_lighting_validate(const crh_lighting* how);
crh_status crh_lighting_texels(uint32_t width, uint32_t height, const void* rgba8, const crh_lighting* how, void* out_rgba8);
// ... 127 lines not shown
```

rust/contrast_renderer_hip/src/ffi.rs:

```rust
#![allow(non_camel_case_types, non_upper_case_globals, dead_code)]
use std::os::raw::{c_char, c_int, c_void};

pub type crh_status = u32;
pub type crh_cull = u32;
pub type crh_compare = u32;
pub type crh_render_op = u32;

pub const CRH_MAX_DASH_INTERVALS: usize = 4;
pub const CRH_MAX_GRADIENT_STOPS: usize = 8;
pub const CRH_MAX_BLUR_SIGMA: usize = 64;
pub const CRH_MAX_BLUR_RADIUS: usize = 192;
pub const CRH_COLOR_MATRIX_MAX: usize = 16;
pub const CRH_MAX_MORPHOLOGY_RADIUS: usize = 192;
pub const CRH_MAX_CONVOLVE_ORDER: usize = 15;
pub const CRH_CONVOLVE_MAX_GAIN: usize = 64;
pub const CRH_MAX_TURBULENCE_OCTAVES: usize = 12;
pub const CRH_TURBULENCE_MAX_FREQUENCY: usize = 4;
pub const CRH_TURBULENCE_MAX_OFFSET: usize = 65536;
pub const CRH_MAX_DISPLACE_SCALE: usize = 1024;
pub const CRH_COMM_ID_BYTES: usize = 128;
pub const CRH_COMM_PHASES: usize = 6;

pub const CRH_OK: u32 = 0;
pub const CRH_ERR_NUMBER_OF_STENCIL_BITS_IS_UNSUPPORTED: u32 = 1;
// ... 267 lines not shown
}
#[repr(C)]
#[derive(Clone, Copy)]
pub struct crh_color_target_state {
    pub blend_enabled: u32,
    pub color: crh_blend_component,
    pub alpha: crh_blend_component,
    pub write_mask: u32,
    pub constant: [f32; 4],
}
#[repr(C)]
#[derive(Clone, Copy)]
pub struct crh_draw {
    pub shape: u32,
    pub instance: u32,
    pub op: u32,
    pub clip_depth: u32,
    pub alpha_layer: u32,
}
#[repr(C)]
#[derive(Clone, Copy)]
pub struct crh_gradient_stop {
    pub offset: f32,
    pub color: [f32; 4],
}
#[repr(C)]
#[derive(Clone, Copy)]
pub struct crh_paint {
    pub kind: u32,
    pub spread: u32,
    pub p0: [f32; 2],
    pub p1: [f32; 2],
    pub n_stops: u32,
    pub stops: [crh_gradient_stop; 8],
}
#[repr(C)]
#[derive(Clone, Copy)]
pub struct crh_composite {
    pub op: u32,
    pub mode: u32,
    pub opacity: f32,
    pub x: i32,
    pub y: i32,
}
#[repr(C)]
#[derive(Clone, Copy)]
pub struct crh_convolve {
    pub order_x: u32,
    pub order_y: u32,
    pub target_x: u32,
    pub target_y: u32,
    pub kernel: *const f32,
    pub divisor: f32,
    pub bias: f32,
    pub edge: u32,
    pub preserve_alpha: u32,
}
#[repr(C)]
#[derive(Clone, Copy)]
pub struct crh_lighting {
    pub op: u32,
    pub light: u32,
    pub edge: u32,
    pub surface_scale: f32,
    pub constant: f32,
    pub specular_exponent: f32,
    pub color: [f32; 3],
    pub azimuth: f32,
    pub elevation: f32,
    pub position: [f32; 3],
    pub points_at: [f32; 3],
    pub spot_exponent: f32,
    pub cone_angle: f32,
}
#[repr(C)]
#[derive(Clone, Copy)]
pub struct crh_turbulence {
    pub kind: u32,
    pub octaves: u32,
    pub seed: i32,
    pub stitch: u32,
    pub opaque: u32,
    pub base_frequency: [f32; 2],
    pub offset: [f32; 2],
}
#[repr(C)]
#[derive(Clone, Copy)]
pub struct crh_displace {
    pub scale: [f32; 2],
    pub x_channel: u32,
    pub y_channel: u32,
    pub filter: u32,
    pub edge: u32,
}
#[repr(C)]
#[derive(Clone, Copy)]
pub struct crh_image_paint {
    pub image: *const crh_image,
    pub filter: u32,
    pub spread_x: u32,
    pub spread_y: u32,
    pub m: [f32; 6],
}
#[repr(C)]
#[derive(Clone, Copy)]
pub struct crh_kernel_time {
    pub name: [c_char; 48],
    pub ms: f32,
    pub algorithmic_bytes: u64,
}
#[repr(C)]
#[derive(Clone, Copy)]
pub struct crh_font_metrics {
    pub units_per_em: u32,
    pub number_of_glyphs: u32,
    pub ascender: i32,
    pub descender: i32,
    pub line_gap: i32,
    pub height: i32,
    pub has_x_height: i32,
    pub x_height: i32,
    pub has_vertical_metrics: i32,
    pub vertical_height: i32,
    pub vertical_line_gap: i32,
    pub has_kerning: i32,
}
#[repr(C)]
#[derive(Clone, Copy)]
pub struct crh_text_layout {
    pub size: f32,
    pub orientation: u32,
    pub major_alignment: u32,
    pub minor_alignment: u32,
}

#[link(name = "contrast_hip")]
extern "C" {
    pub fn crh_renderer_create(config: *const crh_config, device_ordinal: c_int, out: *mut *mut crh_renderer) -> crh_status;
    pub fn crh_renderer_destroy(renderer: *mut crh_renderer);
    pub fn crh_renderer_get_config(renderer: *const crh_renderer, out: *mut crh_config) -> crh_status;
    pub fn crh_renderer_create_blended(config: *const crh_config, blending: *const crh_color_target_state, device_ordinal: c_int, out: *mut *mut crh_renderer) -> crh_status;
    pub fn crh_renderer_get_blending(renderer: *const crh_renderer, out: *mut crh_color_target_state) -> crh_status;
    pub fn crh_convert_dynamic_stroke_options(options: *const crh_dynamic_stroke_options, out: *mut crh_dynamic_stroke_descriptor) -> crh_status;
    pub fn crh_scene_upload(renderer: *mut crh_renderer, batch: *const crh_path_batch, existing: *mut crh_scene, out: *mut *mut crh_scene) -> crh_status;
    pub fn crh_scene_tessellate(scene: *mut crh_scene) -> crh_status;
    pub fn crh_scene_status(scene: *mut crh_scene) -> crh_status;
    pub fn crh_scene_destroy(scene: *mut crh_scene);
    pub fn crh_shape_from_paths(renderer: *mut crh_renderer, one_shape: *const crh_path_batch, existing: *mut crh_scene, out: *mut *mut crh_scene) -> crh_status;
    pub fn crh_scene_shape_layout(scene: *mut crh_scene, shape_index: u32, vertex_offsets: *mut u64, index_offsets: *mut u64) -> crh_status;
    pub fn crh_scene_shape_download(scene: *mut crh_scene, shape_index: u32, vertex_bytes: *mut c_void, index_bytes: *mut c_void) -> crh_status;
    pub fn crh_scene_layout_all(scene: *mut crh_scene, layout: *mut u64, total_vertex_bytes: *mut u64, total_index_bytes: *mut u64) -> crh_status;
    pub fn crh_scene_download_all(scene: *mut crh_scene, vertex_bytes: *mut c_void, index_bytes: *mut c_void) -> crh_status;
    pub fn crh_scene_traffic(scene: *mut crh_scene, bytes_read: *mut u64, bytes_written: *mut u64) -> crh_status;
    pub fn crh_scene_set_dynamic_stroke_options(scene: *mut crh_scene, shape_index: u32, group_index: u32, options: *const crh_dynamic_stroke_options) -> crh_status;
    pub fn crh_frame_create(renderer: *mut crh_renderer, width: u32, height: u32, out: *mut *mut crh_frame) -> crh_status;
    pub fn crh_frame_create_format(renderer: *mut crh_renderer, width: u32, height: u32, format: u32, out: *mut *mut crh_frame) -> crh_status;
    pub fn crh_frame_format(frame: *const crh_frame, format: *mut u32) -> crh_status;
    pub fn crh_frame_destroy(frame: *mut crh_frame);
    pub fn crh_frame_clear(frame: *mut crh_frame) -> crh_status;
    pub fn crh_frame_keep_pass_state(frame: *mut crh_frame) -> crh_status;
    pub fn crh_frame_clear_depth(frame: *mut crh_frame, value: f32) -> crh_status;
    pub fn crh_frame_upload_depth(frame: *mut crh_frame, depth: *const f32) -> crh_status;
    pub fn crh_frame_download_depth(frame: *mut crh_frame, depth_samples: *mut f32) -> crh_status;
    pub fn crh_scene_render(scene: *mut crh_scene, frame: *mut crh_frame, transforms: *const f32, colors: *const f32) -> crh_status;
    pub fn crh_scene_set_instances(scene: *mut crh_scene, transforms: *const f32, colors: *const f32) -> crh_status;
    pub fn crh_scene_render_resident(scene: *mut crh_scene, frame: *mut crh_frame) -> crh_status;
    pub fn crh_scene_render_draws(scene: *mut crh_scene, frame: *mut crh_frame, transforms: *const f32, colors: *const f32, n_instances: u32, draws: *const crh_draw, n_draws: u32) -> crh_status;
    pub fn crh_paint_validate(paint: *const crh_paint) -> crh_status;
    pub fn crh_scene_set_paints(scene: *mut crh_scene, paints: *const crh_paint, n_paints: u32, instance_paint: *const i32, n_instances: u32) -> crh_status;
    pub fn crh_image_create(renderer: *mut crh_renderer, width: u32, height: u32, rgba8: *const c_void, out: *mut *mut crh_image) -> crh_status;
    pub fn crh_image_create_from_frame(frame: *mut crh_frame, out: *mut *mut crh_image) -> crh_status;
    pub fn crh_image_size(image: *const crh_image, width: *mut u32, height: *mut u32) -> crh_status;
    pub fn crh_image_destroy(image: *mut crh_image);
    pub fn crh_image_generate_mipmaps(image: *mut crh_image) -> crh_status;
    pub fn crh_image_level_count(image: *const crh_image, count: *mut u32) -> crh_status;
    pub fn crh_image_download_level(image: *const crh_image, level: u32, rgba8: *mut c_void, width: *mut u32, height: *mut u32) -> crh_status;
    pub fn crh_blur_taps(sigma: f32, taps: *mut u32, capacity: u32, radius: *mut u32) -> crh_status;
    pub fn crh_image_blur(src: *const crh_image, sigma_x: f32, sigma_y: f32, edge: u32, out: *mut *mut crh_image) -> crh_status;
    pub fn crh_composite_validate(how: *const crh_composite) -> crh_status;
    pub fn crh_composite_texels(how: *const crh_composite, source_rgba8: *const c_void, backdrop_rgba8: *const c_void, n: u64, out_rgba8: *mut c_void) -> crh_status;
    pub fn crh_image_composite(backdrop: *const crh_image, source: *const crh_image, how: *const crh_composite, out: *mut *mut crh_image) -> crh_status;
    pub fn crh_color_filter_validate(matrix: *const f32, tables: *const u8) -> crh_status;
    pub fn crh_color_filter_texels(matrix: *const f32, tables: *const u8, rgba8: *const c_void, n: u64, out: *mut c_void) -> crh_status;
    pub fn crh_image_color_filter(src: *const crh_image, matrix: *const f32, tables: *const u8, out: *mut *mut crh_image) -> crh_status;
    pub fn crh_morphology_size(width: u32, height: u32, op: u32, radius_x: u32, radius_y: u32, edge: u32, out_width: *mut u32, out_height: *mut u32) -> crh_status;
    pub fn crh_morphology_texels(width: u32, height: u32, rgba8: *const c_void, op: u32, radius_x: u32, radius_y: u32, edge: u32, out_rgba8: *mut c_void) -> crh_status;
    pub fn crh_image_morphology(src: *const crh_image, op: u32, radius_x: u32, radius_y: u32, edge: u32, out: *mut *mut crh_image) -> crh_status;
    pub fn crh_convolve_validate(how: *const crh_convolve) -> crh_status;
    pub fn crh_convolve_coefficients(how: *const crh_convolve, k: *mut i32, capacity: u32, bias_k: *mut i32) -> crh_status;
    pub fn crh_convolve_texels(width: u32, height: u32, rgba8: *const c_void, how: *const crh_convolve, out_rgba8: *mut c_void) -> crh_status;
    pub fn crh_image_convolve(src: *const crh_image, how: *const crh_convolve, out: *mut *mut crh_image) -> crh_status;
    pub fn crh_lighting_validate(how: *const crh_lighting) -> crh_status;
    pub fn crh_lighting_texels(width: u32, height: u32, rgba8: *const c_void, how: *const crh_lighting, out_rgba8: *mut c_void) -> crh_status;
    pub fn crh_image_lighting(src: *const crh_image, how: *const crh_lighting, out: *mut *mut crh_image) -> crh_status;
    pub fn crh_turbulence_validate(how: *const crh_turbulence) -> crh_status;
    pub fn crh_turbulence_tables(seed: i32, lattice: *mut u8, gradient: *mut f64) -> crh_status;
    pub fn crh_turbulence_texels(width: u32, height: u32, how: *const crh_turbulence, out_rgba8: *mut c_void) -> crh_status;
    pub fn crh_image_turbulence(renderer: *mut crh_renderer, width: u32, height: u32, how: *const crh_turbulence, out: *mut *mut crh_image) -> crh_status;
    pub fn crh_displace_validate(how: *const crh_displace) -> crh_status;
    pub fn crh_displace_offset(how: *const crh_displace, code_x: u32, code_y: u32, q: *mut i32) -> crh_status;
    pub fn crh_displace_texels(width: u32, height: u32, rgba8: *const c_void, map_rgba8: *const c_void, how: *const crh_displace, out_rgba8: *mut c_void) -> crh_status;
    pub fn crh_image_displace(src: *const crh_image, map: *const crh_image, how: *const crh_displace, out: *mut *mut crh_image) -> crh_status;
    pub fn crh_image_paint_validate(paint: *const crh_image_paint) -> crh_status;
    pub fn crh_scene_set_paints_with_images(scene: *mut crh_scene, paints: *const crh_paint, n_paints: u32, image_paints: *const crh_image_paint, n_image_paints: u32, instance_paint: *const i32, n_instances: u32) -> crh_status;
    pub fn crh_frame_upload(frame: *mut crh_frame, rgba8: *const c_void) -> crh_status;
    pub fn crh_frame_load_image(frame: *mut crh_frame, image: *const crh_image) -> crh_status;
    pub fn crh_frame_download(frame: *mut crh_frame, rgba8: *mut c_void) -> crh_status;
    pub fn crh_frame_download_f16(frame: *mut crh_frame, rgba16f: *mut c_void) -> crh_status;
    pub fn crh_frame_device_pointer(frame: *mut crh_frame, rgba8_dev: *mut *mut c_void) -> crh_status;
    pub fn crh_composite_over(renderer: *mut crh_renderer, layers_dev: *const *const c_void, n_layers: u32, n_pixels: u64, dst_dev: *mut c_void) -> crh_status;
    pub fn crh_renderer_synchronize(renderer: *mut crh_renderer) -> crh_status;
    pub fn crh_frame_synchronize(frame: *mut crh_frame) -> crh_status;
    pub fn crh_renderer_stream(renderer: *mut crh_renderer) -> *mut c_void;
    pub fn crh_renderer_enable_timing(renderer: *mut crh_renderer, enabled: c_int) -> crh_status;
    pub fn crh_renderer_kernel_times(renderer: *mut crh_renderer, out: *mut crh_kernel_time, capacity: u32, count: *mut u32) -> crh_status;
    pub fn crh_selftest_fmath(renderer: *mut crh_renderer, fn_: c_int, a: *const f32, b: *const f32, out: *mut f32, n: u64) -> crh_status;
    pub fn crh_selftest_srgb(renderer: *mut crh_renderer, x: *const f32, codes: *mut u8, n: u64, decoded: *mut f32) -> crh_status;
    pub fn crh_font_create(ttf_bytes: *const c_void, n_bytes: usize, out: *mut *mut crh_font) -> crh_status;
    pub fn crh_font_destroy(font: *mut crh_font);
    pub fn crh_font_get_metrics(font: *const crh_font, out: *mut crh_font_metrics) -> crh_status;
    pub fn crh_font_glyph_index(font: *const crh_font, code_point: u32, glyph_id: *mut u16, found: *mut u32) -> crh_status;
    pub fn crh_font_glyph_advance(font: *const crh_font, glyph_id: u16, vertical: u32, advance: *mut u16, found: *mut u32) -> crh_status;
    pub fn crh_font_glyph_bounding_box(font: *const crh_font, glyph_id: u16, box_: *mut i16, found: *mut u32) -> crh_status;
    pub fn crh_font_glyphs_kerning(font: *const crh_font, left: u16, right: u16, kerning: *mut i16, found: *mut u32) -> crh_status;
    pub fn crh_paths_of_glyph(font: *const crh_font, glyph_id: u16, out: *mut *mut crh_path_list) -> crh_status;
    pub fn crh_paths_of_text(font: *const crh_font, layout: *const crh_text_layout, text: *const u32, n_chars: usize, clipping_area: *const f32, n_clip: usize, out: *mut *mut crh_path_list) -> crh_status;
    pub fn crh_text_aligned_positions(font: *const crh_font, layout: *const crh_text_layout, text: *const u32, n_chars: usize, extent: *mut i64, offset: *mut i64, positions: *mut i64, line_ends: *mut u64, line_lengths: *mut u64, n_lines: *mut u64) -> crh_status;
    pub fn crh_path_elliptical_arc(from: *const f32, half_extent: *const f32, rotation: f32, large_arc: u32, sweep: u32, to: *const f32, records: *mut f32, capacity: u32, n_segments: *mut u32, is_line: *mut u32) -> crh_status;
    pub fn crh_path_list_transform(list: *mut crh_path_list, scale: f32, motor: *const f32) -> crh_status;
    pub fn crh_path_list_view(list: *const crh_path_list, out: *mut crh_path_batch) -> crh_status;
    pub fn crh_path_list_destroy(list: *mut crh_path_list);
    pub fn crh_comm_shard(n_items: u32, rank: u32, world: u32, begin: *mut u32, end: *mut u32) -> crh_status;
    pub fn crh_comm_slab_rows(height: u32, rank: u32, world: u32, row_begin: *mut u32, row_end: *mut u32) -> crh_status;
    pub fn crh_comm_unique_id(id128: *mut c_void) -> crh_status;
    pub fn crh_comm_create(renderer: *mut crh_renderer, rank: u32, world: u32, id128: *const c_void, out: *mut *mut crh_comm) -> crh_status;
    pub fn crh_comm_destroy(comm: *mut crh_comm);
    pub fn crh_frame_exchange(comm: *mut crh_comm, layer: *mut crh_frame, result: *mut crh_frame) -> crh_status;
    pub fn crh_frame_set_tile_rows(frame: *mut crh_frame, row_begin: u32, row_end: u32) -> crh_status;
    pub fn crh_frame_gather_slabs(comm: *mut crh_comm, layer: *mut crh_frame, result: *mut crh_frame) -> crh_status;
    pub fn crh_comm_last_traffic(comm: *const crh_comm, bytes_sent: *mut u64, bytes_dense: *mut u64) -> crh_status;
    pub fn crh_comm_last_timing(comm: *mut crh_comm, ms: *mut f32) -> crh_status;
    pub fn crh_comm_last_peer_bytes(comm: *const crh_comm, per_peer: *mut u64) -> crh_status;
    pub fn crh_comm_info(comm: *const crh_comm, nranks: *mut u32, rccl_version: *mut i32) -> crh_status;
    pub fn crh_comm_create_local(renderer: *mut crh_renderer, rank: u32, world: u32, rank0: *mut crh_comm, out: *mut *mut crh_comm) -> crh_status;
    pub fn crh_comm_local_exchange(rank0: *mut crh_comm, layers: *const *mut crh_frame, result: *mut crh_frame) -> crh_status;
    pub fn crh_comm_local_gather_slabs(rank0: *mut crh_comm, layers: *const *mut crh_frame, result: *mut crh_frame) -> crh_status;
    pub fn crh_last_error() -> *const c_char;
    pub fn crh_version() -> *const c_char;
}
```

Baseline: 42.91 million.

## Fuse per-shape range counts into hull kernel and single-pass scan

```diff
diff --git a/contrast_renderer_amd/_ffi.py b/contrast_renderer_amd/_ffi.py
--- a/contrast_renderer_amd/_ffi.py
+++ b/contrast_renderer_amd/_ffi.py
@@ -287,6 +287,7 @@
         "crh_scene_layout_all": (C.c_int, [V, C.POINTER(C.c_uint64), C.POINTER(C.c_uint64), C.POINTER(C.c_uint64)]),
         "crh_scene_download_all": (C.c_int, [V, V, V]),
         "crh_scene_traffic": (C.c_int, [V, C.POINTER(C.c_uint64), C.POINTER(C.c_uint64)]),
+        "crh_debug_scene_ranges": (C.c_int, [V, C.POINTER(C.c_uint32), C.POINTER(C.c_uint32), C.POINTER(C.c_uint32), C.POINTER(C.c_uint32)]),
         "crh_scene_set_dynamic_stroke_options": (C.c_int, [V, C.c_uint32, C.c_uint32, C.POINTER(DynamicStrokeOptionsC)]),
         "crh_frame_create": (C.c_int, [V, C.c_uint32, C.c_uint32, C.POINTER(V)]),
         "crh_frame_create_format": (C.c_int, [V, C.c_uint32, C.c_uint32, C.c_uint32, C.POINTER(V)]),
diff --git a/contrast_renderer_amd/csrc/api.hip b/contrast_renderer_amd/csrc/api.hip
--- a/contrast_renderer_amd/csrc/api.hip
+++ b/contrast_renderer_amd/csrc/api.hip
@@ -642,7 +642,13 @@
     if (sc->has_stroke) HIP_TRY(hipMemsetAsync(d.line_pair_cut, 0, sc->line_pair_cut.cap, ts));
     const uint64_t bytes2[4] = {sc->input_bytes, 0, sc->input_bytes + sc->emitted_bytes, (uint64_t)sc->totals_host[CH_HULL] * 8};
     if (sc->hull_queued_state == 1 && hipEventQuery(sc->hull_queued_ready) == hipSuccess) sc->hull_queued_state = 2;
-    launch_emit(d, ts, r->mark_fn_tess(), r, bytes2, sc->has_stroke, sc->big_shapes, sc->hull_queued_state == 2 ? sc->hull_queued_host : nullptr);
+    const size_t scan_words = (size_t)(d.n_shapes + 511) / 512 + 2;
+    const ShapeCounts counts = {sc->shape_ncand.as<uint32_t>(), sc->shape_nslots.as<uint32_t>(), sc->prim_scan_scratch.as<uint32_t>() + 2 * scan_words};
+    const RangesRoute ranges_route = getenv("CRH_RANGES_UNFUSED") != nullptr ? kRangesUnfused
+                                     : ((sc->has_stroke || sc->big_shapes || d.n_elems == 0 || d.n_runs == 0 || d.n_shapes == 0) ? kRangesCounted : kRangesFromHulls);
+    const bool wait_for_ranges = sc->rendered_once && !sc->last_render_one_event;
+    if (wait_for_ranges && ranges_route == kRangesFromHulls) HIP_TRY(hipStreamWaitEvent(ts, sc->ranges_free, 0));
+    launch_emit(d, ts, r->mark_fn_tess(), r, bytes2, sc->has_stroke, sc->big_shapes, sc->hull_queued_state == 2 ? sc->hull_queued_host : nullptr, ranges_route == kRangesFromHulls ? &counts : nullptr);
     if (sc->hull_queued_state == 0 && (sc->has_stroke || sc->big_shapes)) {
         if (!sc->hull_queued_host) HIP_TRY(hipHostMalloc(reinterpret_cast<void**>(&sc->hull_queued_host), 16, hipHostMallocDefault));
         if (!sc->hull_queued_ready) HIP_TRY(hipEventCreateWithFlags(&sc->hull_queued_ready, hipEventDisableTiming));
@@ -650,9 +656,9 @@
         HIP_TRY(hipEventRecord(sc->hull_queued_ready, ts));
         sc->hull_queued_state = 1;
     }
-    if (sc->rendered_once && !sc->last_render_one_event) HIP_TRY(hipStreamWaitEvent(ts, sc->ranges_free, 0));
-    launch_plain_ranges(d, sc->shape_ncand.as<uint32_t>(), sc->shape_prim_begin.as<uint32_t>(), sc->shape_nslots.as<uint32_t>(), sc->shape_slot_begin.as<uint32_t>(),
-                        sc->prim_scan_scratch.as<uint32_t>(), sc->prim_scan_scratch.as<uint32_t>() + ((size_t)(d.n_shapes + 511) / 512 + 2), ts);
+    if (wait_for_ranges && ranges_route != kRangesFromHulls) HIP_TRY(hipStreamWaitEvent(ts, sc->ranges_free, 0));
+    launch_plain_ranges(d, counts, sc->shape_prim_begin.as<uint32_t>(), sc->shape_slot_begin.as<uint32_t>(), sc->prim_scan_scratch.as<uint32_t>(), sc->prim_scan_scratch.as<uint32_t>() + scan_words,
+                        ranges_route, ts);
     if (r->timing & 2u) crh_renderer::mark_cb_tess(r, "tess_prim_ranges", 0);
     HIP_TRY(hipEventRecord(sc->tess_done, ts));
     HIP_TRY(hipGetLastError());
@@ -1916,7 +1922,7 @@
         !hip_ok(sc->transforms.ensure((size_t)b->n_shapes * 64), "hipMalloc") || !hip_ok(sc->colors.ensure((size_t)b->n_shapes * 16), "hipMalloc") ||
         !hip_ok(sc->shape_ncand.ensure((size_t)b->n_shapes * 4 + 4), "hipMalloc") || !hip_ok(sc->shape_prim_begin.ensure(((size_t)b->n_shapes + 1) * 4), "hipMalloc") ||
         !hip_ok(sc->shape_nslots.ensure((size_t)b->n_shapes * 4 + 4), "hipMalloc") || !hip_ok(sc->shape_slot_begin.ensure(((size_t)b->n_shapes + 1) * 4), "hipMalloc") ||
-        !hip_ok(sc->prim_scan_scratch.ensure(((size_t)(b->n_shapes + 511) / 512 + 2) * 8), "hipMalloc")) {
+        !hip_ok(sc->prim_scan_scratch.ensure(((size_t)(b->n_shapes + 511) / 512 + 2) * 8 + (size_t)shape_partial_words(b->n_shapes) * 4 + 8), "hipMalloc")) {
         rc = CRH_ERR_HIP;
         goto fail;
     }
@@ -2061,6 +2067,17 @@
     if (!sc) return CRH_ERR_INVALID_ARGUMENT;
     if (bytes_read) *bytes_read = sc->input_bytes;
     if (bytes_written) *bytes_written = sc->emitted_bytes;
+    return CRH_OK;
+}
+crh_status crh_debug_scene_ranges(crh_scene* sc, uint32_t* ncand, uint32_t* prim_begin, uint32_t* nslots, uint32_t* slot_begin) {
+    if (!sc || !ncand || !prim_begin || !nslots || !slot_begin || !sc->tessellated_once) return CRH_ERR_INVALID_ARGUMENT;
+    HIP_TRY(hipSetDevice(sc->renderer->device));
+    HIP_TRY(sc->renderer->sync());
+    const size_t n = sc->d.n_shapes;
+    if (n) HIP_TRY(hipMemcpy(ncand, sc->shape_ncand.p, n * 4, hipMemcpyDeviceToHost));
+    HIP_TRY(hipMemcpy(prim_begin, sc->shape_prim_begin.p, (n + 1) * 4, hipMemcpyDeviceToHost));
+    if (n) HIP_TRY(hipMemcpy(nslots, sc->shape_nslots.p, n * 4, hipMemcpyDeviceToHost));
+    HIP_TRY(hipMemcpy(slot_begin, sc->shape_slot_begin.p, (n + 1) * 4, hipMemcpyDeviceToHost));
     return CRH_OK;
 }
 crh_status crh_scene_set_dynamic_stroke_options(crh_scene* sc, uint32_t shape, uint32_t group, const crh_dynamic_stroke_options* o) {
diff --git a/contrast_renderer_amd/csrc/bin_edges.hip b/contrast_renderer_amd/csrc/bin_edges.hip
--- a/contrast_renderer_amd/csrc/bin_edges.hip
+++ b/contrast_renderer_amd/csrc/bin_edges.hip
@@ -1892,13 +1892,19 @@
     hipLaunchKernelGGL(k_item_nslots, dim3((n_items + 255u) / 256u), dim3(256), 0, stream, s, r, n_items, item_nslots);
     launch_scan_u32(item_nslots, slot_begin, scratch, n_items, stream);
 }
-__global__ __launch_bounds__(64) void k_shape_counts(SceneDev s, uint32_t* shape_ncand, uint32_t* shape_nslots) {
+__global__ __launch_bounds__(64) void k_shape_counts(SceneDev s, ShapeCounts out) {
     const uint32_t shape = blockIdx.x * 64u + threadIdx.x;
-    if (shape >= s.n_shapes) return;
-    uint32_t c[8];
-    shape_ncand[shape] = shape_candidates(s, shape, c);
-    RasterParams plain = {};
-    shape_nslots[shape] = item_slots(s, item_of(plain, shape)).total;
+    uint32_t ncand = 0, nslots = 0;
+    if (shape < s.n_shapes) {
+        uint32_t c[8];
+        out.ncand[shape] = ncand = shape_candidates(s, shape, c);
+        RasterParams plain = {};
+        out.nslots[shape] = nslots = item_slots(s, item_of(plain, shape)).total;
+    }
+    if (!out.partial) return;
+#pragma unroll
+    for (int d = 32; d > 0; d >>= 1) ncand += (uint32_t)__shfl_xor((int)ncand, d, 64), nslots += (uint32_t)__shfl_xor((int)nslots, d, 64);
+    if (threadIdx.x == 0u) out.partial[2u * blockIdx.x] = ncand, out.partial[2u * blockIdx.x + 1u] = nslots;
 }
 struct WaveScan {
     const uint32_t* in;
@@ -1939,17 +1945,48 @@
         if (i0 + k < n) j.out[i0 + k] += sum;
     if (blockIdx.x + 1u == blocks && lane == 0u) j.out[n] = sum + j.block_sum[blockIdx.x];
 }
-void launch_plain_ranges(const SceneDev& s, uint32_t* shape_ncand, uint32_t* shape_prim_begin, uint32_t* shape_nslots, uint32_t* shape_slot_begin, uint32_t* scratch0, uint32_t* scratch1, hipStream_t stream) {
+__global__ __launch_bounds__(64) void k_shape_ranges(WaveScan a, WaveScan b, uint32_t n, const uint32_t* partial, uint32_t per_partial) {
+    const WaveScan j = blockIdx.y ? b : a;
+    const uint32_t lane = threadIdx.x, i0 = blockIdx.x * kWaveScanBlock + lane * kWaveScanItems;
+    uint32_t v[kWaveScanItems], mine = 0;
+#pragma unroll
+    for (uint32_t k = 0; k < kWaveScanItems; ++k) v[k] = i0 + k < n ? j.in[i0 + k] : 0u, mine += v[k];
+    uint32_t before = 0;
+    const uint32_t in_front = blockIdx.x * (kWaveScanBlock / per_partial);
+    for (uint32_t g = lane; g < in_front; g += 64u) before += partial[2u * g + blockIdx.y];
+#pragma unroll
+    for (int d = 32; d > 0; d >>= 1) before += (uint32_t)__shfl_xor((int)before, d, 64);
+    uint32_t incl = mine;
+#pragma unroll
+    for (int d = 1; d < 64; d <<= 1) {
+        const uint32_t up = __shfl_up(incl, d, 64);
+        if (lane >= (uint32_t)d) incl += up;
+    }
+    uint32_t run = before + incl - mine;
+#pragma unroll
+    for (uint32_t k = 0; k < kWaveScanItems; ++k) {
+        if (i0 + k < n) j.out[i0 + k] = run;
+        run += v[k];
+    }
+    if (blockIdx.x + 1u == gridDim.x && lane == 63u) j.out[n] = before + incl;
+}
+static_assert(kWaveScanBlock % kHullBatch == 0u && kWaveScanBlock % 64u == 0u, "a block of k_shape_ranges begins where a partial sum does");
+void launch_plain_ranges(const SceneDev& s, const ShapeCounts& counts, uint32_t* shape_prim_begin, uint32_t* shape_slot_begin, uint32_t* scratch0, uint32_t* scratch1, RangesRoute route, hipStream_t stream) {
     if (s.n_shapes == 0) {
         (void)hipMemsetAsync(shape_prim_begin, 0, 4, stream);
         (void)hipMemsetAsync(shape_slot_begin, 0, 4, stream);
         return;
     }
-    hipLaunchKernelGGL(k_shape_counts, dim3((s.n_shapes + 63u) / 64u), dim3(64), 0, stream, s, shape_ncand, shape_nslots);
     const uint32_t blocks = (s.n_shapes + kWaveScanBlock - 1u) / kWaveScanBlock;
-    const WaveScan a = {shape_ncand, shape_prim_begin, scratch0}, b = {shape_nslots, shape_slot_begin, scratch1};
-    hipLaunchKernelGGL(k_wave_scan_local2, dim3(blocks, 2), dim3(64), 0, stream, a, b, s.n_shapes);
-    hipLaunchKernelGGL(k_wave_scan_add2, dim3(blocks, 2), dim3(64), 0, stream, a, b, s.n_shapes, blocks);
+    const WaveScan a = {counts.ncand, shape_prim_begin, scratch0}, b = {counts.nslots, shape_slot_begin, scratch1};
+    if (route == kRangesUnfused) {
+        hipLaunchKernelGGL(k_shape_counts, dim3((s.n_shapes + 63u) / 64u), dim3(64), 0, stream, s, ShapeCounts{counts.ncand, counts.nslots, nullptr});
+        hipLaunchKernelGGL(k_wave_scan_local2, dim3(blocks, 2), dim3(64), 0, stream, a, b, s.n_shapes);
+        hipLaunchKernelGGL(k_wave_scan_add2, dim3(blocks, 2), dim3(64), 0, stream, a, b, s.n_shapes, blocks);
+        return;
+    }
+    if (route == kRangesCounted) hipLaunchKernelGGL(k_shape_counts, dim3((s.n_shapes + 63u) / 64u), dim3(64), 0, stream, s, counts);
+    hipLaunchKernelGGL(k_shape_ranges, dim3(blocks, 2), dim3(64), 0, stream, a, b, s.n_shapes, counts.partial, route == kRangesFromHulls ? kHullBatch : 64u);
 }
 uint32_t flat_threads_for(uint32_t n_items) {
     if (const char* e = getenv("CRH_BIN_FLAT_THREADS")) return atoi(e) == 64 ? 64u : kFlatThreads;
diff --git a/contrast_renderer_amd/csrc/edge_slots.hpp b/contrast_renderer_amd/csrc/edge_slots.hpp
--- a/contrast_renderer_amd/csrc/edge_slots.hpp
+++ b/contrast_renderer_amd/csrc/edge_slots.hpp
@@ -22,12 +22,11 @@
     uint32_t fe0, synth_a, hull0, synth_b, total;
     uint32_t cb[8];
 };
-CRH_D ItemSlots item_slots(const SceneDev& s, const DrawItem& it) {
+CRH_D ItemSlots item_slots(const SceneDev& s, const DrawItem& it, uint32_t hn) {
     ItemSlots k;
-    shape_candidates(s, it.shape, k.cb);
+    shape_candidates(s, it.shape, k.cb, hn);
     const uint32_t* b0 = s.shape_base + it.shape * kShapeRow;
     const bool stencil = (it.ops & 1u) != 0u, cover = (it.ops >> 4) != 0u;
-    const uint32_t hn = s.hull_count[it.shape];
     k.n_tri = stencil ? k.cb[1] + (k.cb[6] - k.cb[2]) : 0u;
     k.n_fe = stencil ? b0[NCH + CH_SOLID_V] - b0[CH_SOLID_V] : 0u;
     k.n_hull = (cover && hn >= 3u) ? hn : 0u;
@@ -38,5 +37,6 @@
     k.total = k.synth_b + 28u;
     return k;
 }
+CRH_D ItemSlots item_slots(const SceneDev& s, const DrawItem& it) { return item_slots(s, it, s.hull_count[it.shape]); }
 
 }
diff --git a/contrast_renderer_amd/csrc/launch.hpp b/contrast_renderer_amd/csrc/launch.hpp
--- a/contrast_renderer_amd/csrc/launch.hpp
+++ b/contrast_renderer_amd/csrc/launch.hpp
@@ -11,7 +11,18 @@
 typedef void (*MarkFn)(void*, const char*, uint64_t);
 
 void launch_tessellate(const SceneDev& s, hipStream_t stream, MarkFn mark, void* ctx, const uint64_t bytes[4], bool has_stroke, bool need_totals);
-void launch_emit(const SceneDev& s, hipStream_t stream, MarkFn mark, void* ctx, const uint64_t bytes[4], bool has_stroke, bool big_shapes, const uint32_t* hull_queued);
+struct ShapeCounts {
+    uint32_t* ncand;
+    uint32_t* nslots;
+    uint32_t* partial;
+};
+#ifndef CRH_HULL_BATCH
+#define CRH_HULL_BATCH 4
+#endif
+constexpr uint32_t kHullBatch = CRH_HULL_BATCH;
+static_assert(kHullBatch != 0u && (kHullBatch & (kHullBatch - 1u)) == 0u && kHullBatch <= 32u, "k_hull_small sums its Shapes' counts over 2 * kHullBatch lanes, and a scan block of 512 Shapes begins at a partial sum's first Shape");
+constexpr uint32_t shape_partial_words(uint32_t n_shapes) { return 2u * ((n_shapes + kHullBatch - 1u) / kHullBatch); }
+void launch_emit(const SceneDev& s, hipStream_t stream, MarkFn mark, void* ctx, const uint64_t bytes[4], bool has_stroke, bool big_shapes, const uint32_t* hull_queued, const ShapeCounts* counts);
 void launch_build_elements(const UploadBuild& u, hipStream_t stream);
 void launch_fmath(int fn, const float* a, const float* b, float* out, uint64_t n, hipStream_t stream);
 
@@ -58,7 +69,8 @@
 void launch_scatter(const RasterParams& r, hipStream_t stream, MarkFn mark, void* ctx);
 void launch_shape_bounds(const SceneDev& s, float* bounds, hipStream_t stream);
 void launch_slab_items(const RasterParams& r, uint8_t* elsewhere, hipStream_t stream);
-void launch_plain_ranges(const SceneDev& s, uint32_t* shape_ncand, uint32_t* shape_prim_begin, uint32_t* shape_nslots, uint32_t* shape_slot_begin, uint32_t* scratch0, uint32_t* scratch1, hipStream_t stream);
+enum RangesRoute : uint32_t { kRangesUnfused = 0, kRangesCounted = 1, kRangesFromHulls = 2 };
+void launch_plain_ranges(const SceneDev& s, const ShapeCounts& counts, uint32_t* shape_prim_begin, uint32_t* shape_slot_begin, uint32_t* scratch0, uint32_t* scratch1, RangesRoute route, hipStream_t stream);
 bool bin_itemwise(const RasterParams& r);
 void flat_batches(const uint32_t* cost, uint32_t n_items, std::vector<uint32_t>& runs);
 void flat_batch_limits(uint32_t n_items, uint32_t limits[4]);
diff --git a/contrast_renderer_amd/csrc/raster_common.hpp b/contrast_renderer_amd/csrc/raster_common.hpp
--- a/contrast_renderer_amd/csrc/raster_common.hpp
+++ b/contrast_renderer_amd/csrc/raster_common.hpp
@@ -184,10 +184,10 @@
     return out;
 }
 
-CRH_D uint32_t shape_candidates(const SceneDev& s, uint32_t shape, uint32_t c[8]) {
+CRH_D uint32_t shape_candidates(const SceneDev& s, uint32_t shape, uint32_t c[8], uint32_t hn) {
     const uint32_t* b0 = s.shape_base + shape * kShapeRow;
     const uint32_t* b1 = b0 + NCH;
-    const uint32_t lvn = b1[CH_LINE_V] - b0[CH_LINE_V], svn = b1[CH_SOLID_V] - b0[CH_SOLID_V], hn = s.hull_count[shape];
+    const uint32_t lvn = b1[CH_LINE_V] - b0[CH_LINE_V], svn = b1[CH_SOLID_V] - b0[CH_SOLID_V];
     c[0] = lvn >= 3u ? lvn - 2u : 0u;
     c[1] = c[0] + 3u * (b1[CH_JOINT] - b0[CH_JOINT]);
     c[2] = c[1] + (svn >= 3u ? svn - 2u : 0u);
@@ -198,6 +198,7 @@
     c[7] = c[6] + (hn >= 3u ? hn - 2u : 0u);
     return c[7];
 }
+CRH_D uint32_t shape_candidates(const SceneDev& s, uint32_t shape, uint32_t c[8]) { return shape_candidates(s, shape, c, s.hull_count[shape]); }
 
 CRH_D DrawItem item_of(const RasterParams& r, uint32_t i) {
     if (r.items) return r.items[i];
diff --git a/contrast_renderer_amd/csrc/tessellate.hip b/contrast_renderer_amd/csrc/tessellate.hip
--- a/contrast_renderer_amd/csrc/tessellate.hip
+++ b/contrast_renderer_amd/csrc/tessellate.hip
@@ -1,3 +1,4 @@
+#include "edge_slots.hpp"
 #include "fill.hpp"
 #include "launch.hpp"
 #include "paint_angle.hpp"
@@ -518,10 +519,6 @@
 CRH_D uint32_t fan_to_strip_source(uint32_t i, uint32_t h) { return (i & 1u) == 0 ? (i >> 1) : h - 1u - (i >> 1); }
 
 constexpr uint32_t kHullWaves = 1;
-#ifndef CRH_HULL_BATCH
-#define CRH_HULL_BATCH 4
-#endif
-constexpr uint32_t kHullBatch = CRH_HULL_BATCH;
 constexpr uint32_t kHullRow = kHullSmall + 1;
 
 template <uint32_t J>
@@ -586,13 +583,35 @@
     }
 }
 
-__global__ __launch_bounds__(64 * kHullWaves) void k_hull_small(SceneDev s) {
+CRH_D void hull_small_counts(const SceneDev& s, const ShapeCounts& out, uint32_t first_shape, uint32_t lane, uint32_t h) {
+    const uint32_t shape = first_shape + (lane >> 1);
+    uint32_t ncand = 0, nslots = 0;
+    if ((lane & 1u) == 0u && shape < s.n_shapes) {
+        uint32_t c[8];
+        ncand = shape_candidates(s, shape, c, h);
+        RasterParams plain = {};
+        nslots = item_slots(s, item_of(plain, shape), h).total;
+        out.ncand[shape] = ncand;
+        out.nslots[shape] = nslots;
+    }
+#pragma unroll
+    for (uint32_t d = 1; d < 2u * kHullBatch; d <<= 1) {
+        ncand += (uint32_t)__shfl_xor((int)ncand, (int)d, 64);
+        nslots += (uint32_t)__shfl_xor((int)nslots, (int)d, 64);
+    }
+    if (lane == 0u) out.partial[2u * blockIdx.x] = ncand, out.partial[2u * blockIdx.x + 1u] = nslots;
+}
+
+__global__ __launch_bounds__(64 * kHullWaves) void k_hull_small(SceneDev s, ShapeCounts out) {
     __shared__ float2 sorted[kHullBatch][kHullRow];
     __shared__ uint8_t stack[kHullBatch][2 * kHullSmall];
     __shared__ uint32_t count[kHullBatch];
     const uint32_t lane = threadIdx.x & 63u, wave = threadIdx.x >> 6;
-    if (!fits(s)) return;
     const uint32_t first_shape = blockIdx.x * kHullBatch;
+    if (!fits(s)) {
+        if (out.ncand && wave == 0u && lane < 2u * kHullBatch) hull_small_counts(s, out, first_shape, lane, 0u);
+        return;
+    }
     constexpr uint32_t kPerWave = kHullBatch / kHullWaves;
     uint32_t n_of[kPerWave], base_of[kPerWave];
 #pragma unroll
@@ -637,47 +656,51 @@
         if (lane == 0) count[slot] = n;
     }
     __syncthreads();
-#if CRH_ABLATE_HULL == 1
-    return;
-#endif
     if (wave != 0 || lane >= 2u * kHullBatch) return;
     const uint32_t slot = lane >> 1, upper = lane & 1u;
+    const uint32_t shape = first_shape + slot;
+#if CRH_ABLATE_HULL == 1
+    const uint32_t n = 0;
+#else
     const uint32_t n = count[slot];
-    const uint32_t shape = first_shape + slot;
-    if (n == 0) return;
-    const float2* pts = sorted[slot];
-    uint8_t* chain = stack[slot] + upper * kHullSmall;
-    uint32_t m = 0;
-    if (n < 3) {
-        if (!upper)
-            for (uint32_t i = 0; i < n; ++i) chain[i] = (uint8_t)i;
-        m = upper ? 1u : n + 1u;
-    } else {
-        float2 a = make_float2(0.0f, 0.0f), b = a;
-        for (uint32_t k = 0; k < n; ++k) {
-            const uint32_t i = upper ? n - 1u - k : k;
-            const float2 c = pts[i];
-            while (m > 1 && turn(a, b, c) <= kErrorMargin) {
-                m -= 1;
-                b = a;
-                if (m >= 2) a = pts[chain[m - 2]];
+#endif
+    uint32_t h = 0;
+    if (n != 0) {
+        const float2* pts = sorted[slot];
+        uint8_t* chain = stack[slot] + upper * kHullSmall;
+        uint32_t m = 0;
+        if (n < 3) {
+            if (!upper)
+                for (uint32_t i = 0; i < n; ++i) chain[i] = (uint8_t)i;
+            m = upper ? 1u : n + 1u;
+        } else {
+            float2 a = make_float2(0.0f, 0.0f), b = a;
+            for (uint32_t k = 0; k < n; ++k) {
+                const uint32_t i = upper ? n - 1u - k : k;
+                const float2 c = pts[i];
+                while (m > 1 && turn(a, b, c) <= kErrorMargin) {
+                    m -= 1;
+                    b = a;
+                    if (m >= 2) a = pts[chain[m - 2]];
+                }
+                chain[m++] = (uint8_t)i;
+                a = b;
+                b = c;
             }
-            chain[m++] = (uint8_t)i;
-            a = b;
-            b = c;
-        }
-    }
-    const uint32_t ml = (uint32_t)__shfl((int)m, (int)(lane & ~1u), 64) - 1u, mu = (uint32_t)__shfl((int)m, (int)(lane | 1u), 64) - 1u;
-    const uint32_t h = ml + mu;
-    const uint8_t* lower_chain = stack[slot];
-    const uint8_t* upper_chain = stack[slot] + kHullSmall;
-    const uint32_t base = s.shape_base[shape * kShapeRow + CH_HULL];
-    for (uint32_t i = upper; i < h; i += 2u) {
-        const uint32_t c = fan_to_strip_source(i, h);
-        const float2 q = pts[c < ml ? lower_chain[c] : upper_chain[c - ml]];
-        s.hull_v[base + i] = {q.x, q.y};
-    }
-    if (!upper) s.hull_count[shape] = h;
+        }
+        const uint32_t ml = (uint32_t)__shfl((int)m, (int)(lane & ~1u), 64) - 1u, mu = (uint32_t)__shfl((int)m, (int)(lane | 1u), 64) - 1u;
+        h = ml + mu;
+        const uint8_t* lower_chain = stack[slot];
+        const uint8_t* upper_chain = stack[slot] + kHullSmall;
+        const uint32_t base = s.shape_base[shape * kShapeRow + CH_HULL];
+        for (uint32_t i = upper; i < h; i += 2u) {
+            const uint32_t c = fan_to_strip_source(i, h);
+            const float2 q = pts[c < ml ? lower_chain[c] : upper_chain[c - ml]];
+            s.hull_v[base + i] = {q.x, q.y};
+        }
+        if (!upper) s.hull_count[shape] = h;
+    }
+    if (out.ncand) hull_small_counts(s, out, first_shape, lane, h);
 }
 
 template <uint32_t CAP, uint32_t QUEUE, uint32_t PACK>
@@ -912,7 +935,7 @@
     hipLaunchKernelGGL(k_shape_rows, dim3((s.n_shapes + 255u) / 256u), dim3(256), 0, stream, s);
     if (mark) mark(ctx, "tess_scan", bytes[1]);
 }
-void launch_emit(const SceneDev& s, hipStream_t stream, MarkFn mark, void* ctx, const uint64_t bytes[4], bool has_stroke, bool big_shapes, const uint32_t* hull_queued) {
+void launch_emit(const SceneDev& s, hipStream_t stream, MarkFn mark, void* ctx, const uint64_t bytes[4], bool has_stroke, bool big_shapes, const uint32_t* hull_queued, const ShapeCounts* counts) {
     if (s.n_elems == 0) return;
     if (s.n_runs) {
         if (s.run_block == 128u) {
@@ -935,7 +958,7 @@
         (void)hipMemsetAsync(s.hull_large_count, 0, 16, stream);
         hipLaunchKernelGGL(k_hull_queues, dim3((s.n_shapes + 255u) / 256u), dim3(256), 0, stream, s);
     }
-    hipLaunchKernelGGL(k_hull_small, dim3((s.n_shapes + kHullBatch - 1u) / kHullBatch), dim3(64 * kHullWaves), 0, stream, s);
+    hipLaunchKernelGGL(k_hull_small, dim3((s.n_shapes + kHullBatch - 1u) / kHullBatch), dim3(64 * kHullWaves), 0, stream, s, (counts && !(has_stroke || big_shapes)) ? *counts : ShapeCounts{nullptr, nullptr, nullptr});
     if (mark) mark(ctx, "tess_hull", bytes[3]);
     if (has_stroke || big_shapes) {
         if (!hull_queued || hull_queued[0]) hipLaunchKernelGGL((k_hull_large<kHullMid, 0, kHullPack>), dim3(min(((hull_queued ? hull_queued[0] : s.n_shapes) + kHullPack - 1u) / kHullPack, 16384u)), dim3(64), 0, stream, s);
diff --git a/include/contrast_hip.h b/include/contrast_hip.h
--- a/include/contrast_hip.h
+++ b/include/contrast_hip.h
@@ -187,6 +187,7 @@
 crh_status crh_scene_layout_all(crh_scene* scene, uint64_t* layout , uint64_t* total_vertex_bytes, uint64_t* total_index_bytes);
 crh_status crh_scene_download_all(crh_scene* scene, void* vertex_bytes, void* index_bytes);
 crh_status crh_scene_traffic(crh_scene* scene, uint64_t* bytes_read, uint64_t* bytes_written);
+crh_status crh_debug_scene_ranges(crh_scene* scene, uint32_t* ncand, uint32_t* prim_begin, uint32_t* nslots, uint32_t* slot_begin);
 
 crh_status crh_scene_set_dynamic_stroke_options(crh_scene* scene, uint32_t shape_index, uint32_t group_index, const crh_dynamic_stroke_options* options);
 
diff --git a/rust/contrast_renderer_hip/src/ffi.rs b/rust/contrast_renderer_hip/src/ffi.rs
--- a/rust/contrast_renderer_hip/src/ffi.rs
+++ b/rust/contrast_renderer_hip/src/ffi.rs
@@ -443,6 +443,7 @@
     pub fn crh_scene_layout_all(scene: *mut crh_scene, layout: *mut u64, total_vertex_bytes: *mut u64, total_index_bytes: *mut u64) -> crh_status;
     pub fn crh_scene_download_all(scene: *mut crh_scene, vertex_bytes: *mut c_void, index_bytes: *mut c_void) -> crh_status;
     pub fn crh_scene_traffic(scene: *mut crh_scene, bytes_read: *mut u64, bytes_written: *mut u64) -> crh_status;
+    pub fn crh_debug_scene_ranges(scene: *mut crh_scene, ncand: *mut u32, prim_begin: *mut u32, nslots: *mut u32, slot_begin: *mut u32) -> crh_status;
     pub fn crh_scene_set_dynamic_stroke_options(scene: *mut crh_scene, shape_index: u32, group_index: u32, options: *const crh_dynamic_stroke_options) -> crh_status;
     pub fn crh_frame_create(renderer: *mut crh_renderer, width: u32, height: u32, out: *mut *mut crh_frame) -> crh_status;
     pub fn crh_frame_create_format(renderer: *mut crh_renderer, width: u32, height: u32, format: u32, out: *mut *mut crh_frame) -> crh_status;
```

Result: no change. 42.94 million, median of 2 (+0.1%).
